# APRIL-ZJU/Ctrl-VIO

Measured on NVIDIA H100. Metric: residual+Jacobian block evaluations per second (sliding-window LM solve), higher is better.
Workload: dtype f64

## Files before the change

ctrl-vio_b200/csrc/engine.cu:

```cuda
#include <cuda_runtime.h>

#include <algorithm>
#include <atomic>
#include <chrono>
#include <cmath>
#include <cstdio>
#include <cstdlib>
#include <cstring>
#include <map>
#include <string>
#include <vector>

#include "../../include/ctvio.h"
#include "frontend.h"
#include "kernels.h"
#include "marginalize.h"
#include "poly_min.h"

using namespace ctvio;

namespace {

thread_local std::string g_err;
int fail(int code, const std::string& msg) {
// ... 205 lines not shown
    d.idx_ld = 6 * nK + 6 * nB;
    d.np = d.idx_ld + 1;
    return d;
  }
  NormalEqPtrs ne(int b) {
    double* s = ne_slab[b].p;
    return NormalEqPtrs{s, s + off_gc, s + off_hl, s + off_gl, s + off_wld, s + off_W, &d_scal.p->cost_eval};
  }
  LandmarkLayout lml() { return LandmarkLayout{d_lo.p, d_hi.p, d_woff.p}; }
};

namespace {

struct ArenaScope {
  PinnedArena* prev;
  explicit ArenaScope(ctvio_engine* e) : prev(g_arena) {
    if (e->stream && cudaStreamQuery(e->stream) == cudaSuccess) e->arena.rewind();
    else cudaGetLastError();
    g_arena = &e->arena;
  }
  ~ArenaScope() { g_arena = prev; }
};

int refresh_mirror(ctvio_engine* e, cudaStream_t on = nullptr) {
  const size_t need = 4 * size_t(e->nK) + kPStride * size_t(e->nK) + 6 * size_t(std::max(e->nB, 1)) + size_t(std::max(e->nL, 1)) + 8;
  if (need > e->h_mirror_cap) {
    if (e->h_mirror) cudaFreeHost(e->h_mirror);
    e->h_mirror = nullptr;
    e->h_mirror_cap = 0;
    if (cudaHostAlloc(reinterpret_cast<void**>(&e->h_mirror), (2 * need) * sizeof(double), cudaHostAllocDefault) != cudaSuccess) {
      cudaGetLastError();
      e->mirror_valid = false;
      return CTVIO_OK;
    }
    e->h_mirror_cap = 2 * need;
  }
  DevState& x = e->x[e->cur];
  double* m = e->h_mirror;
  cudaStream_t st = on ? on : e->stream;
  CUDA_OK(cudaMemcpyAsync(m, x.q.p, 4 * size_t(e->nK) * sizeof(double), cudaMemcpyDeviceToHost, st));
  m += 4 * size_t(e->nK);
  CUDA_OK(cudaMemcpyAsync(m, x.p.p, kPStride * size_t(e->nK) * sizeof(double), cudaMemcpyDeviceToHost, st));
  m += kPStride * size_t(e->nK);
  if (e->nB) CUDA_OK(cudaMemcpyAsync(m, x.bias.p, 6 * size_t(e->nB) * sizeof(double), cudaMemcpyDeviceToHost, st));
  m += 6 * size_t(std::max(e->nB, 1));
  if (e->nL) CUDA_OK(cudaMemcpyAsync(m, x.rho.p, size_t(e->nL) * sizeof(double), cudaMemcpyDeviceToHost, st));
  m += size_t(std::max(e->nL, 1));
  CUDA_OK(cudaMemcpyAsync(m, x.ld.p, sizeof(double), cudaMemcpyDeviceToHost, st));
  e->mirror_valid = true;
  return CTVIO_OK;
}

int knot_window_first(const ctvio_engine* e, int64_t t) {
  int64_t s = (t - e->cfg.t0_ns) / e->cfg.dt_ns;
  return int(s);
}

bool knot_window(const ctvio_engine* e, int64_t t, int& first, int& last) {
  const int64_t maxt = e->cfg.t0_ns + int64_t(e->nK - 3) * e->cfg.dt_ns;
  if (t < e->cfg.t0_ns || t >= maxt) return false;
  const int smax = e->nK - 4;
  const int s1 = knot_window_first(e, t);
  int64_t t2 = t + e->cfg.rs_padding_ns;
  int s2 = (t2 >= maxt) ? smax : int((t2 - e->cfg.t0_ns) / e->cfg.dt_ns);
  if (s2 > s1 + 1) return false;
  first = s1;
  last = std::min(s2 + 3, e->nK - 1);
  return true;
}

int prepare_prior(ctvio_engine* e);
int fetch_new_prior(ctvio_engine* e);

int prepare(ctvio_engine* e) {
  if (!e->have_knots) return fail(CTVIO_ERR_STATE, "knots have not been set");
  ArenaScope arena(e);
  static const bool prep_timing = std::getenv("CTVIO_PREP_TIMING") != nullptr;
  auto tp0 = std::chrono::steady_clock::now();
  auto lap = [&](const char* what) {
    if (!prep_timing) return;
    auto t = std::chrono::steady_clock::now();
    std::fprintf(stderr, "[prepare] %-22s %7.1f us\n", what, std::chrono::duration<double, std::micro>(t - tp0).count());
    tp0 = t;
  };
  if (e->nK < 4) return fail(CTVIO_ERR_STATE, "need at least 4 knots");
  if (!e->have_bias) { e->nB = 0; }
  cudaStream_t st = e->stream;
  const ProblemDims d = e->dims();
  if (e->structure_dirty) {
    e->shard_checked = false;
    const int n = int(e->img.size());
    std::vector<int32_t>&wi0 = e->img_wi0, &wj0 = e->img_wj0;
    wi0.resize(n); wj0.resize(n);
    e->img_li.resize(n); e->img_lj.resize(n);
    e->h_lo.assign(e->nL, INT32_MAX);
    e->h_hi.assign(e->nL, 0);
    struct WinCache { int64_t t = INT64_MIN; int f = 0, l = 0; bool ok = false; } wc[64];
    auto window_of = [&](int64_t t, int& f, int& l) {
      WinCache& c = wc[size_t(uint64_t(t) * 0x9E3779B97F4A7C15ull >> 58)];
      if (c.t != t) { c.t = t; c.ok = knot_window(e, t, c.f, c.l); }
      f = c.f; l = c.l;
      return c.ok;
    };
    for (int k = 0; k < n; ++k) {
      const HostImage& o = e->img[k];
      int f0, l0, f1, l1;
      if (!window_of(o.ti, f0, l0) || !window_of(o.tj, f1, l1))
        return fail(CTVIO_ERR_TIME_RANGE, "image factor time (+ rolling-shutter padding) outside the spline");
      if (o.lm < 0 || o.lm >= e->nL) return fail(CTVIO_ERR_INVALID, "landmark index out of range");
      wi0[k] = f0; wj0[k] = f1;
      e->img_li[k] = l0; e->img_lj[k] = l1;
      e->h_lo[o.lm] = std::min(e->h_lo[o.lm], 6 * std::min(f0, f1));
      e->h_hi[o.lm] = std::max(e->h_hi[o.lm], 6 * (std::max(l0, l1) + 1));
    }
    e->img_order.resize(n);
    {
      bool lm_sorted = true;
      for (int k = 1; k < n && lm_sorted; ++k) lm_sorted = e->img[k - 1].lm <= e->img[k].lm;
      const size_t nKk = size_t(e->nK) + 1;
      if (lm_sorted && nKk * nKk <= (size_t(1) << 22)) {
        std::vector<int32_t> start(nKk * nKk + 1, 0);
        for (int k = 0; k < n; ++k) ++start[size_t(wi0[k]) * nKk + size_t(wj0[k]) + 1];
        for (size_t g = 1; g < start.size(); ++g) start[g] += start[g - 1];
        for (int k = 0; k < n; ++k) e->img_order[start[size_t(wi0[k]) * nKk + size_t(wj0[k])]++] = k;
      } else {
        std::vector<uint64_t> key(n);
        const uint64_t nLl = uint64_t(std::max(e->nL, 1));
        if (uint64_t(nKk) * nKk * nLl < (uint64_t(1) << 40) && uint64_t(n) < (uint64_t(1) << 24)) {
          for (int k = 0; k < n; ++k)
            key[k] = (((uint64_t(wi0[k]) * nKk + uint64_t(wj0[k])) * nLl + uint64_t(e->img[k].lm)) << 24) | uint64_t(k);
          std::sort(key.begin(), key.end());
          for (int k = 0; k < n; ++k) e->img_order[k] = int32_t(key[k] & 0xffffffu);
        } else {
          for (int k = 0; k < n; ++k) e->img_order[k] = k;
          std::stable_sort(e->img_order.begin(), e->img_order.end(), [&](int a, int b) {
            if (wi0[a] != wi0[b]) return wi0[a] < wi0[b];
            if (wj0[a] != wj0[b]) return wj0[a] < wj0[b];
            return e->img[a].lm < e->img[b].lm;
          });
        }
      }
    }
    std::vector<longlong2> ht(n);
    std::vector<double2> hpi(n), hpj(n);
    std::vector<int4> hm(n);
    for (int k = 0; k < n; ++k) {
      const HostImage& o = e->img[e->img_order[k]];
      ht[k] = make_longlong2(o.ti, o.tj);
      hpi[k] = make_double2(o.pi[0], o.pi[1]);
      hpj[k] = make_double2(o.pj[0], o.pj[1]);
      hm[k] = make_int4(o.rowi, o.rowj, o.lm, o.marg);
    }
    lap("image windows + sort");
    int cap = kVisObsPerRound;
    if (const char* env = std::getenv("CTVIO_VIS_CAP")) cap = std::max(kVisObsPerRound, std::atoi(env) / kVisObsPerRound * kVisObsPerRound);
    std::vector<VisualItem>& items = e->h_items;
    items.clear();
    for (int k = 0; k < n;) {
      const int a = e->img_order[k];
      int end = k;
      while (end < n && wi0[e->img_order[end]] == wi0[a] && wj0[e->img_order[end]] == wj0[a]) ++end;
      const int cnt = end - k;
      const int nchunks = (cnt + cap - 1) / cap;
      const int per = (cnt + nchunks - 1) / nchunks;
      for (int s = k; s < end; s += per) items.push_back(VisualItem{s, std::min(per, end - s), wi0[a], wj0[a]});
      k = end;
    }
    e->n_items = int(items.size());
    if (!e->img_desc.empty()) {
      std::vector<ctvio::FactorDesc> sd(n);
      for (int k = 0; k < n; ++k) sd[k] = e->img_desc[e->img_order[k]];
      CUDA_OK(e->d_img_desc.upload(sd, st));
      CUDA_OK(e->d_img_t.reserve(n)); CUDA_OK(e->d_img_pi.reserve(n)); CUDA_OK(e->d_img_pj.reserve(n)); CUDA_OK(e->d_img_meta.reserve(n));
      ctvio::GatherFactorsArgs ga;
      ga.n = n; ga.desc = e->d_img_desc.p; ga.table = e->d_frames.p; ga.frame_t = e->d_frame_t.p;
      ga.frame_cap = ctvio_engine::kFrameCap;
      ga.t = e->d_img_t.p; ga.pi = e->d_img_pi.p; ga.pj = e->d_img_pj.p; ga.meta = e->d_img_meta.p;
      e->launches += ctvio::launch_gather_factors(ga, st);
    } else {
      CUDA_OK(e->d_img_t.upload(ht, st));
      CUDA_OK(e->d_img_pi.upload(hpi, st));
      CUDA_OK(e->d_img_pj.upload(hpj, st));
      CUDA_OK(e->d_img_meta.upload(hm, st));
    }
    CUDA_OK(e->d_img_orig.upload(e->img_order, st));
    CUDA_OK(e->d_items.upload(items, st));

    lap("image arrays + upload");
    e->h_woff.assign(e->nL + 1, 0);
    for (int l = 0; l < e->nL; ++l) {
      if (e->h_hi[l] == 0) e->h_lo[l] = 0;
      e->h_woff[l + 1] = e->h_woff[l] + (e->h_hi[l] - e->h_lo[l]);
    }
    CUDA_OK(e->d_lo.upload(e->h_lo, st));
    CUDA_OK(e->d_hi.upload(e->h_hi, st));
    CUDA_OK(e->d_woff.upload(e->h_woff, st));
    lap("landmark layout");
    const int ni = int(e->imu.size());
    std::vector<longlong2> it(ni);
    std::vector<double2> iga(3 * size_t(ni));
    const int64_t maxt = e->cfg.t0_ns + int64_t(e->nK - 3) * e->cfg.dt_ns;
    std::vector<int32_t>& imu_order = e->imu_order;
    imu_order.assign(ni, 0);
    std::vector<int32_t> imu_s(ni);
    for (int k = 0; k < ni; ++k) {
      const HostImu& o = e->imu[k];
      if (o.t < e->cfg.t0_ns || o.t >= maxt) return fail(CTVIO_ERR_TIME_RANGE, "imu time outside the spline");
      if (o.node < 0 || o.node >= e->nB) return fail(CTVIO_ERR_INVALID, "bias node out of range");
      imu_order[k] = k;
      imu_s[k] = knot_window_first(e, o.t);
    }
    std::stable_sort(imu_order.begin(), imu_order.end(), [&](int a, int b) {
      if (imu_s[a] != imu_s[b]) return imu_s[a] < imu_s[b];
      return e->imu[a].node < e->imu[b].node;
    });
    std::vector<ImuItem> imu_items;
    for (int k = 0; k < ni; ++k) {
      const HostImu& o = e->imu[imu_order[k]];
      it[k] = make_longlong2(o.t, o.node);
      iga[3 * k] = make_double2(o.gyro[0], o.gyro[1]);
      iga[3 * k + 1] = make_double2(o.gyro[2], o.accel[0]);
      iga[3 * k + 2] = make_double2(o.accel[1], o.accel[2]);
      const int s = imu_s[imu_order[k]];
      if (imu_items.empty() || imu_items.back().s != s || imu_items.back().node != o.node ||
          imu_items.back().count >= kImuMaxPerItem)
        imu_items.push_back(ImuItem{k, 0, s, o.node});
      imu_items.back().count++;
    }
    e->n_imu_items = int(imu_items.size());
    CUDA_OK(e->d_imu_items.upload(imu_items, st));
    CUDA_OK(e->d_imu_orig.upload(imu_order, st));
    if (!e->imu_src.empty()) {
      std::vector<int2> src(ni);
      for (int k = 0; k < ni; ++k) src[k] = make_int2(e->imu_src[imu_order[k]], e->imu[imu_order[k]].node);
      CUDA_OK(e->d_imu_src.upload(src, st));
      CUDA_OK(e->d_imu_t.reserve(ni)); CUDA_OK(e->d_imu_ga.reserve(3 * size_t(ni)));
      e->launches += ctvio::launch_gather_imu(e->d_imu_src.p, ni, e->d_imu_tab_t.p, e->d_imu_tab_ga.p, e->d_imu_t.p, e->d_imu_ga.p, st);
    } else {
      CUDA_OK(e->d_imu_t.upload(it, st));
      CUDA_OK(e->d_imu_ga.upload(iga, st));
    }
    const int nb = int(e->biasf.size());
    std::vector<int2> bij(nb);
    std::vector<double> bs(6 * size_t(nb));
    for (int k = 0; k < nb; ++k) {
      const HostBias& o = e->biasf[k];
      if (o.i < 0 || o.i >= e->nB || o.j < 0 || o.j >= e->nB) return fail(CTVIO_ERR_INVALID, "bias node out of range");
      bij[k] = make_int2(o.i, o.j);
      for (int c = 0; c < 6; ++c) bs[6 * k + c] = o.s[c];
    }
    CUDA_OK(e->d_bf_ij.upload(bij, st));
    CUDA_OK(e->d_bf_s.upload(bs, st));

    lap("imu / bias");
    const size_t np = size_t(d.np);
    e->off_gc = np * np;
    e->off_hl = e->off_gc + np;
    e->off_gl = e->off_hl + e->nL;
    e->off_wld = e->off_gl + e->nL;
    e->off_W = e->off_wld + e->nL;
    e->ne_slab_len = e->off_W + size_t(e->h_woff[e->nL]);
    for (int b = 0; b < 2; ++b) CUDA_OK(e->ne_slab[b].reserve(e->ne_slab_len));
    e->npad = ((d.np + kCholNB - 1) / kCholNB) * kCholNB;
    CUDA_OK(e->d_M.reserve(size_t(e->npad) * e->npad + 3 * size_t(e->npad)));
    if (chol_dag_lpub_len(e->npad) > e->d_Linv.cap || chol_dag_part_len(e->npad) > e->d_chol_part.cap || e->linv_npad != e->npad) {
      CUDA_OK(e->d_Linv.reserve(chol_dag_lpub_len(e->npad)));
      CUDA_OK(e->d_chol_part.reserve(chol_dag_part_len(e->npad)));
      e->launches += launch_chol_dag_init(e->d_Linv.p, e->d_chol_part.p, e->npad, e->stream);
      e->linv_npad = e->npad;
      e->chol_seq = 0;
    }
    lap("buffers");
    {
      const int T = e->npad / kCholNB;
      std::vector<std::vector<int32_t>> lists(size_t(T) * (T + 1) / 2);
      std::vector<int32_t> order;
      for (int l = 0; l < e->nL; ++l)
        if (e->h_hi[l] > 0) order.push_back(l);
      std::stable_sort(order.begin(), order.end(), [&](int a, int b) {
        if (e->h_lo[a] != e->h_lo[b]) return e->h_lo[a] < e->h_lo[b];
        return e->h_hi[a] < e->h_hi[b];
      });
      size_t total = 0;
      for (int l : order) {
        int blocks[64], nbk = 0;
        const int b0 = e->h_lo[l] / kCholNB, b1 = (e->h_hi[l] - 1) / kCholNB;
        for (int b = b0; b <= b1 && nbk < 63; ++b) blocks[nbk++] = b;
        for (int x = 0; x < nbk; ++x)
          for (int y = 0; y <= x; ++y) {
            lists[size_t(blocks[x]) * (blocks[x] + 1) / 2 + blocks[y]].push_back(l);
            ++total;
          }
      }
      const int n_sm = device_sm_count();
      const int part = std::max(32, int((total / size_t(2 * n_sm) + 31) / 32) * 32);
      std::vector<SchurTileItem> items;
      std::vector<SchurEntry> flat;
      flat.reserve(total);
      for (int ti = 0; ti < T; ++ti)
        for (int tj = 0; tj <= ti; ++tj) {
          const std::vector<int32_t>& v = lists[size_t(ti) * (ti + 1) / 2 + tj];
          for (size_t s0 = 0; s0 < v.size(); s0 += part)
            items.push_back(SchurTileItem{ti, tj, int32_t(flat.size() + s0), int32_t(std::min(v.size() - s0, size_t(part)))});
          for (int32_t l : v) flat.push_back(SchurEntry{l, e->h_lo[l], e->h_hi[l], 0, e->h_woff[l]});
        }
      e->n_schur_items = int(items.size());
      CUDA_OK(e->d_schur_list.upload(flat, st));
      CUDA_OK(e->d_schur_items.upload(items, st));
      CUDA_OK(e->d_lis.reserve(e->nL));
      CUDA_OK(e->d_lc.reserve(e->nL));
    }
    lap("schur lists");
    if (chol_dag_flags_len(e->npad) > e->d_chol_flags.cap) {
      CUDA_OK(e->d_chol_flags.reserve(chol_dag_flags_len(e->npad)));
      CUDA_OK(cudaMemsetAsync(e->d_chol_flags.p, 0, e->d_chol_flags.cap * sizeof(int32_t), e->stream));
    }
    CUDA_OK(e->d_y.reserve(e->npad));
    CUDA_OK(e->d_sc.reserve(np));
    CUDA_OK(e->d_sl.reserve(e->nL));
    CUDA_OK(e->d_hh.reserve(e->nL));
    CUDA_OK(e->d_dc.reserve(np));
    CUDA_OK(e->d_dl.reserve(e->nL));
    if (e->nL > 0) CUDA_OK(cudaMemsetAsync(e->d_hh.p, 0, sizeof(double) * e->nL, st));
    e->prior_dirty = true;
  }
  lap("reserves");
  if (e->structure_dirty || e->masks_dirty) {
    e->h_cmask.assign(d.np, 0);
    for (int k = 0; k < e->nK; ++k)
      if (e->opt.lock_traj || (e->opt.fixed_knot_index >= 0 && k <= e->opt.fixed_knot_index))
        for (int c = 0; c < 6; ++c) e->h_cmask[6 * k + c] = 1;
    for (int b = 0; b < e->nB; ++b)
      for (int c = 0; c < 3; ++c) {
        if (e->opt.lock_wb) e->h_cmask[d.idx_bias0 + 6 * b + c] = 1;
        if (e->opt.lock_ab) e->h_cmask[d.idx_bias0 + 6 * b + 3 + c] = 1;
      }
    if (e->opt.fix_ld) e->h_cmask[d.idx_ld] = 1;
    std::vector<uint8_t> touched(d.np + e->nL, 0);
    auto mark = [&](int f, int l) {
      for (int k = f; k <= l; ++k)
        for (int c = 0; c < 6; ++c) touched[6 * k + c] = 1;
    };
    {
      std::vector<uint8_t> seen(size_t(e->nK) * 8, 0);
      auto mark_once = [&](int f, int l) {
        uint8_t& sflag = seen[size_t(f) * 8 + size_t(l - f)];
        if (!sflag) { sflag = 1; mark(f, l); }
      };
      const size_t n = e->img.size();
      for (size_t k = 0; k < n; ++k) {
        mark_once(e->img_wi0[k], e->img_li[k]);
        mark_once(e->img_wj0[k], e->img_lj[k]);
        touched[d.np + e->img[k].lm] = 1;
      }
      if (n) touched[d.idx_ld] = 1;
    }
    for (const HostImu& o : e->imu) {
      const int s = knot_window_first(e, o.t);
      mark(s, s + 3);
      for (int c = 0; c < 6; ++c) touched[d.idx_bias0 + 6 * o.node + c] = 1;
    }
    for (const HostBias& o : e->biasf)
      for (int c = 0; c < 6; ++c) touched[d.idx_bias0 + 6 * o.i + c] = touched[d.idx_bias0 + 6 * o.j + c] = 1;
    if (e->prior.n > 0 && e->prior_enabled)
      for (size_t b = 0; b < e->prior.type.size(); ++b) {
        const int g = ctvio::prior_block_base(e->prior.type[b], e->prior.index[b], d.nK, d.nB);
        const int ls = (e->prior.type[b] == CTVIO_BLK_LD || e->prior.type[b] == CTVIO_BLK_RHO) ? 1 : 3;
        if (g >= 0) for (int c = 0; c < ls; ++c) touched[g + c] = 1;
      }
    e->h_active.assign(d.np + e->nL, 0);
    for (int i = 0; i < d.np; ++i) e->h_active[i] = touched[i] && !e->h_cmask[i];
    for (int l = 0; l < e->nL; ++l) e->h_active[d.np + l] = touched[d.np + l];
    CUDA_OK(e->d_cmask.upload(e->h_cmask, st));
    CUDA_OK(e->d_active.upload(e->h_active, st));
    e->masks_dirty = false;
  }
  lap("masks");
  e->structure_dirty = false;
  if (e->prior_dirty) {
    const int rc = prepare_prior(e);
    if (rc != CTVIO_OK) return rc;
  }
// ... 50 lines not shown
PriorPtrs prior_ptrs(ctvio_engine* e) {
  PriorPtrs p;
  std::memset(&p, 0, sizeof(p));
  p.n = e->prior_enabled ? e->prior.n : 0;
  if (p.n <= 0) return p;
  p.n_blocks = int(e->prior.type.size());
  p.J = e->d_prior_J.p; p.r = e->d_prior_r.p; p.JtJ = e->d_prior_JtJ.p;
  p.type = e->d_prior_type.p; p.index = e->d_prior_index.p; p.col = e->d_prior_col.p;
  p.x0 = e->d_prior_x0.p; p.col2g = e->d_prior_col2g.p;
  p.dx = e->d_prior_dx.p; p.res = e->d_prior_res.p;
  return p;
}

VisualLaunch visual_launch(ctvio_engine* e, int xb, int nb, double cauchy) {
  VisualLaunch v;
  v.obs = ImageObsPtrs{e->d_img_t.p, e->d_img_pi.p, e->d_img_pj.p, e->d_img_meta.p, int32_t(e->img.size())};
  v.items = e->d_items.p;
  v.n_items = e->n_items;
  v.st = e->state(xb).ptrs();
  v.ne = e->ne(nb);
  v.lm = e->lml();
  v.dims = e->dims();
  v.sp = e->sp;
  v.rig = e->rig;
  v.cauchy = cauchy;
  v.cmask = e->d_cmask.p;
  v.scal = e->d_scal.p;
  v.use_tma = e->use_tma;
  v.det_ticket = e->deterministic ? e->d_ticket.p : nullptr;
  return v;
}
ImuLaunch imu_launch(ctvio_engine* e, int xb, int nb) {
  ImuLaunch v;
  v.obs = ImuObsPtrs{e->d_imu_t.p, e->d_imu_ga.p, int32_t(e->imu.size())};
  v.items = e->d_imu_items.p;
  v.n_items = e->n_imu_items;
  v.st = e->state(xb).ptrs();
  v.ne = e->ne(nb);
  v.dims = e->dims();
  v.sp = e->sp;
  v.rig = e->rig;
  v.cmask = e->d_cmask.p;
  v.scal = e->d_scal.p;
  v.det_ticket = e->deterministic ? e->d_ticket.p : nullptr;
  return v;
}
SmallFactorsLaunch small_launch(ctvio_engine* e, int xb, int nb) {
  SmallFactorsLaunch v;
  v.bf = BiasFactorPtrs{e->d_bf_ij.p, e->d_bf_s.p, int32_t(e->biasf.size())};
  v.prior = prior_ptrs(e);
  v.st = e->state(xb).ptrs();
  v.ne = e->ne(nb);
  v.dims = e->dims();
  v.cmask = e->d_cmask.p;
  v.scal = e->d_scal.p;
  v.deterministic = e->deterministic ? 1 : 0;
  return v;
}
LinearLaunch linear_launch(ctvio_engine* e, int nb) {
  LinearLaunch a;
  a.dims = e->dims();
  a.ne = e->ne(nb);
  a.lm = e->lml();
  a.schur_list = e->d_schur_list.p;
  a.schur_items = e->d_schur_items.p;
  a.n_schur_items = e->n_schur_items;
  a.lis = e->d_lis.p; a.lc = e->d_lc.p;
  a.cmask = e->d_cmask.p;
  a.active = e->d_active.p;
  a.sc = e->d_sc.p; a.sl = e->d_sl.p;
  a.M = e->d_M.p; a.Linv = e->d_Linv.p; a.y = e->d_y.p;
  a.rhs = e->d_M.p + size_t(e->npad) * e->npad;
  a.diagA = a.rhs + e->npad;
  a.yf = a.diagA + e->npad;
  a.chol_part = e->d_chol_part.p; a.chol_flags = e->d_chol_flags.p; a.chol_seq = &e->chol_seq;
  a.sharded = e->world > 1 ? 1 : 0;
  a.hh = e->d_hh.p; a.dc = e->d_dc.p; a.dl = e->d_dl.p;
  a.npad = e->npad;
  a.scal = e->d_scal.p;
  a.go = nullptr;
  a.det_ticket = e->deterministic ? e->d_ticket.p : nullptr;
  return a;
}

int allreduce_scalars(ctvio_engine* e, bool publish = false) {
  if (e->world <= 1) return CTVIO_OK;
  CUDA_OK(e->d_shard_scal.reserve(8 + 8 * size_t(e->world)));
  e->launches += ctvio::launch_shard_scalars_pack(e->d_scal.p, e->d_shard_scal.p, e->stream);
  std::string err;
  if (!ctvio::comm_allgather(e->nccl_comm, e->d_shard_scal.p, e->d_shard_scal.p + 8, 8, e->stream, &err))
    return fail(CTVIO_ERR_NCCL, err);
  e->launches += ctvio::launch_shard_scalars_reduce(e->d_shard_scal.p + 8, e->world, e->d_scal.p, publish ? e->h_pub : nullptr,
                                                    publish ? ++e->pub_seq : 0, e->stream);
  return CTVIO_OK;
}

int shard_consensus(ctvio_engine* e, int local_rc) {
  if (e->world <= 1) return local_rc;
  const std::string local_msg = g_err;
  cudaStream_t st = e->stream;
  CUDA_OK(e->d_tmp.reserve(16));
  const double flag = local_rc ? 1.0 : 0.0;
  double total = 0.0;
  CUDA_OK(cudaMemcpyAsync(e->d_tmp.p, &flag, sizeof(double), cudaMemcpyHostToDevice, st));
  std::string err;
  if (!ctvio::comm_allreduce_sum(e->nccl_comm, e->d_tmp.p, 1, st, &err)) return fail(CTVIO_ERR_NCCL, err);
  CUDA_OK(cudaMemcpyAsync(&total, e->d_tmp.p, sizeof(double), cudaMemcpyDeviceToHost, st));
  CUDA_OK(cudaStreamSynchronize(st));
  if (local_rc) return fail(local_rc, local_msg);
  if (total != 0.0) return fail(CTVIO_ERR_STATE, "another rank of the sharded solve failed before the first collective");
  return CTVIO_OK;
}

int shard_check_ownership(ctvio_engine* e) {
  if (e->world <= 1 || e->shard_checked) return CTVIO_OK;
  cudaStream_t st = e->stream;
  std::vector<double> owned(size_t(std::max(e->nL, 1)), 0.0);
  for (const HostImage& o : e->img) owned[o.lm] = 1.0;
  CUDA_OK(e->d_rho_sync.reserve(2 * size_t(std::max(e->nL, 1))));
  CUDA_OK(cudaMemcpyAsync(e->d_rho_sync.p, owned.data(), owned.size() * sizeof(double), cudaMemcpyHostToDevice, st));
  std::string err;
  if (!ctvio::comm_allreduce_sum(e->nccl_comm, e->d_rho_sync.p, owned.size(), st, &err)) return fail(CTVIO_ERR_NCCL, err);
  CUDA_OK(cudaMemcpyAsync(owned.data(), e->d_rho_sync.p, owned.size() * sizeof(double), cudaMemcpyDeviceToHost, st));
  CUDA_OK(cudaStreamSynchronize(st));
  for (int l = 0; l < e->nL; ++l)
    if (owned[l] > 1.0)
      return fail(CTVIO_ERR_INVALID, "sharded solve: landmark " + std::to_string(l) + " has observations on " +
                                         std::to_string(int(owned[l])) + " ranks (shard image factors by landmark)");
  e->shard_checked = true;
  return CTVIO_OK;
}

int lm_step(ctvio_engine* e, int nb, double radius, const ApplyLaunch* fused_apply = nullptr, const double* radius_dev = nullptr,
            const int32_t* go = nullptr) {
  LinearLaunch lin = linear_launch(e, nb);
  lin.go = go;
  cudaStream_t st = e->stream;
  if (e->deterministic) cudaMemsetAsync(e->d_ticket.p, 0, 2 * sizeof(int32_t), st);
  e->launches += launch_reduced_system(lin, radius, st, radius_dev);
  if (e->world > 1) {
    std::string err;
    const size_t count = ctvio::shard_pack_len(e->npad);
    CUDA_OK(e->d_shard_pack.reserve(count));
    e->launches += ctvio::launch_shard_pack(lin, e->d_shard_pack.p, st);
    if (!ctvio::comm_allreduce_sum(e->nccl_comm, e->d_shard_pack.p, count, st, &err)) return fail(CTVIO_ERR_NCCL, err);
    e->launches += ctvio::launch_shard_unpack(lin, e->d_shard_pack.p, radius, st);
  }
  e->launches += launch_factor_solve(lin, st);
  if (fused_apply) e->launches += launch_step_and_apply(lin, *fused_apply, st);
  else e->launches += launch_step_vectors(lin, st);
  return CTVIO_OK;
}

void evaluate(ctvio_engine* e, int xb, int nb, bool full, bool reset_cost = true) {
  cudaStream_t st = e->stream;
  if (full) {
    if (e->slab_zeroed[nb]) {
      cudaStreamWaitEvent(st, e->ev_zero, 0);
      e->slab_zeroed[nb] = false;
    } else {
      cudaMemsetAsync(e->ne_slab[nb].p, 0, e->ne_slab_len * sizeof(double), st);
    }
  }
  if (reset_cost) cudaMemsetAsync(&e->d_scal.p->cost_eval, 0, sizeof(double), st);
  const bool fork = (e->rank == 0) && (!e->imu.empty() || !e->biasf.empty() || (e->prior.n > 0 && e->prior_enabled));
  if (e->deterministic) {
    cudaMemsetAsync(e->d_ticket.p, 0, 2 * sizeof(int32_t), st);
    e->launches += launch_visual(visual_launch(e, xb, nb, e->cfg.cauchy_solve), full, st);
    if (fork) {
      cudaMemsetAsync(e->d_ticket.p, 0, 2 * sizeof(int32_t), st);
      e->launches += launch_imu(imu_launch(e, xb, nb), full, st);
      e->launches += launch_small_factors(small_launch(e, xb, nb), full, st);
    }
    return;
  }
  const bool split = fork && !e->imu.empty() && (!e->biasf.empty() || (e->prior.n > 0 && e->prior_enabled));
  if (fork) {
    cudaEventRecord(e->ev_fork, st);
    cudaStreamWaitEvent(e->stream2, e->ev_fork, 0);
    e->launches += launch_imu(imu_launch(e, xb, nb), full, e->stream2);
    if (split) {
      cudaStreamWaitEvent(e->stream3, e->ev_fork, 0);
      e->launches += launch_small_factors(small_launch(e, xb, nb), full, e->stream3);
      cudaEventRecord(e->ev_join3, e->stream3);
    } else {
      e->launches += launch_small_factors(small_launch(e, xb, nb), full, e->stream2);
    }
    cudaEventRecord(e->ev_join, e->stream2);
  }
  e->launches += launch_visual(visual_launch(e, xb, nb, e->cfg.cauchy_solve), full, st);
  if (fork) cudaStreamWaitEvent(st, e->ev_join, 0);
  if (split) cudaStreamWaitEvent(st, e->ev_join3, 0);
}

void prezero_slab(ctvio_engine* e, int nb) {
  cudaMemsetAsync(e->ne_slab[nb].p, 0, e->ne_slab_len * sizeof(double), e->stream2);
  cudaEventRecord(e->ev_zero, e->stream2);
  e->slab_zeroed[nb] = true;
}

int read_scalars(ctvio_engine* e, bool published = false) {
  if (published) {
    volatile unsigned long long* seq = &e->h_pub->seq;
    unsigned spins = 0;
    while (*seq != e->pub_seq) {
      if ((++spins & 0xfffu) == 0 && cudaStreamQuery(e->stream) != cudaErrorNotReady) {
        if (*seq == e->pub_seq) break;
        CUDA_OK(cudaStreamSynchronize(e->stream));
        CUDA_OK(cudaStreamSynchronize(e->stream2));
        if (*seq != e->pub_seq) return fail(CTVIO_ERR_CUDA, "LM step finished without publishing its scalars");
      }
    }
    std::atomic_thread_fence(std::memory_order_acquire);
    *e->h_scal = const_cast<const LmPublished*>(e->h_pub)->s;
  } else {
    CUDA_OK(cudaMemcpyAsync(e->h_scal, e->d_scal.p, sizeof(LmScalars), cudaMemcpyDeviceToHost, e->stream));
    CUDA_OK(cudaStreamSynchronize(e->stream));
  }
  if ((e->h_scal->error_flags & 1) || (e->world > 1 && e->h_scal->err_sum > 0.0)) {
    cudaMemsetAsync(&e->d_scal.p->error_flags, 0, sizeof(int32_t), e->stream);
    return fail(CTVIO_ERR_TIME_RANGE, "a factor time left its knot window / the spline (line delay too large?)");
  }
  return CTVIO_OK;
}

int ensure_table(ctvio_engine* e) {
  if (!e->table_valid) {
    e->launches += launch_knot_table(e->x[e->cur].ptrs(), e->nK, e->stream);
    e->table_valid = true;
  }
  return CTVIO_OK;
}

int alloc_state(ctvio_engine* e, DevState& s) {
  CUDA_OK(s.q.reserve(4 * size_t(e->nK)));
  CUDA_OK(s.p.reserve(kPStride * size_t(e->nK)));
  CUDA_OK(s.tab.reserve(size_t(std::max(e->nK - 1, 1))));
  CUDA_OK(s.bias.reserve(6 * size_t(std::max(e->nB, 1))));
  CUDA_OK(s.rho.reserve(size_t(std::max(e->nL, 1))));
  CUDA_OK(s.ld.reserve(1));
  return CTVIO_OK;
}

}

extern "C" {

const char* ctvio_last_error(void) { return g_err.c_str(); }
int ctvio_abi_version(void) { return CTVIO_ABI_VERSION; }

int ctvio_create(const ctvio_config* cfg, ctvio_handle* out) {
  if (!cfg || !out) return fail(CTVIO_ERR_INVALID, "null argument");
  if (cfg->dt_ns <= 0) return fail(CTVIO_ERR_INVALID, "dt_ns must be positive");
  if (cfg->rs_padding_ns < 0 || cfg->rs_padding_ns > cfg->dt_ns)
    return fail(CTVIO_ERR_INVALID, "rs_padding_ns must lie in [0, dt_ns]: the staged knot window holds 5 knots "
                                   "(4 + one interval of rolling-shutter padding, se3_spline.h:463-503 with 39 ms / 50 ms)");
  int ndev = 0;
  if (cudaGetDeviceCount(&ndev) != cudaSuccess || ndev == 0)
    return fail(CTVIO_ERR_NO_DEVICE, "no CUDA device visible: the ctvio engine has no CPU fallback");
  if (cfg->device < 0 || cfg->device >= ndev) return fail(CTVIO_ERR_NO_DEVICE, "device ordinal out of range");
  CUDA_OK(cudaSetDevice(cfg->device));
  cudaDeviceProp prop;
  CUDA_OK(cudaGetDeviceProperties(&prop, cfg->device));
  if (prop.major != 9 || prop.minor != 0)
    return fail(CTVIO_ERR_NO_DEVICE, "libctvio_b200 is built for sm_90a (H100) only");
  ctvio_engine* e = new ctvio_engine();
  e->cfg = *cfg;
  std::memset(&e->opt, 0, sizeof(e->opt));
  e->opt.fixed_knot_index = -1;
  e->opt.fix_ld = 1;
  e->sp = SplineParams{cfg->t0_ns, cfg->dt_ns, 0, 1e9 / double(cfg->dt_ns)};
  e->rig.R_CI = so3_matrix(Q4{cfg->q_CtoI[0], cfg->q_CtoI[1], cfg->q_CtoI[2], cfg->q_CtoI[3]});
  e->rig.p_CI = V3{cfg->p_CinI[0], cfg->p_CinI[1], cfg->p_CinI[2]};
  e->rig.w_img = cfg->image_weight;
  e->rig.gravity = V3{cfg->gravity[0], cfg->gravity[1], cfg->gravity[2]};
  for (int k = 0; k < 6; ++k) e->rig.imu_info[k] = cfg->imu_info[k];
  if (const char* det = std::getenv("CTVIO_DETERMINISTIC")) e->deterministic = det[0] == '1';
  if (const char* ns = std::getenv("CTVIO_NO_SPECULATION")) e->speculate = ns[0] != '1';
  if (const char* dp = std::getenv("CTVIO_STAGED_PUBLISH")) e->staged_publish = dp[0] == '1';
  const char* no_tma = std::getenv("CTVIO_NO_TMA");
  e->use_tma = !(no_tma && no_tma[0] == '1');
  if (cudaStreamCreateWithFlags(&e->stream, cudaStreamNonBlocking) != cudaSuccess ||
      cudaStreamCreateWithFlags(&e->stream2, cudaStreamNonBlocking) != cudaSuccess ||
      cudaStreamCreateWithFlags(&e->stream3, cudaStreamNonBlocking) != cudaSuccess ||
      cudaEventCreateWithFlags(&e->ev_join3, cudaEventDisableTiming) != cudaSuccess ||
      cudaEventCreate(&e->ev0) != cudaSuccess || cudaEventCreate(&e->ev1) != cudaSuccess ||
      cudaEventCreateWithFlags(&e->ev_fork, cudaEventDisableTiming) != cudaSuccess ||
      cudaEventCreateWithFlags(&e->ev_join, cudaEventDisableTiming) != cudaSuccess ||
      cudaEventCreateWithFlags(&e->ev_zero, cudaEventDisableTiming) != cudaSuccess ||
      cudaEventCreate(&e->ev_iter) != cudaSuccess || e->d_dec.reserve(1) != cudaSuccess || e->d_pubstage.reserve(1) != cudaSuccess ||
      cudaHostAlloc(&e->h_pub, sizeof(LmPublished), cudaHostAllocMapped) != cudaSuccess ||
      cudaMallocHost(&e->h_scal, sizeof(LmScalars)) != cudaSuccess || e->d_scal.reserve(1) != cudaSuccess ||
      e->d_ticket.reserve(4) != cudaSuccess) {
    delete e;
    return fail(CTVIO_ERR_CUDA, "could not create stream / events / scalar block");
  }
  cudaMemsetAsync(e->d_scal.p, 0, sizeof(LmScalars), e->stream);
  std::memset(e->h_pub, 0, sizeof(LmPublished));
  *out = e;
  return CTVIO_OK;
}

int ctvio_destroy(ctvio_handle e) {
  if (!e) return CTVIO_OK;
  cudaSetDevice(e->cfg.device);
  cudaStreamSynchronize(e->stream);
  ctvio::comm_destroy(e->nccl_comm);
  if (e->h_scal) cudaFreeHost(e->h_scal);
  if (e->h_pub) cudaFreeHost(e->h_pub);
  if (e->h_mirror) cudaFreeHost(e->h_mirror);
  if (e->ev_zero) cudaEventDestroy(e->ev_zero);
  cudaEventDestroy(e->ev0);
  cudaEventDestroy(e->ev1);
  cudaEventDestroy(e->ev_fork);
  cudaEventDestroy(e->ev_join);
  cudaStreamDestroy(e->stream2);
  if (e->stream3) cudaStreamDestroy(e->stream3);
  if (e->ev_join3) cudaEventDestroy(e->ev_join3);
  cudaStreamDestroy(e->stream);
  delete e;
  return CTVIO_OK;
}

int ctvio_set_options(ctvio_handle e, const ctvio_options* o) {
  if (!e || !o) return fail(CTVIO_ERR_INVALID, "null argument");
  e->opt = *o;
  e->masks_dirty = true;
  e->prior_dirty = true;
  return CTVIO_OK;
}

int ctvio_set_knots(ctvio_handle e, int32_t n, const double* q, const double* p) {
  if (!e || !q || !p || n < 4) return fail(CTVIO_ERR_INVALID, "need >= 4 knots");
  cudaSetDevice(e->cfg.device);
  if (n != e->nK) e->structure_dirty = true;
  e->nK = n;
  e->sp.n_knots = n;
  for (int b = 0; b < 2; ++b) { const int rc = alloc_state(e, e->x[b]); if (rc) return rc; }
  ArenaScope arena(e);
  std::vector<double> p4(kPStride * size_t(n), 0.0);
  for (int k = 0; k < n; ++k) for (int c = 0; c < 3; ++c) p4[kPStride * k + c] = p[3 * k + c];
  CUDA_OK(staged_h2d(e->x[e->cur].q.p, q, 4 * size_t(n) * sizeof(double), e->stream));
  CUDA_OK(staged_h2d(e->x[e->cur].p.p, p4.data(), p4.size() * sizeof(double), e->stream));
  e->mirror_valid = false;
  e->h2d_bytes += size_t(n) * 56;
// ... 158 lines not shown
                    const int32_t* index, const int32_t* col, const double* x0) {
  if (!e) return fail(CTVIO_ERR_INVALID, "null handle");
  e->prior = ctvio::PriorHost();
  e->prior_dirty = true;
  e->prior_on_device = false;
  e->masks_dirty = true;
  if (n <= 0) return CTVIO_OK;
  if (!J || !r || nb <= 0 || !type || !index || !col || !x0) return fail(CTVIO_ERR_INVALID, "null argument");
  {
    std::vector<uint8_t> covered(size_t(n), 0);
    for (int b = 0; b < nb; ++b) {
      if (type[b] < CTVIO_BLK_ROT || type[b] > CTVIO_BLK_RHO) return fail(CTVIO_ERR_INVALID, "prior block type out of range");
      const int ls = (type[b] == CTVIO_BLK_LD || type[b] == CTVIO_BLK_RHO) ? 1 : 3;
      if (col[b] < 0 || col[b] + ls > n) return fail(CTVIO_ERR_INVALID, "prior block column outside [0, n)");
      for (int c = 0; c < ls; ++c) {
        if (covered[col[b] + c]) return fail(CTVIO_ERR_INVALID, "prior blocks overlap");
        covered[col[b] + c] = 1;
      }
    }
    for (int c = 0; c < n; ++c)
      if (!covered[c]) return fail(CTVIO_ERR_INVALID, "prior blocks do not cover all n columns");
  }
  e->prior.n = n;
  e->prior.J.assign(J, J + size_t(n) * n);
  e->prior.r.assign(r, r + n);
  e->prior.type.assign(type, type + nb);
  e->prior.index.assign(index, index + nb);
  e->prior.col.assign(col, col + nb);
  e->prior.x0.assign(x0, x0 + 4 * size_t(nb));
  return CTVIO_OK;
}

int ctvio_solve(ctvio_handle e, int32_t max_iterations, ctvio_summary* out) {
  if (!e) return fail(CTVIO_ERR_INVALID, "null handle");
  cudaSetDevice(e->cfg.device);
  int rc = prepare(e);
  rc = shard_consensus(e, rc);
  if (rc) return rc;
  rc = shard_check_ownership(e);
  if (rc) return rc;
  cudaStream_t st = e->stream;
  const ProblemDims d = e->dims();
  const double initial_radius = 1e4, max_radius = 1e16, min_radius = 1e-32, min_relative_decrease = 1e-3;
  const double function_tolerance = 1e-6, gradient_tolerance = 1e-10, parameter_tolerance = 1e-8;
  const int max_consecutive_invalid = 5;
  const double ls_sufficient_decrease = 1e-4, ls_max_contraction = 1e-3, ls_min_contraction = 0.6, ls_min_step = 1e-9;
  const int ls_max_iterations = 20;

  ctvio_summary sum;
  std::memset(&sum, 0, sizeof(sum));
  const int64_t launches0 = e->launches;
  cudaEventRecord(e->ev0, st);

  const bool is_constrained = !e->opt.fix_ld && (e->world > 1 || e->h_active[d.idx_ld]);
  if (is_constrained) {
    double ld;
    CUDA_OK(cudaMemcpyAsync(&ld, e->x[e->cur].ld.p, sizeof(double), cudaMemcpyDeviceToHost, st));
    CUDA_OK(cudaStreamSynchronize(st));
    const double c = std::min(std::max(ld, e->opt.ld_lower), e->opt.ld_upper);
    if (c != ld) CUDA_OK(cudaMemcpyAsync(e->x[e->cur].ld.p, &c, sizeof(double), cudaMemcpyHostToDevice, st));
  }
  ensure_table(e);
  const bool sharded = e->world > 1;
  int cur = e->cur;
  evaluate(e, cur, cur, true);
  sum.num_jacobian_evals++;
  LinearLaunch lin = linear_launch(e, cur);
  if (sharded) {
    e->launches += launch_extract_diag(lin, st);
    std::string err;
    if (!ctvio::comm_allreduce_sum(e->nccl_comm, lin.diagA, size_t(e->npad), st, &err)) return fail(CTVIO_ERR_NCCL, err);
    e->launches += launch_jacobi_scale_from_diag(lin, st);
  } else {
    e->launches += launch_jacobi_scale(lin, st);
  }
  if (sharded) {
    e->launches += launch_gradient_norm(lin, e->x[cur].ptrs(), e->opt.fix_ld, e->opt.ld_lower, e->opt.ld_upper, st);
    rc = allreduce_scalars(e);
    if (rc) return rc;
    rc = read_scalars(e);
  } else {
    e->launches += launch_gradient_norm(lin, e->x[cur].ptrs(), e->opt.fix_ld, e->opt.ld_lower, e->opt.ld_upper, st, true, e->h_pub,
                                        ++e->pub_seq);
    rc = read_scalars(e, true);
  }
  if (rc) return rc;
  double x_cost = e->h_scal->cost_eval;
  double gmax = e->h_scal->gmax;
  sum.initial_cost = x_cost;
  sum.num_successful_steps = 1;

  double radius = initial_radius, decrease_factor = 2.0;
  int num_invalid = 0;
  bool last_ok = true;
  int iter = 0;
  int term = CTVIO_TERM_NO_CONVERGENCE;

  auto make_apply = [&](int from, int to, double alpha) {
    ApplyLaunch ap;
    ap.dims = d;
    ap.x = e->state(from).ptrs();
    ap.xc = e->state(to).ptrs();
    ap.dc = e->d_dc.p; ap.dl = e->d_dl.p;
    ap.alpha = alpha;
    ap.active = e->d_active.p;
    ap.count_camera = e->rank == 0 ? 1 : 0;
    ap.clamp_ld = e->opt.fix_ld ? 0 : 1;
    ap.ld_lower = e->opt.ld_lower; ap.ld_upper = e->opt.ld_upper;
    ap.scal = e->d_scal.p;
    ap.det_ticket = e->deterministic ? e->d_ticket.p : nullptr;
    return ap;
  };
  auto apply = [&](int from, int to, double alpha, bool reset = true) {
    if (e->deterministic) cudaMemsetAsync(e->d_ticket.p, 0, 2 * sizeof(int32_t), st);
    e->launches += launch_apply_step(make_apply(from, to, alpha), st, reset);
  };

  bool spec_size_ok = e->img.size() <= 20000;
  if (const char* sp = std::getenv("CTVIO_SPECULATION")) {
    if (std::strcmp(sp, "always") == 0) spec_size_ok = true;
    if (std::strcmp(sp, "never") == 0) spec_size_ok = false;
  }
  const bool pipelined = e->speculate && spec_size_ok && !sharded && !is_constrained && !e->deterministic;
  int cur_ne = cur;
  if (pipelined) {
    rc = alloc_state(e, e->xs);
    if (rc) return rc;
    bool spec_ready = false;
    bool spec_in_flight = false;
    int spec_out = -1;
    unsigned spec_chol_seq0 = e->chol_seq;
    double host_spec_us = 0, host_wait_us = 0;
    static const bool lm_trace = std::getenv("CTVIO_LM_TRACE") != nullptr;
    cudaEventRecord(e->ev_iter, st);
    while (true) {
      if (iter >= max_iterations) { term = CTVIO_TERM_NO_CONVERGENCE; break; }
      if (last_ok && gmax <= gradient_tolerance) { term = CTVIO_TERM_GRADIENT; break; }
      if (radius < min_radius) { term = CTVIO_TERM_MIN_RADIUS; break; }
      ++iter;
      const int cand_ne = cur_ne ^ 1;
      int cand;
      if (spec_ready) {
        cand = spec_out;
        prezero_slab(e, cand_ne);
      } else {
        cand = 0;
        while (cand == cur) ++cand;
        if (!spec_in_flight) prezero_slab(e, cand_ne);
        const ApplyLaunch full_step = make_apply(cur, cand, 1.0);
        rc = lm_step(e, cur_ne, radius, &full_step);
        if (rc) return rc;
      }
      sum.num_linear_solves++;
      evaluate(e, cand, cand_ne, true, false);
      sum.num_jacobian_evals++;
      const LmDecideArgs da{e->d_dec.p, x_cost, radius, min_relative_decrease, max_radius,
                            parameter_tolerance, function_tolerance, gradient_tolerance, min_radius};
      e->launches += launch_gradient_norm(linear_launch(e, cand_ne), e->state(cand).ptrs(), e->opt.fix_ld, e->opt.ld_lower,
                                          e->opt.ld_upper, st, false, e->staged_publish ? e->d_pubstage.p : e->h_pub, ++e->pub_seq,
                                          &da);
      cudaEventRecord(e->ev_iter, st);
      if (e->staged_publish) {
        cudaStreamWaitEvent(e->stream2, e->ev_iter, 0);
        e->launches += launch_publish(e->d_pubstage.p, e->h_pub, e->stream2);
      }
      spec_ready = false;
      if (iter < max_iterations) {
        spec_out = 0;
        while (spec_out == cur || spec_out == cand) ++spec_out;
        const ApplyLaunch spec_step = make_apply(cand, spec_out, 1.0);
        spec_chol_seq0 = e->chol_seq;
        const auto th0 = std::chrono::steady_clock::now();
        rc = lm_step(e, cand_ne, 0.0, &spec_step, &e->d_dec.p->radius_next, &e->d_dec.p->go);
        if (rc) return rc;
        spec_ready = true;
        spec_in_flight = true;
        host_spec_us += std::chrono::duration<double, std::micro>(std::chrono::steady_clock::now() - th0).count();
      }
      const auto th1 = std::chrono::steady_clock::now();
      rc = read_scalars(e, true);
      host_wait_us += std::chrono::duration<double, std::micro>(std::chrono::steady_clock::now() - th1).count();
      if (rc) return rc;
      const LmScalars sc = *e->h_scal;
      const LmDecision dec = const_cast<const LmPublished*>(e->h_pub)->dec;
      if (spec_ready && !dec.go) {
        e->chol_seq = spec_chol_seq0;
        spec_ready = false;
      }
      if (!dec.valid) {
        spec_ready = false;
        ++sum.num_unsuccessful_steps;
        last_ok = false;
        if (++num_invalid >= max_consecutive_invalid) { term = CTVIO_TERM_FAILURE; break; }
        radius /= decrease_factor;
        decrease_factor *= 2.0;
        continue;
      }
      num_invalid = 0;
      const double step_norm = std::sqrt(sc.step_norm2), x_norm = std::sqrt(sc.x_norm2);
      if (step_norm <= parameter_tolerance * (x_norm + parameter_tolerance)) { term = CTVIO_TERM_PARAMETER; break; }
      const double cost_change = x_cost - sc.cost_eval;
      if (std::fabs(cost_change) <= function_tolerance * x_cost) { term = CTVIO_TERM_FUNCTION; break; }
      if (dec.accept) {
        cur = cand;
        cur_ne = cand_ne;
        x_cost = sc.cost_eval;
        gmax = sc.gmax;
        radius = dec.radius_next;
        decrease_factor = 2.0;
        last_ok = true;
        ++sum.num_successful_steps;
        if (!spec_ready) spec_in_flight = false;
      } else {
        spec_ready = false;
        radius /= decrease_factor;
        decrease_factor *= 2.0;
        last_ok = false;
        ++sum.num_unsuccessful_steps;
      }
    }
    if (cur == 2) {
      const int f = 0;
      DevState &a = e->xs, &b = e->x[f];
      std::swap(a.q.p, b.q.p); std::swap(a.q.cap, b.q.cap);
      std::swap(a.p.p, b.p.p); std::swap(a.p.cap, b.p.cap);
      std::swap(a.bias.p, b.bias.p); std::swap(a.bias.cap, b.bias.cap);
      std::swap(a.rho.p, b.rho.p); std::swap(a.rho.cap, b.rho.cap);
      std::swap(a.ld.p, b.ld.p); std::swap(a.ld.cap, b.ld.cap);
      std::swap(a.tab.p, b.tab.p); std::swap(a.tab.cap, b.tab.cap);
      cur = f;
    }
    e->cur = cur;
    e->table_valid = true;
    e->slab_zeroed[0] = e->slab_zeroed[1] = false;
    CUDA_OK(cudaStreamWaitEvent(e->stream2, e->ev_iter, 0));
    {
      const int rcm = refresh_mirror(e, e->stream2);
      if (rcm) return rcm;
    }
    CUDA_OK(cudaStreamSynchronize(e->stream2));
    float ms = 0;
    cudaEventElapsedTime(&ms, e->ev0, e->ev_iter);
    if (lm_trace) std::fprintf(stderr, "[lm] iters %d device %.3f ms host: spec enqueue %.1f us/iter, wait %.1f us/iter\n", iter, ms, host_spec_us / std::max(iter, 1), host_wait_us / std::max(iter, 1));
    sum.iterations = iter;
    sum.termination = term;
    sum.final_cost = x_cost;
    sum.final_radius = radius;
    sum.device_ms = ms;
    sum.kernel_launches = e->launches - launches0;
    if (out) *out = sum;
    return CTVIO_OK;
  }

  while (true) {
    if (iter >= max_iterations) { term = CTVIO_TERM_NO_CONVERGENCE; break; }
    if (last_ok && gmax <= gradient_tolerance) { term = CTVIO_TERM_GRADIENT; break; }
    if (radius < min_radius) { term = CTVIO_TERM_MIN_RADIUS; break; }
    ++iter;
    const int cand = cur ^ 1;
    prezero_slab(e, cand);
    const ApplyLaunch full_step = make_apply(cur, cand, 1.0);
    rc = lm_step(e, cur, radius, &full_step);
    if (rc) return rc;
    sum.num_linear_solves++;
    evaluate(e, cand, cand, true, false);
    sum.num_jacobian_evals++;
    LinearLaunch linc = linear_launch(e, cand);
    if (!sharded) {
      e->launches += launch_gradient_norm(linc, e->x[cand].ptrs(), e->opt.fix_ld, e->opt.ld_lower, e->opt.ld_upper, st, false,
                                          e->h_pub, ++e->pub_seq);
    } else {
      e->launches += launch_gradient_norm(linc, e->x[cand].ptrs(), e->opt.fix_ld, e->opt.ld_lower, e->opt.ld_upper, st, false,
                                          nullptr, 0);
      rc = allreduce_scalars(e, true);
      if (rc) return rc;
    }
    rc = read_scalars(e, true);
    if (rc) return rc;
    LmScalars sc = *e->h_scal;
    const double model_cost_change = -sc.gd - 0.5 * sc.dHd;
    const bool valid = !sc.chol_fail && std::isfinite(model_cost_change) && model_cost_change > 0.0;
    if (!valid) {
      ++sum.num_unsuccessful_steps;
      last_ok = false;
      if (++num_invalid >= max_consecutive_invalid) { term = CTVIO_TERM_FAILURE; break; }
      radius /= decrease_factor;
      decrease_factor *= 2.0;
      continue;
    }
    num_invalid = 0;
    double cand_cost = sc.cost_eval, cand_gmax = sc.gmax, step_norm2 = sc.step_norm2, x_norm2 = sc.x_norm2;
    if (is_constrained) {
      const double g0 = sc.gd;
      struct Sample { double x, value, gradient; bool value_ok, grad_ok; };
      Sample initial{0.0, x_cost, g0, true, true}, previous{0, 0, 0, false, false};
      Sample current{1.0, cand_cost, 0.0, std::isfinite(cand_cost), false};
      bool have_grad = false;
      int ls_iters = 0;
      bool success = true;
      while (!current.value_ok || current.value > x_cost + ls_sufficient_decrease * g0 * current.x) {
        ++ls_iters;
        if (ls_iters >= ls_max_iterations) { success = false; break; }
        if (current.value_ok && !have_grad) {
          e->launches += ctvio::launch_dot_gradient(linear_launch(e, cand), st);
          rc = allreduce_scalars(e);
          if (rc) return rc;
          rc = read_scalars(e);
          if (rc) return rc;
          current.gradient = e->h_scal->gd;
          current.grad_ok = std::isfinite(current.gradient);
        }
        const double smin = ls_max_contraction * current.x, smax = ls_min_contraction * current.x;
        double step;
// ... 190 lines not shown
  if (!e || !counts || !sums) return fail(CTVIO_ERR_INVALID, "null argument");
  cudaSetDevice(e->cfg.device);
  int rc = prepare(e);
  if (rc) return rc;
  ensure_table(e);
  cudaStream_t st = e->stream;
  const size_t ni = e->img.size(), nm = e->imu.size(), nb = e->biasf.size();
  const int np_ = e->prior_enabled ? e->prior.n : 0;
  DevBuf<double> dr, dout;
  DevBuf<int32_t> ds;
  CUDA_OK(dr.reserve(2 * ni + 6 * nm + 8));
  CUDA_OK(ds.reserve(2 * ni + nm + 8));
  CUDA_OK(dout.reserve(18));
  CUDA_OK(cudaMemsetAsync(dout.p, 0, 18 * sizeof(double), st));
  if (ni) e->launches += launch_probe_image(visual_launch(e, e->cur, e->cur, 0.0), e->d_img_orig.p, false, dr.p, ds.p, nullptr, st);
  if (nm) e->launches += launch_probe_imu(imu_launch(e, e->cur, e->cur), e->d_imu_orig.p, false, dr.p + 2 * ni, ds.p + 2 * ni, nullptr, st);
  e->launches += ctvio::launch_abs_column_sums(dr.p, int(ni), 2, dout.p, st);
  e->launches += ctvio::launch_abs_column_sums(dr.p + 2 * ni, int(nm), 6, dout.p + 2, st);
  e->launches += ctvio::launch_bias_abs_sums(e->d_bf_ij.p, e->d_bf_s.p, int(nb), e->x[e->cur].bias.p, dout.p + 8, st);
  if (np_ > 0) {
    e->launches += launch_small_factors(small_launch(e, e->cur, e->cur), false, st);
  }
  rc = read_scalars(e);
  if (rc) return rc;
  CUDA_OK(cudaMemcpy(sums, dout.p, 18 * sizeof(double), cudaMemcpyDeviceToHost));
  counts[0] = int32_t(ni); counts[1] = int32_t(nm); counts[2] = int32_t(nb); counts[3] = np_ > 0 ? 1 : 0;
  if (prior_sum && np_ > 0) {
    CUDA_OK(cudaMemcpy(prior_sum, e->d_prior_res.p, size_t(np_) * sizeof(double), cudaMemcpyDeviceToHost));
    for (int i = 0; i < np_; ++i) prior_sum[i] = std::fabs(prior_sum[i]);
  }
  return CTVIO_OK;
}

int ctvio_eval_cost(ctvio_handle e, double* cost) {
  if (!e || !cost) return fail(CTVIO_ERR_INVALID, "null argument");
  cudaSetDevice(e->cfg.device);
  int rc = prepare(e);
  if (rc) return rc;
  ensure_table(e);
  evaluate(e, e->cur, e->cur, false);
  rc = read_scalars(e);
  if (rc) return rc;
  *cost = e->h_scal->cost_eval;
  return CTVIO_OK;
}

int ctvio_normal_equations(ctvio_handle e, double* Hcc, double* gc, double* hl, double* gl, double* cost) {
  if (!e) return fail(CTVIO_ERR_INVALID, "null handle");
  cudaSetDevice(e->cfg.device);
  int rc = prepare(e);
  if (rc) return rc;
  ensure_table(e);
  evaluate(e, e->cur, e->cur, true);
  rc = read_scalars(e);
  if (rc) return rc;
  const ProblemDims d = e->dims();
  const size_t np = d.np;
  NormalEqPtrs ne = e->ne(e->cur);
  if (Hcc) {
    std::vector<double> up(np * np);
    CUDA_OK(cudaMemcpy(up.data(), ne.A, np * np * sizeof(double), cudaMemcpyDeviceToHost));
    for (size_t i = 0; i < np; ++i)
      for (size_t j = i; j < np; ++j) Hcc[i * np + j] = Hcc[j * np + i] = up[i * np + j];
  }
  if (gc) CUDA_OK(cudaMemcpy(gc, ne.gc, np * sizeof(double), cudaMemcpyDeviceToHost));
  if (hl && e->nL) CUDA_OK(cudaMemcpy(hl, ne.hl, e->nL * sizeof(double), cudaMemcpyDeviceToHost));
  if (gl && e->nL) CUDA_OK(cudaMemcpy(gl, ne.gl, e->nL * sizeof(double), cudaMemcpyDeviceToHost));
  if (cost) *cost = e->h_scal->cost_eval;
  return CTVIO_OK;
}

int ctvio_query_trajectory(ctvio_handle e, int32_t n, const int64_t* t, double* q, double* p, double* omega,
                           double* vel, double* acc) {
  if (!e || n < 0 || (n > 0 && !t)) return fail(CTVIO_ERR_INVALID, "bad argument");
  if (!e->have_knots) return fail(CTVIO_ERR_STATE, "knots have not been set");
  cudaSetDevice(e->cfg.device);
  ensure_table(e);
  if (n == 0) return CTVIO_OK;
  DevBuf<int64_t> dt;
  DevBuf<double> out;
  CUDA_OK(dt.reserve(n));
  CUDA_OK(out.reserve(16 * size_t(n)));
  cudaStream_t st = e->stream;
  CUDA_OK(cudaMemcpyAsync(dt.p, t, size_t(n) * sizeof(int64_t), cudaMemcpyHostToDevice, st));
  QueryLaunch a;
  a.st = e->x[e->cur].ptrs();
  a.sp = e->sp;
  a.n = n;
  a.t = dt.p;
  a.q = out.p; a.p = out.p + 4 * size_t(n); a.omega = out.p + 7 * size_t(n); a.vel = out.p + 10 * size_t(n);
  a.acc = out.p + 13 * size_t(n);
  a.scal = e->d_scal.p;
  e->launches += launch_query(a, st);
  int rc = read_scalars(e);
  if (rc) return rc;
  if (q) CUDA_OK(cudaMemcpy(q, a.q, 4 * size_t(n) * sizeof(double), cudaMemcpyDeviceToHost));
  if (p) CUDA_OK(cudaMemcpy(p, a.p, 3 * size_t(n) * sizeof(double), cudaMemcpyDeviceToHost));
  if (omega) CUDA_OK(cudaMemcpy(omega, a.omega, 3 * size_t(n) * sizeof(double), cudaMemcpyDeviceToHost));
  if (vel) CUDA_OK(cudaMemcpy(vel, a.vel, 3 * size_t(n) * sizeof(double), cudaMemcpyDeviceToHost));
  if (acc) CUDA_OK(cudaMemcpy(acc, a.acc, 3 * size_t(n) * sizeof(double), cudaMemcpyDeviceToHost));
  return CTVIO_OK;
}

int ctvio_triangulate(ctvio_handle e, int32_t n_frames, const double* Rs, const double* Ps, const double* ric,
                      const double* tic, int32_t nl, const int32_t* start_frame, const int32_t* obs_offset,
                      const double* obs_point, int32_t window_size, double init_depth, double* depth) {
  if (!e || n_frames <= 0 || !Rs || !Ps || !ric || !tic || nl < 0 || (nl > 0 && (!start_frame || !obs_offset || !obs_point || !depth)))
    return fail(CTVIO_ERR_INVALID, "bad argument");
  if (nl == 0) return CTVIO_OK;
  cudaSetDevice(e->cfg.device);
  const int total = obs_offset[nl];
  if (total < 0) return fail(CTVIO_ERR_INVALID, "obs_offset must be non-decreasing");
  for (int l = 0; l < nl; ++l)
    if (obs_offset[l + 1] < obs_offset[l]) return fail(CTVIO_ERR_INVALID, "obs_offset must be non-decreasing");
  cudaStream_t st = e->stream;
  const size_t nd = 12 * size_t(n_frames) + 3 * size_t(total) + size_t(nl);
  CUDA_OK(e->d_tmp.reserve(nd));
  CUDA_OK(e->d_tri_idx.reserve(2 * size_t(nl) + 1));
  double* dRs = e->d_tmp.p;
  double* dPs = dRs + 9 * size_t(n_frames);
  double* dobs = dPs + 3 * size_t(n_frames);
  double* ddepth = dobs + 3 * size_t(total);
  CUDA_OK(cudaMemcpyAsync(dRs, Rs, 9 * size_t(n_frames) * sizeof(double), cudaMemcpyHostToDevice, st));
  CUDA_OK(cudaMemcpyAsync(dPs, Ps, 3 * size_t(n_frames) * sizeof(double), cudaMemcpyHostToDevice, st));
  if (total) CUDA_OK(cudaMemcpyAsync(dobs, obs_point, 3 * size_t(total) * sizeof(double), cudaMemcpyHostToDevice, st));
  CUDA_OK(cudaMemcpyAsync(ddepth, depth, size_t(nl) * sizeof(double), cudaMemcpyHostToDevice, st));
  CUDA_OK(cudaMemcpyAsync(e->d_tri_idx.p, start_frame, size_t(nl) * sizeof(int32_t), cudaMemcpyHostToDevice, st));
  CUDA_OK(cudaMemcpyAsync(e->d_tri_idx.p + nl, obs_offset, (size_t(nl) + 1) * sizeof(int32_t), cudaMemcpyHostToDevice, st));
  ctvio::TriangulateArgs a;
  a.n_frames = n_frames; a.Rs = dRs; a.Ps = dPs;
  for (int k = 0; k < 9; ++k) a.ric.m[k] = ric[k];
  a.tic = V3{tic[0], tic[1], tic[2]};
  a.n_landmarks = nl; a.start_frame = e->d_tri_idx.p; a.obs_offset = e->d_tri_idx.p + nl; a.obs_point = dobs;
  a.window_size = window_size; a.init_depth = init_depth; a.depth = ddepth;
  e->launches += ctvio::launch_triangulate(a, st);
  CUDA_OK(cudaMemcpyAsync(depth, ddepth, size_t(nl) * sizeof(double), cudaMemcpyDeviceToHost, st));
  CUDA_OK(cudaStreamSynchronize(st));
  return CTVIO_OK;
}

int ctvio_profile_kernels(ctvio_handle e, int32_t reps, int32_t flush_l2, double* out) {
  if (!e || !out || reps == 0) return fail(CTVIO_ERR_INVALID, "bad argument");
  const bool visual_only = reps < 0;
  if (visual_only) reps = -reps;
  cudaSetDevice(e->cfg.device);
  int rc = prepare(e);
  if (rc) return rc;
  ensure_table(e);
  cudaStream_t st = e->stream;
  const int cur = e->cur, cand = cur ^ 1;
  DevBuf<unsigned char> flush;
  const size_t flush_bytes = size_t(256) << 20;
  if (flush_l2) CUDA_OK(flush.reserve(flush_bytes));
  if (visual_only) {
    for (int k = 0; k < 8; ++k) out[k] = 0.0;
    double total = 0;
    for (int it = -3; it < reps; ++it) {
      if (flush_l2) cudaMemsetAsync(flush.p, it & 0xff, flush_bytes, st);
      cudaMemsetAsync(e->ne_slab[cur].p, 0, e->ne_slab_len * sizeof(double), st);
      cudaEventRecord(e->ev0, st);
      launch_visual(visual_launch(e, cur, cur, e->cfg.cauchy_solve), true, st);
      cudaEventRecord(e->ev1, st);
      if (cudaEventSynchronize(e->ev1) != cudaSuccess) return fail(CTVIO_ERR_CUDA, "kernel failed while profiling");
      float ms = 0;
      cudaEventElapsedTime(&ms, e->ev0, e->ev1);
      if (it >= 0) total += ms;
    }
    out[0] = total / reps;
    cudaMemsetAsync(&e->d_scal.p->error_flags, 0, sizeof(int32_t), st);
    CUDA_OK(cudaStreamSynchronize(st));
    return CTVIO_OK;
  }
  evaluate(e, cur, cur, true);
  LinearLaunch lin = linear_launch(e, cur);
  launch_jacobi_scale(lin, st);
  launch_lm_step(lin, 1e4, st);
  rc = read_scalars(e);
  if (rc) return rc;
  ApplyLaunch ap;
  ap.dims = e->dims();
  ap.x = e->x[cur].ptrs(); ap.xc = e->x[cand].ptrs();
  ap.dc = e->d_dc.p; ap.dl = e->d_dl.p; ap.alpha = 1.0; ap.active = e->d_active.p;
  ap.count_camera = 1;
  ap.clamp_ld = e->opt.fix_ld ? 0 : 1; ap.ld_lower = e->opt.ld_lower; ap.ld_upper = e->opt.ld_upper;
  ap.scal = e->d_scal.p;
  auto time_stage = [&](int stage, double* ms_out) -> int {
    double total = 0;
    for (int it = -3; it < reps; ++it) {
      if (flush_l2) cudaMemsetAsync(flush.p, it & 0xff, flush_bytes, st);
      if (stage == 0 || stage == 1 || stage == 2)
        cudaMemsetAsync(e->ne_slab[cur].p, 0, e->ne_slab_len * sizeof(double), st);
      cudaEventRecord(e->ev0, st);
      switch (stage) {
        case 0: launch_visual(visual_launch(e, cur, cur, e->cfg.cauchy_solve), true, st); break;
        case 1: launch_imu(imu_launch(e, cur, cur), true, st); break;
        case 2: launch_small_factors(small_launch(e, cur, cur), true, st); break;
        case 3: launch_reduced_system(lin, 1e4, st); break;
        case 4: launch_factor_solve(lin, st); break;
        case 5: launch_step_vectors(lin, st); break;
        case 6: launch_apply_step(ap, st); break;
        default: launch_visual(visual_launch(e, cur, cur, e->cfg.cauchy_solve), false, st); break;
      }
      cudaEventRecord(e->ev1, st);
      if (cudaEventSynchronize(e->ev1) != cudaSuccess) return fail(CTVIO_ERR_CUDA, "kernel failed while profiling");
      float ms = 0;
      cudaEventElapsedTime(&ms, e->ev0, e->ev1);
      if (it >= 0) total += ms;
    }
    *ms_out = total / reps;
    return CTVIO_OK;
  };
  for (int stage : {0, 1, 2, 7}) { rc = time_stage(stage, &out[stage]); if (rc) return rc; }
  evaluate(e, cur, cur, true);
  {
    double total3 = 0, total4 = 0, total5 = 0;
    for (int it = -3; it < reps; ++it) {
      float ms;
      if (flush_l2) cudaMemsetAsync(flush.p, it & 0xff, flush_bytes, st);
      cudaEventRecord(e->ev0, st); launch_reduced_system(lin, 1e4, st); cudaEventRecord(e->ev1, st);
      cudaEventSynchronize(e->ev1); cudaEventElapsedTime(&ms, e->ev0, e->ev1); if (it >= 0) total3 += ms;
      if (flush_l2) cudaMemsetAsync(flush.p, it & 0xff, flush_bytes, st);
      cudaEventRecord(e->ev0, st); launch_factor_solve(lin, st); cudaEventRecord(e->ev1, st);
      cudaEventSynchronize(e->ev1); cudaEventElapsedTime(&ms, e->ev0, e->ev1); if (it >= 0) total4 += ms;
      if (flush_l2) cudaMemsetAsync(flush.p, it & 0xff, flush_bytes, st);
      cudaEventRecord(e->ev0, st); launch_step_vectors(lin, st); cudaEventRecord(e->ev1, st);
      cudaEventSynchronize(e->ev1); cudaEventElapsedTime(&ms, e->ev0, e->ev1); if (it >= 0) total5 += ms;
    }
    out[3] = total3 / reps; out[4] = total4 / reps; out[5] = total5 / reps;
  }
  rc = time_stage(6, &out[6]);
  if (rc) return rc;
  cudaMemsetAsync(&e->d_scal.p->error_flags, 0, sizeof(int32_t), st);
  CUDA_OK(cudaStreamSynchronize(st));
  return CTVIO_OK;
}

int ctvio_selfcheck_solver(ctvio_handle e, int32_t reps, int32_t* mismatches, double* rel_residual) {
  if (!e || !mismatches || !rel_residual || reps <= 0) return fail(CTVIO_ERR_INVALID, "bad argument");
  cudaSetDevice(e->cfg.device);
  int rc = prepare(e);
  if (rc) return rc;
  ensure_table(e);
  cudaStream_t st = e->stream;
  const int cur = e->cur;
  evaluate(e, cur, cur, true);
  LinearLaunch lin = linear_launch(e, cur);
  launch_jacobi_scale(lin, st);
  launch_reduced_system(lin, 1e4, st);
  const size_t n = size_t(e->npad), len = n * n + n;
  DevBuf<double> backup;
  CUDA_OK(backup.reserve(len));
  CUDA_OK(cudaMemcpyAsync(backup.p, lin.M, len * sizeof(double), cudaMemcpyDeviceToDevice, st));
  std::vector<double> hM(len), x0(n), x(n);
  CUDA_OK(cudaMemcpyAsync(hM.data(), lin.M, len * sizeof(double), cudaMemcpyDeviceToHost, st));
  *mismatches = 0;
  for (int r = 0; r < reps; ++r) {
    if (r > 0) CUDA_OK(cudaMemcpyAsync(lin.M, backup.p, len * sizeof(double), cudaMemcpyDeviceToDevice, st));
    launch_factor_solve(lin, st);
    CUDA_OK(cudaMemcpyAsync((r == 0 ? x0 : x).data(), lin.y, n * sizeof(double), cudaMemcpyDeviceToHost, st));
    CUDA_OK(cudaStreamSynchronize(st));
    if (r > 0 && std::memcmp(x.data(), x0.data(), n * sizeof(double)) != 0) ++*mismatches;
  }
  for (size_t i = 0; i < n; ++i)
    for (size_t j = i + 1; j < n; ++j) hM[i * n + j] = hM[j * n + i];
  const double* rhs = hM.data() + n * n;
  double rmax = 0, bmax = 0;
  for (size_t i = 0; i < n; ++i) {
    double s = -rhs[i];
    for (size_t j = 0; j < n; ++j) s += hM[i * n + j] * x0[j];
    rmax = std::max(rmax, std::fabs(s));
    bmax = std::max(bmax, std::fabs(rhs[i]));
  }
  *rel_residual = bmax > 0 ? rmax / bmax : rmax;
  cudaMemsetAsync(&e->d_scal.p->error_flags, 0, sizeof(int32_t), st);
  CUDA_OK(cudaStreamSynchronize(st));
  return CTVIO_OK;
}

int ctvio_measure_fp64_tflops(ctvio_handle e, double* tflops) {
  if (!e || !tflops) return fail(CTVIO_ERR_INVALID, "null argument");
  cudaSetDevice(e->cfg.device);
  const double v = ctvio::measure_fp64_tflops(e->stream);
  if (v < 0) return fail(CTVIO_ERR_CUDA, "fp64 micro-benchmark failed");
  *tflops = v;
  return CTVIO_OK;
}

int ctvio_measure_fp64_tensor_tflops(ctvio_handle e, double* tflops) {
  if (!e || !tflops) return fail(CTVIO_ERR_INVALID, "null argument");
  cudaSetDevice(e->cfg.device);
  const double v = ctvio::measure_fp64_tensor_tflops(e->stream);
  if (v < 0) return fail(CTVIO_ERR_CUDA, "fp64 tensor-core micro-benchmark failed");
  *tflops = v;
  return CTVIO_OK;
}

int ctvio_marginalize(ctvio_handle e, int32_t* n_out, int32_t* nb_out) {
  if (!e || !n_out || !nb_out) return fail(CTVIO_ERR_INVALID, "null argument");
  *n_out = 0;
  *nb_out = 0;
  cudaSetDevice(e->cfg.device);
  e->new_prior = ctvio::PriorHost();
  if (!e->opt.is_marg_state) return CTVIO_OK;
  ArenaScope arena(e);
  int rc = prepare(e);
  if (rc) return rc;
  ensure_table(e);
  cudaStream_t st = e->stream;
  const ProblemDims d = e->dims();
  const int later = e->opt.ctrl_to_be_opt_later, nowk = e->opt.ctrl_to_be_opt_now;
  const bool drop_knots = later > nowk;

  struct Key {
    int type, index;
    bool operator<(const Key& o) const {
      auto rank = [](const Key& k) {
        switch (k.type) {
          case CTVIO_BLK_ROT: return std::make_pair(0, 2 * k.index);
          case CTVIO_BLK_POS: return std::make_pair(0, 2 * k.index + 1);
          case CTVIO_BLK_BG: return std::make_pair(1, 2 * k.index);
          case CTVIO_BLK_BA: return std::make_pair(1, 2 * k.index + 1);
          case CTVIO_BLK_LD: return std::make_pair(2, 0);
          default: return std::make_pair(3, k.index);
        }
      };
      return rank(*this) < rank(o);
    }
  };
  struct Info { bool dropped = false; int pos = -1; };
  std::map<Key, Info> blocks;
  auto touch = [&](int type, int index, bool drop) { Info& b = blocks[Key{type, index}]; b.dropped = b.dropped || drop; };
  bool use_prior = false;
  if (e->prior.n > 0) {
    auto is_drop = [&](size_t b) {
      const int t = e->prior.type[b], i = e->prior.index[b];
      const bool isknot = t == CTVIO_BLK_ROT || t == CTVIO_BLK_POS;
      return (isknot && i >= nowk && i < later) || ((t == CTVIO_BLK_BG || t == CTVIO_BLK_BA) && i == 0);
    };
    for (size_t b = 0; b < e->prior.type.size(); ++b) use_prior = use_prior || is_drop(b);
    if (use_prior)
      for (size_t b = 0; b < e->prior.type.size(); ++b) touch(e->prior.type[b], e->prior.index[b], is_drop(b));
  }
  std::vector<int32_t> marg_img, marg_imu;
  for (size_t k = 0; k < e->img_order.size(); ++k) {
    const HostImage& o = e->img[e->img_order[k]];
    if (!o.marg) continue;
    marg_img.push_back(int32_t(k));
    int f0, l0, f1, l1;
    knot_window(e, o.ti, f0, l0);
    knot_window(e, o.tj, f1, l1);
    for (int side = 0; side < 2; ++side)
      for (int kk = (side ? f1 : f0); kk <= (side ? l1 : l0); ++kk) {
        touch(CTVIO_BLK_ROT, kk, drop_knots && kk < later);
        touch(CTVIO_BLK_POS, kk, drop_knots && kk < later);
// ... 498 lines not shown
```

ctrl-vio_b200/csrc/kernels.h:

```cpp
#pragma once
#include <cuda_runtime.h>

#include <atomic>

#include <cstdint>

#include "spline_eval.cuh"

namespace ctvio {

constexpr int kPStride = 4;
constexpr int kVisThreads = 256;
constexpr int kVisObsPerRound = 128;
constexpr int kLocalDim = 64;
constexpr int kRowStride = 66;
constexpr int kObsStride = 2 * kRowStride + 2;
constexpr int kWinKnots = 5;
constexpr int kColLd = 60, kColR = 61, kColRho = 62;
constexpr int kCholNB = 64;

struct StatePtrs {
  double* q;
  double* p;
  double* bias;
// ... 21 lines not shown
};

struct VisualItem {
  int32_t start, count;
  int32_t wi0, wj0;
};

struct ImuObsPtrs {
  const longlong2* t_node;
  const double2* ga;
  int32_t n;
};

struct ImuItem {
  int32_t start, count;
  int32_t s, node;
};
constexpr int kImuMaxPerItem = 32;

struct BiasFactorPtrs {
  const int2* ij;
  const double* sqrt_info;
  int32_t n;
};

struct PriorPtrs {
  int32_t n, n_blocks;
  const double* J;
  const double* r;
  const double* JtJ;
  const int32_t* type;
  const int32_t* index;
  const int32_t* col;
  const double* x0;
  const int32_t* col2g;
  double* dx;
  double* res;
};

struct ProblemDims {
  int32_t nK, nB, nL, np, idx_bias0, idx_ld;
};

struct LandmarkLayout {
  const int32_t* lo;
  const int32_t* hi;
  const int64_t* woff;
};

struct SchurEntry {
  int32_t l, lo, hi, pad;
  int64_t woff;
};
struct SchurTileItem {
  int32_t ti, tj;
  int32_t first, count;
};

struct LmScalars {
  double cost_eval;
  double gd;
  double dHd;
  double step_norm2;
  double x_norm2;
  double err_sum;
  double gmax;
  double dir_max;
  double ld_value;
  int32_t chol_fail;
  int32_t error_flags;
  int32_t pad[2];
};
struct LmDecision {
  double radius_next;
  double model_cost_change;
  double rho;
  int32_t valid;
  int32_t accept;
  int32_t go;
  int32_t pad;
};
struct LmDecideArgs {
  LmDecision* dec;
  double x_cost, radius;
  double min_relative_decrease, max_radius;
  double parameter_tolerance, function_tolerance, gradient_tolerance, min_radius;
};
struct LmPublished {
  LmScalars s;
  LmDecision dec;
  unsigned long long seq;
  unsigned long long pad;
};
constexpr int kLmSumScalars = 6;

struct PerDeviceOnce {
  std::atomic<unsigned long long> mask{0};
  bool first() {
    int d = 0;
    cudaGetDevice(&d);
    const unsigned long long bit = 1ull << (d & 63);
    return !(mask.fetch_or(bit) & bit);
  }
};
inline int device_sm_count() {
  static std::atomic<int> cache[64];
  int d = 0;
  cudaGetDevice(&d);
  int v = cache[d & 63].load(std::memory_order_relaxed);
  if (v == 0) {
    cudaDeviceGetAttribute(&v, cudaDevAttrMultiProcessorCount, d);
    cache[d & 63].store(v, std::memory_order_relaxed);
  }
  return v;
}

#if defined(__CUDACC__)
__device__ __forceinline__ void det_ticket_wait(const int* ticket, int my) {
  if (!ticket) return;
  if (threadIdx.x == 0) {
    int v;
    do { asm volatile("ld.acquire.gpu.global.s32 %0, [%1];" : "=r"(v) : "l"(ticket) : "memory"); } while (v != my);
  }
  __syncthreads();
}
__device__ __forceinline__ void det_ticket_done(int* ticket, int my) {
  if (!ticket) return;
  __threadfence();
  __syncthreads();
  if (threadIdx.x == 0) asm volatile("st.release.gpu.global.s32 [%0], %1;" ::"l"(ticket), "r"(my + 1) : "memory");
}
#endif

int launch_knot_table(const StatePtrs& st, int nK, cudaStream_t s);

struct VisualLaunch {
  ImageObsPtrs obs;
  const VisualItem* items;
  int32_t n_items;
  StatePtrs st;
  NormalEqPtrs ne;
  LandmarkLayout lm;
  ProblemDims dims;
  SplineParams sp;
  RigParams rig;
  double cauchy;
  const uint8_t* cmask;
  LmScalars* scal;
  bool use_tma;
  int* det_ticket = nullptr;
};
int launch_visual(const VisualLaunch& a, bool full, cudaStream_t s);
size_t visual_smem_bytes();

struct ImuLaunch {
  ImuObsPtrs obs;
  const ImuItem* items;
  int32_t n_items;
  StatePtrs st;
  NormalEqPtrs ne;
  ProblemDims dims;
  SplineParams sp;
  RigParams rig;
  const uint8_t* cmask;
  LmScalars* scal;
  int* det_ticket = nullptr;
};
int launch_imu(const ImuLaunch& a, bool full, cudaStream_t s);

struct SmallFactorsLaunch {
  BiasFactorPtrs bf;
  PriorPtrs prior;
  StatePtrs st;
  NormalEqPtrs ne;
  ProblemDims dims;
  const uint8_t* cmask;
  LmScalars* scal;
  int deterministic = 0;
};
int launch_small_factors(const SmallFactorsLaunch& a, bool full, cudaStream_t s);

int launch_probe_image(const VisualLaunch& a, const int32_t* orig_index, bool want_jac, double* r, int32_t* s,
                       double* J, cudaStream_t st);
int launch_probe_imu(const ImuLaunch& a, const int32_t* orig_index, bool want_jac, double* r, int32_t* s, double* J,
                     cudaStream_t st);

struct LinearLaunch {
  ProblemDims dims;
  NormalEqPtrs ne;
  LandmarkLayout lm;
  const SchurEntry* schur_list;
  const SchurTileItem* schur_items;
  int32_t n_schur_items;
  double* lis;
  double* lc;
  const uint8_t* cmask;
  const uint8_t* active;
  double* sc;
  double* sl;
  double* M;
  double* Linv;
  double* rhs;
  double* y;
  double* yf;
  double* chol_part;
  int32_t* chol_flags;
  unsigned* chol_seq;
  double* hh;
  double* diagA;
  int32_t sharded;
  double* dc;
  double* dl;
  int32_t npad;
  LmScalars* scal;
  int* det_ticket;
  const int32_t* go;
};
int launch_jacobi_scale(const LinearLaunch& a, cudaStream_t s);
int launch_lm_step(const LinearLaunch& a, double radius, cudaStream_t s);
int launch_reduced_system(const LinearLaunch& a, double radius, cudaStream_t s, const double* radius_dev = nullptr);
int launch_publish(const LmPublished* stage, LmPublished* pub, cudaStream_t s);
int launch_factor_solve(const LinearLaunch& a, cudaStream_t s);
bool chol_dag_supported(int npad, int n_sm);
size_t chol_dag_part_len(int npad);
size_t chol_dag_flags_len(int npad);
size_t chol_dag_lpub_len(int npad);
int launch_chol_dag_init(double* linv_buf, double* part_buf, int npad, cudaStream_t s);
int launch_chol_dag(const LinearLaunch& a, cudaStream_t s);
int launch_chol_coop(const LinearLaunch& a, cudaStream_t s);
int launch_step_vectors(const LinearLaunch& a, cudaStream_t s);
int launch_add_damping(const LinearLaunch& a, double radius, cudaStream_t s);
int launch_extract_diag(const LinearLaunch& a, cudaStream_t s);
int launch_jacobi_scale_from_diag(const LinearLaunch& a, cudaStream_t s);
int launch_gradient_norm(const LinearLaunch& a, const StatePtrs& st, int fix_ld, double ld_lower, double ld_upper,
                         cudaStream_t s, bool reset = true, LmPublished* pub = nullptr, unsigned long long seq = 0,
                         const LmDecideArgs* decide = nullptr);

struct ApplyLaunch {
  int32_t count_camera;
  ProblemDims dims;
  StatePtrs x, xc;
  const double* dc;
  const double* dl;
  double alpha;
  const uint8_t* active;
  int32_t clamp_ld;
  double ld_lower, ld_upper;
  LmScalars* scal;
  int* det_ticket = nullptr;
};
int launch_apply_step(const ApplyLaunch& a, cudaStream_t s, bool reset = true);
int launch_step_and_apply(const LinearLaunch& a, const ApplyLaunch& ap, cudaStream_t s);
int launch_gauge_realign(const StatePtrs& st, int nK, int min_idx, const double* R0_t0_dev, cudaStream_t s);

struct QueryLaunch {
  StatePtrs st;
  SplineParams sp;
  int32_t n;
  const int64_t* t;
  double *q, *p, *omega, *vel, *acc;
  LmScalars* scal;
};
int launch_query(const QueryLaunch& a, cudaStream_t s);

}
```

ctrl-vio_b200/csrc/kernels_linear.cu:

```cuda
#include <algorithm>

#include "dmma_tiles.cuh"
#include <cstddef>

#include "kernels.h"

namespace ctvio {

__device__ __forceinline__ double warp_sum_d(double v) {
#pragma unroll
  for (int o = 16; o > 0; o >>= 1) v += __shfl_xor_sync(0xffffffffu, v, o);
  return v;
}
__device__ __forceinline__ double warp_max_d(double v) {
#pragma unroll
  for (int o = 16; o > 0; o >>= 1) v = fmax(v, __shfl_xor_sync(0xffffffffu, v, o));
  return v;
}
__device__ __forceinline__ void atomic_max_pos(double* addr, double v) {
  atomicMax(reinterpret_cast<unsigned long long*>(addr), static_cast<unsigned long long>(__double_as_longlong(v)));
}

constexpr double kMinLmDiag = 1e-6, kMaxLmDiag = 1e32;

__global__ void jacobi_scale_kernel(LinearLaunch a) {
  const int i = blockIdx.x * blockDim.x + threadIdx.x;
  const int np = a.dims.np;
  if (i < np) a.sc[i] = 1.0 / (1.0 + sqrt(a.ne.A[size_t(i) * np + i]));
  if (i < a.dims.nL) a.sl[i] = 1.0 / (1.0 + sqrt(a.ne.hl[i]));
}
int launch_jacobi_scale(const LinearLaunch& a, cudaStream_t s) {
  const int n = max(a.dims.np, a.dims.nL);
  jacobi_scale_kernel<<<(n + 255) / 256, 256, 0, s>>>(a);
  return 1;
}

__global__ void scale_copy_kernel(LinearLaunch a, double radius, const double* __restrict__ radius_dev) {
  if (radius_dev) radius = *radius_dev;
  const int npad = a.npad, np = a.dims.np;
  const size_t idx = size_t(blockIdx.x) * blockDim.x + threadIdx.x;
  if (idx < size_t(a.dims.nL)) {
    const int l = int(idx);
    const double sl = a.sl[l], hl = a.ne.hl[l];
    const double hs = sl * sl * hl;
    const double hh = hl > 0.0 ? hs + fmin(fmax(hs, kMinLmDiag), kMaxLmDiag) / radius : 0.0;
    const double is = hh > 0.0 ? rsqrt(hh) * sl : 0.0;
    a.hh[l] = hh;
    a.lis[l] = is;
    a.lc[l] = is * a.ne.gl[l];
  }
  if (idx >= size_t(npad) * npad) return;
  const int i = int(idx / npad), j = int(idx % npad);
  double m;
  const double ident = a.sharded ? 0.0 : 1.0;
  if (i < np && j < np) {
    if (a.cmask[i] || a.cmask[j]) {
      m = (i == j) ? ident : 0.0;
    } else {
      const double v = (i <= j) ? a.ne.A[size_t(i) * np + j] : a.ne.A[size_t(j) * np + i];
      m = a.sc[i] * v * a.sc[j];
      if (i == j) {
        if (a.sharded) a.diagA[i] = v;
        else m += fmin(fmax(m, kMinLmDiag), kMaxLmDiag) / radius;
      }
    }
  } else {
    m = (i == j) ? ident : 0.0;
    if (a.sharded && i == j) a.diagA[i] = 0.0;
  }
  if (a.sharded && i == j && i < np && a.cmask[i]) a.diagA[i] = 0.0;
  a.M[idx] = m;
  if (j == 0) {
    a.rhs[i] = (i < np && !a.cmask[i]) ? a.sc[i] * a.ne.gc[i] : 0.0;
    if (i == 0) {
      a.scal->gd = 0.0;
      a.scal->dHd = 0.0;
      a.scal->dir_max = 0.0;
      a.scal->chol_fail = 0;
      a.scal->step_norm2 = 0.0;
      a.scal->x_norm2 = 0.0;
      a.scal->cost_eval = 0.0;
      a.scal->gmax = 0.0;
    }
  }
}

constexpr int kSchurKC = 32;
__device__ __forceinline__ void schur_fetch(const LinearLaunch& a, const SchurTileItem& it, int c0, int k, int dseg,
                                            const double* scA, const double* scB, double sc_ld, bool diag, double va[8],
                                            double vb[8], double cl[3]) {
#pragma unroll
  for (int e = 0; e < 8; ++e) va[e] = vb[e] = 0.0;
  cl[0] = cl[1] = cl[2] = 0.0;
  if (c0 + k >= it.count) return;
  const SchurEntry en = a.schur_list[it.first + c0 + k];
  const double is = a.lis[en.l];
  const double* Wl = a.ne.W + en.woff - en.lo;
  const int ga0 = kCholNB * it.ti + dseg, gb0 = kCholNB * it.tj + dseg;
  cl[0] = a.lc[en.l];
  cl[1] = is * a.ne.wld[en.l] * sc_ld;
  cl[2] = en.lo / kCholNB == it.ti ? 1.0 : 0.0;
  if (ga0 + 8 > en.lo && ga0 < en.hi) {
#pragma unroll
    for (int e = 0; e < 8; ++e)
      if (ga0 + e >= en.lo && ga0 + e < en.hi) va[e] = is * Wl[ga0 + e] * scA[dseg + e];
  }
  if (!diag && gb0 + 8 > en.lo && gb0 < en.hi) {
#pragma unroll
    for (int e = 0; e < 8; ++e)
      if (gb0 + e >= en.lo && gb0 + e < en.hi) vb[e] = is * Wl[gb0 + e] * scB[dseg + e];
  }
}

__global__ void __launch_bounds__(256, 2) schur_tile_kernel(LinearLaunch a) {
  __shared__ __align__(16) double At[kSchurKC * kTS];
  __shared__ __align__(16) double Bt[kSchurKC * kTS];
  __shared__ double scA[kCholNB], scB[kCholNB], cvec[3][kSchurKC];
  const SchurTileItem it = a.schur_items[blockIdx.x];
  const int tid = threadIdx.x;
  const Lane L = lane_of(tid);
  const int np = a.dims.np, npad = a.npad, ild = a.dims.idx_ld;
  const bool diag = it.ti == it.tj;
  if (tid < kCholNB) {
    const int ga = kCholNB * it.ti + tid, gb = kCholNB * it.tj + tid;
    scA[tid] = (ga < np && !a.cmask[ga]) ? a.sc[ga] : 0.0;
    scB[tid] = (gb < np && !a.cmask[gb]) ? a.sc[gb] : 0.0;
  }
  const double sc_ld = a.cmask[ild] ? 0.0 : a.sc[ild];
  const int go = a.go ? *a.go : 1;
  __syncthreads();
  if (!go) return;
  Frag acc;
  frag_zero(acc);
  double racc = 0.0, lacc = 0.0, ll = 0.0, lr = 0.0;
  const int k = tid >> 3, dseg = (tid & 7) * 8;
  double va[8], vb[8], cl[3];
  schur_fetch(a, it, 0, k, dseg, scA, scB, sc_ld, diag, va, vb, cl);
  for (int c0 = 0; c0 < it.count; c0 += kSchurKC) {
#pragma unroll
    for (int e = 0; e < 8; e += 2) {
      *reinterpret_cast<double2*>(At + k * kTS + dseg + e) = make_double2(va[e], va[e + 1]);
      if (!diag) *reinterpret_cast<double2*>(Bt + k * kTS + dseg + e) = make_double2(vb[e], vb[e + 1]);
    }
    if ((tid & 7) == 0) { cvec[0][k] = cl[0]; cvec[1][k] = cl[1]; cvec[2][k] = cl[2]; }
    __syncthreads();
    if (c0 + kSchurKC < it.count) schur_fetch(a, it, c0 + kSchurKC, k, dseg, scA, scB, sc_ld, diag, va, vb, cl);
    tile_gemm_dmma<false, kSchurKC>(At, diag ? At : Bt, acc, L);
    if (diag) {
      if (tid < kCholNB) {
#pragma unroll 8
        for (int kk = 0; kk < kSchurKC; ++kk) {
          const double v = At[kk * kTS + tid];
          racc = fma(v, cvec[0][kk], racc);
          lacc = fma(v, cvec[1][kk], lacc);
        }
      } else if (tid < kCholNB + kSchurKC) {
        const int kk = tid - kCholNB;
        const double vld = cvec[1][kk] * cvec[2][kk];
// ... 32 lines not shown


__device__ __forceinline__ void camera_step_block(const LinearLaunch& a, int block, double* dsh) {
  __shared__ double red[3][8];
  const int np = a.dims.np;
  const int i = block * 8 + (threadIdx.x >> 5);
  const int lane = threadIdx.x & 31;
  double gd = 0, dHd = 0, dmax = 0;
  const int j0 = block * 8;
  for (int j = j0 + threadIdx.x; j < np; j += blockDim.x) dsh[j - j0] = a.cmask[j] ? 0.0 : -a.sc[j] * a.y[j];
  __syncthreads();
  if (i < np) {
    const double di = dsh[i - j0];
    if (lane == 0) {
      a.dc[i] = di;
      gd = a.ne.gc[i] * di;
      dmax = fabs(di);
      if (!isfinite(di)) a.scal->chol_fail = 1;
    }
    if (di != 0.0) {
      double s = 0;
      for (int j = i + lane; j < np; j += 32) s = fma(a.ne.A[size_t(i) * np + j] * (j == i ? 0.5 : 1.0), dsh[j - j0], s);
      dHd = 2.0 * di * s;
    }
  }
  dHd = warp_sum_d(dHd);
  if (lane == 0) { red[0][threadIdx.x >> 5] = gd; red[1][threadIdx.x >> 5] = dHd; red[2][threadIdx.x >> 5] = dmax; }
  __syncthreads();
  det_ticket_wait(a.det_ticket ? a.det_ticket + 1 : nullptr, blockIdx.x);
  if (threadIdx.x == 0) {
    double g = 0, h = 0, m = 0;
    for (int w = 0; w < 8; ++w) { g += red[0][w]; h += red[1][w]; m = fmax(m, red[2][w]); }
    atomicAdd(&a.scal->gd, g);
    atomicAdd(&a.scal->dHd, h);
    atomic_max_pos(&a.scal->dir_max, m);
  }
  det_ticket_done(a.det_ticket ? a.det_ticket + 1 : nullptr, blockIdx.x);
}

__device__ __forceinline__ void landmark_step_block(const LinearLaunch& a, int block, const ApplyLaunch* ap = nullptr) {
  __shared__ double red[3][8];
  __shared__ double red2[2][8];
  double xn = 0, sn = 0;
  const int lane = threadIdx.x & 31, warp = threadIdx.x >> 5;
  const int l = block * 8 + warp;
  double gd = 0, dHd = 0, dmax = 0;
  if (l < a.dims.nL) {
    const double sl = a.sl[l];
    const int lo = a.lm.lo[l], hi = a.lm.hi[l], ild = a.dims.idx_ld;
    const double* Wl = a.ne.W + a.lm.woff[l] - lo;
    double wy = 0;
    for (int g = lo + lane; g < hi; g += 32) wy = fma(Wl[g], a.cmask[g] ? 0.0 : a.sc[g] * a.y[g], wy);
    wy = warp_sum_d(wy);
    if (lane == 0) {
      wy = fma(a.ne.wld[l], a.cmask[ild] ? 0.0 : a.sc[ild] * a.y[ild], wy);
      const double hh = a.hh[l];
      const double yl = hh > 0.0 ? (sl * a.ne.gl[l] - sl * wy) / hh : 0.0;
      const double d = -sl * yl;
      a.dl[l] = d;
      gd = a.ne.gl[l] * d;
      dHd = 2.0 * d * (-wy) + a.ne.hl[l] * d * d;
      dmax = fabs(d);
      if (!isfinite(d)) a.scal->chol_fail = 1;
      if (ap) {
        const double v = ap->x.rho[l], vn = v + d;
        ap->xc.rho[l] = vn;
        if (ap->active[a.dims.np + l]) { xn = v * v; sn = (v - vn) * (v - vn); }
      }
    }
  }
  if (lane == 0) { red[0][warp] = gd; red[1][warp] = dHd; red[2][warp] = dmax; red2[0][warp] = xn; red2[1][warp] = sn; }
  __syncthreads();
  det_ticket_wait(a.det_ticket ? a.det_ticket + 1 : nullptr, blockIdx.x);
  if (threadIdx.x == 0) {
    double g = 0, h = 0, m = 0, x = 0, s = 0;
    for (int w = 0; w < 8; ++w) { g += red[0][w]; h += red[1][w]; m = fmax(m, red[2][w]); x += red2[0][w]; s += red2[1][w]; }
    if (g != 0.0) atomicAdd(&a.scal->gd, g);
    if (h != 0.0) atomicAdd(&a.scal->dHd, h);
    if (m > 0.0) atomic_max_pos(&a.scal->dir_max, m);
    if (x != 0.0) atomicAdd(&a.scal->x_norm2, x);
    if (s != 0.0) atomicAdd(&a.scal->step_norm2, s);
  }
  det_ticket_done(a.det_ticket ? a.det_ticket + 1 : nullptr, blockIdx.x);
}

__global__ void __launch_bounds__(256) step_vectors_kernel(LinearLaunch a, int ncb) {
  extern __shared__ double step_dsh[];
  if (int(blockIdx.x) < ncb) camera_step_block(a, blockIdx.x, step_dsh);
  else landmark_step_block(a, blockIdx.x - ncb, nullptr);
}

__global__ void add_damping_kernel(LinearLaunch a, double radius) {
  const int i = blockIdx.x * blockDim.x + threadIdx.x;
  if (i >= a.npad) return;
  double* d = a.M + size_t(i) * a.npad + i;
  if (i < a.dims.np && !a.cmask[i]) {
    const double sd = a.sc[i] * a.sc[i] * a.diagA[i];
    *d += fmin(fmax(sd, kMinLmDiag), kMaxLmDiag) / radius;
  } else {
    *d = 1.0;
    a.rhs[i] = 0.0;
  }
}
int launch_add_damping(const LinearLaunch& a, double radius, cudaStream_t s) {
  add_damping_kernel<<<(a.npad + 255) / 256, 256, 0, s>>>(a, radius);
  return 1;
}
__global__ void extract_diag_kernel(LinearLaunch a) {
  const int i = blockIdx.x * blockDim.x + threadIdx.x;
  if (i >= a.npad) return;
  a.diagA[i] = i < a.dims.np ? a.ne.A[size_t(i) * a.dims.np + i] : 0.0;
}
int launch_extract_diag(const LinearLaunch& a, cudaStream_t s) {
  extract_diag_kernel<<<(a.npad + 255) / 256, 256, 0, s>>>(a);
  return 1;
}
__global__ void jacobi_scale_from_diag_kernel(LinearLaunch a) {
  const int i = blockIdx.x * blockDim.x + threadIdx.x;
  if (i < a.dims.np) a.sc[i] = 1.0 / (1.0 + sqrt(a.diagA[i]));
  if (i < a.dims.nL) a.sl[i] = 1.0 / (1.0 + sqrt(a.ne.hl[i]));
}
int launch_jacobi_scale_from_diag(const LinearLaunch& a, cudaStream_t s) {
  const int n = max(a.dims.np, a.dims.nL);
  jacobi_scale_from_diag_kernel<<<(n + 255) / 256, 256, 0, s>>>(a);
  return 1;
}

int launch_reduced_system(const LinearLaunch& a, double radius, cudaStream_t s, const double* radius_dev) {
  int launches = 0;
  const size_t total = std::max(size_t(a.npad) * a.npad, size_t(a.dims.nL));
  scale_copy_kernel<<<unsigned((total + 255) / 256), 256, 0, s>>>(a, radius, radius_dev);
  ++launches;
  if (a.n_schur_items > 0) {
    schur_tile_kernel<<<a.n_schur_items, 256, 0, s>>>(a);
    ++launches;
  }
  return launches;
}

int launch_step_vectors(const LinearLaunch& a, cudaStream_t s) {
  const int ncb = (a.dims.np + 7) / 8, nlb = (a.dims.nL + 7) / 8;
  step_vectors_kernel<<<ncb + nlb, 256, size_t(a.dims.np) * sizeof(double), s>>>(a, ncb);
  return 1;
}

int launch_lm_step(const LinearLaunch& a, double radius, cudaStream_t s) {
  return launch_reduced_system(a, radius, s) + launch_factor_solve(a, s) + launch_step_vectors(a, s);
}

__global__ void __launch_bounds__(1024) gradient_norm_kernel(LinearLaunch a, StatePtrs st, int fix_ld, double ld_lower,
                                                             double ld_upper, LmPublished* pub, unsigned long long seq,
                                                             LmDecideArgs da) {
  __shared__ double red[32];
  const int np = a.dims.np, nL = a.dims.nL;
  double v = 0.0;
  for (int i = blockIdx.x * blockDim.x + threadIdx.x; i < np + nL; i += gridDim.x * blockDim.x) {
    if (!a.active[i]) continue;
    double x;
    if (i < np) {
      x = fabs(a.ne.gc[i]);
      if (i == a.dims.idx_ld && !fix_ld) {
        const double ld = *st.ld;
        x = fabs(ld - fmin(fmax(ld - a.ne.gc[i], ld_lower), ld_upper));
      }
    } else {
      x = fabs(a.ne.gl[i - np]);
    }
    v = fmax(v, x);
  }
  v = warp_max_d(v);
  if ((threadIdx.x & 31) == 0) red[threadIdx.x >> 5] = v;
  __syncthreads();
  if (threadIdx.x < 32) {
    v = warp_max_d(red[threadIdx.x]);
    if (threadIdx.x == 0) {
      bool last = true;
      if (gridDim.x > 1) {
        atomicMax(reinterpret_cast<unsigned long long*>(&a.scal->gmax), static_cast<unsigned long long>(__double_as_longlong(v)));
        __threadfence();
        last = atomicAdd(&a.scal->pad[0], 1) == int(gridDim.x) - 1;
        if (last) a.scal->pad[0] = 0;
      } else {
        a.scal->gmax = fmax(a.scal->gmax, v);
      }
      if (last && pub) {
        static_assert(sizeof(LmScalars) == 88, "scalar block is copied as five 16-byte words + one 8-byte word");
        __threadfence();
        const uint4* src = reinterpret_cast<const uint4*>(a.scal);
        uint4 w[5];
#pragma unroll
        for (int k = 0; k < 5; ++k) w[k] = __ldcg(src + k);
        const uint2 w5 = __ldcg(reinterpret_cast<const uint2*>(src + 5));
        uint4* dst = reinterpret_cast<uint4*>(&pub->s);
#pragma unroll
        for (int k = 0; k < 5; ++k) dst[k] = w[k];
        *reinterpret_cast<uint2*>(dst + 5) = w5;
        if (da.dec) {
          LmScalars sc;
          uint4* loc = reinterpret_cast<uint4*>(&sc);
#pragma unroll
          for (int k = 0; k < 5; ++k) loc[k] = w[k];
          *reinterpret_cast<uint2*>(loc + 5) = w5;
          LmDecision d;
          d.model_cost_change = __dsub_rn(-sc.gd, __dmul_rn(0.5, sc.dHd));
          d.valid = (!sc.chol_fail && isfinite(d.model_cost_change) && d.model_cost_change > 0.0) ? 1 : 0;
          d.rho = __ddiv_rn(__dsub_rn(da.x_cost, sc.cost_eval), d.model_cost_change);
          d.accept = (d.valid && d.rho > da.min_relative_decrease) ? 1 : 0;
          const double t = __dsub_rn(__dmul_rn(2.0, d.rho), 1.0);
          const double t3 = __dmul_rn(__dmul_rn(t, t), t);
          d.radius_next = fmin(da.max_radius, __ddiv_rn(da.radius, fmax(1.0 / 3.0, __dsub_rn(1.0, t3))));
          const double step_norm = sqrt(sc.step_norm2), x_norm = sqrt(sc.x_norm2);
          const bool stop = step_norm <= __dmul_rn(da.parameter_tolerance, __dadd_rn(x_norm, da.parameter_tolerance)) ||
                            fabs(__dsub_rn(da.x_cost, sc.cost_eval)) <= __dmul_rn(da.function_tolerance, da.x_cost) ||
                            fmax(sc.gmax, v) <= da.gradient_tolerance || d.radius_next < da.min_radius;
          d.go = (d.accept && !stop) ? 1 : 0;
          d.pad = 0;
          *da.dec = d;
          pub->dec = d;
        }
        __threadfence_system();
        *reinterpret_cast<volatile unsigned long long*>(&pub->seq) = seq;
      }
    }
  }
}
int launch_gradient_norm(const LinearLaunch& a, const StatePtrs& st, int fix_ld, double ld_lower, double ld_upper,
                         cudaStream_t s, bool reset, LmPublished* pub, unsigned long long seq, const LmDecideArgs* decide) {
  if (reset) cudaMemsetAsync(&a.scal->gmax, 0, sizeof(double), s);
  LmDecideArgs da{};
  if (decide) da = *decide;
  const int n = a.dims.np + a.dims.nL;
  const int grid = std::min(16, std::max(1, (n + 1023) / 1024));
  gradient_norm_kernel<<<grid, 1024, 0, s>>>(a, st, fix_ld, ld_lower, ld_upper, pub, seq, da);
  return 1;
}

__global__ void publish_kernel(const LmPublished* __restrict__ stage, LmPublished* pub) {
  if (threadIdx.x == 0) {
    static_assert(sizeof(LmPublished) % 16 == 0, "copied as 16-byte words");
    constexpr int kWords = int(offsetof(LmPublished, seq) / 16);
    static_assert(offsetof(LmPublished, seq) % 16 == 0, "payload is a whole number of 16-byte words");
    const uint4* src = reinterpret_cast<const uint4*>(stage);
    uint4* dst = reinterpret_cast<uint4*>(pub);
    uint4 w[kWords];
#pragma unroll
    for (int k = 0; k < kWords; ++k) w[k] = __ldcg(src + k);
    const unsigned long long seq = __ldcg(&stage->seq);
#pragma unroll
    for (int k = 0; k < kWords; ++k) dst[k] = w[k];
    __threadfence_system();
    *reinterpret_cast<volatile unsigned long long*>(&pub->seq) = seq;
  }
}
int launch_publish(const LmPublished* stage, LmPublished* pub, cudaStream_t s) {
  publish_kernel<<<1, 32, 0, s>>>(stage, pub);
  return 1;
}

struct StepSource {
  const double* dc;
  const double* y;
  const double* sc;
  const uint8_t* cmask;
  __device__ __forceinline__ double operator()(int g) const {
    if (dc) return dc[g];
    return cmask[g] ? 0.0 : -sc[g] * y[g];
  }
};

__device__ __forceinline__ Q4 stepped_knot(const ApplyLaunch& a, const StepSource& src, int i) {
  const double d0 = src(6 * i), d1 = src(6 * i + 1), d2 = src(6 * i + 2);
  const Q4 q = load_q(a.x.q, i);
  if (d0 != 0.0 || d1 != 0.0 || d2 != 0.0) return so3_mul(q, so3_exp(V3{a.alpha * d0, a.alpha * d1, a.alpha * d2}));
  return q;
}

__device__ __forceinline__ void apply_step_block(const ApplyLaunch& a, const StepSource& src, int block, bool with_landmarks) {
  __shared__ double red[2][8];
  const int i = block * blockDim.x + threadIdx.x;
  const int nK = a.dims.nK, nB = a.dims.nB, nL = with_landmarks ? a.dims.nL : 0;
  double xn = 0, sn = 0;
  if (i < nK) {
    const Q4 q = load_q(a.x.q, i);
    const Q4 qn = stepped_knot(a, src, i);
    a.xc.q[4 * i] = qn.x; a.xc.q[4 * i + 1] = qn.y; a.xc.q[4 * i + 2] = qn.z; a.xc.q[4 * i + 3] = qn.w;
    if (i + 1 < nK) {
      const Q4 qm = stepped_knot(a, src, i + 1);
      const double q2[8] = {qn.x, qn.y, qn.z, qn.w, qm.x, qm.y, qm.z, qm.w};
      KnotPair kp;
      make_knot_pair(q2, 0, kp);
      a.xc.tab[i] = kp;
    }
    if (a.count_camera && a.active[6 * i]) {
      xn += q.x * q.x + q.y * q.y + q.z * q.z + q.w * q.w;
      sn += (q.x - qn.x) * (q.x - qn.x) + (q.y - qn.y) * (q.y - qn.y) + (q.z - qn.z) * (q.z - qn.z) + (q.w - qn.w) * (q.w - qn.w);
    }
#pragma unroll
    for (int c = 0; c < 3; ++c) {
      const double p = a.x.p[kPStride * i + c];
      const double pn = p + a.alpha * src(6 * i + 3 + c);
      a.xc.p[kPStride * i + c] = pn;
      if (a.count_camera && a.active[6 * i + 3 + c]) { xn += p * p; sn += (p - pn) * (p - pn); }
    }
    a.xc.p[kPStride * i + 3] = 0.0;
  } else if (i < nK + 6 * nB) {
    const int b = i - nK;
    const double v = a.x.bias[b];
    const double vn = v + a.alpha * src(a.dims.idx_bias0 + b);
    a.xc.bias[b] = vn;
    if (a.count_camera && a.active[a.dims.idx_bias0 + b]) { xn += v * v; sn += (v - vn) * (v - vn); }
  } else if (i == nK + 6 * nB) {
    const double v = *a.x.ld;
    double vn = v + a.alpha * src(a.dims.idx_ld);
    if (a.clamp_ld) vn = fmin(fmax(vn, a.ld_lower), a.ld_upper);
    *a.xc.ld = vn;
    a.scal->ld_value = vn;
    if (a.count_camera && a.active[a.dims.idx_ld]) { xn += v * v; sn += (v - vn) * (v - vn); }
  } else if (i < nK + 6 * nB + 1 + nL) {
    const int l = i - (nK + 6 * nB + 1);
    const double v = a.x.rho[l];
    const double vn = v + a.alpha * a.dl[l];
    a.xc.rho[l] = vn;
    if (a.active[a.dims.np + l]) { xn += v * v; sn += (v - vn) * (v - vn); }
  }
  xn = warp_sum_d(xn); sn = warp_sum_d(sn);
  if ((threadIdx.x & 31) == 0) { red[0][threadIdx.x >> 5] = xn; red[1][threadIdx.x >> 5] = sn; }
  __syncthreads();
  det_ticket_wait(a.det_ticket ? a.det_ticket + 1 : nullptr, blockIdx.x);
  if (threadIdx.x == 0) {
    double x = 0, s = 0;
    for (int w = 0; w < 8; ++w) { x += red[0][w]; s += red[1][w]; }
    if (x != 0.0) atomicAdd(&a.scal->x_norm2, x);
    if (s != 0.0) atomicAdd(&a.scal->step_norm2, s);
  }
  det_ticket_done(a.det_ticket ? a.det_ticket + 1 : nullptr, blockIdx.x);
}

__global__ void __launch_bounds__(256) apply_step_kernel(ApplyLaunch a) {
  apply_step_block(a, StepSource{a.dc, nullptr, nullptr, nullptr}, blockIdx.x, true);
}

int launch_apply_step(const ApplyLaunch& a, cudaStream_t s, bool reset) {
  const int n = a.dims.nK + 6 * a.dims.nB + 1 + a.dims.nL;
  if (reset) cudaMemsetAsync(&a.scal->step_norm2, 0, 2 * sizeof(double), s);
  apply_step_kernel<<<(n + 255) / 256, 256, 0, s>>>(a);
  return 1;
}

__global__ void __launch_bounds__(256) step_apply_kernel(LinearLaunch a, ApplyLaunch ap, int ncb, int nlb) {
  extern __shared__ double step_dsh[];
  const int b = blockIdx.x;
  if (b < ncb) camera_step_block(a, b, step_dsh);
  else if (b < ncb + nlb) landmark_step_block(a, b - ncb, &ap);
  else apply_step_block(ap, StepSource{nullptr, a.y, a.sc, a.cmask}, b - ncb - nlb, false);
}

int launch_step_and_apply(const LinearLaunch& a, const ApplyLaunch& ap, cudaStream_t s) {
  const int ncb = (a.dims.np + 7) / 8, nlb = (a.dims.nL + 7) / 8;
  const int nab = (a.dims.nK + 6 * a.dims.nB + 1 + 255) / 256;
  step_apply_kernel<<<ncb + nlb + nab, 256, size_t(a.dims.np) * sizeof(double), s>>>(a, ap, ncb, nlb);
  return 1;
}

__device__ void r2ypr_deg(const M3& R, double ypr[3]) {
  const double nx = R.m[0], ny = R.m[3], nz = R.m[6];
  const double ox = R.m[1], oy = R.m[4];
  const double ax = R.m[2], ay = R.m[5];
  const double y = atan2(ny, nx);
  const double p = atan2(-nz, nx * cos(y) + ny * sin(y));
  const double r = atan2(ax * sin(y) - ay * cos(y), -ox * sin(y) + oy * cos(y));
  const double k = 180.0 / 3.14159265358979323846;
  ypr[0] = y * k; ypr[1] = p * k; ypr[2] = r * k;
}

__global__ void gauge_realign_kernel(StatePtrs st, int nK, int min_idx, const double* R0t0) {
  __shared__ double T[16];
  if (threadIdx.x == 0) {
// ... 34 lines not shown
```

ctrl-vio_b200/csrc/kernels_residual.cu:

```cuda
#include <cstdio>

#include "kernels.h"

namespace ctvio {


__device__ __forceinline__ uint32_t smem_u32(const void* p) { return static_cast<uint32_t>(__cvta_generic_to_shared(p)); }

__device__ __forceinline__ void mbar_init(uint64_t* bar, uint32_t count) {
  asm volatile("mbarrier.init.shared::cta.b64 [%0], %1;" ::"r"(smem_u32(bar)), "r"(count) : "memory");
}
__device__ __forceinline__ void fence_mbar_init() { asm volatile("fence.mbarrier_init.release.cluster;" ::: "memory"); }
__device__ __forceinline__ void fence_proxy_async() { asm volatile("fence.proxy.async.shared::cta;" ::: "memory"); }
__device__ __forceinline__ void mbar_expect_tx(uint64_t* bar, uint32_t bytes) {
  asm volatile("mbarrier.arrive.expect_tx.shared::cta.b64 _, [%0], %1;" ::"r"(smem_u32(bar)), "r"(bytes) : "memory");
}
__device__ __forceinline__ void tma_bulk_g2s(void* dst, const void* src, uint32_t bytes, uint64_t* bar) {
  asm volatile("cp.async.bulk.shared::cluster.global.mbarrier::complete_tx::bytes [%0], [%1], %2, [%3];" ::"r"(
                   smem_u32(dst)),
               "l"(src), "r"(bytes), "r"(smem_u32(bar))
               : "memory");
}
__device__ __forceinline__ bool mbar_try_wait(uint64_t* bar, uint32_t phase) {
  uint32_t ok;
  asm volatile(
      "{\n"
      ".reg .pred p;\n"
      "mbarrier.try_wait.parity.shared::cta.b64 p, [%1], %2;\n"
      "selp.u32 %0, 1, 0, p;\n"
      "}\n"
      : "=r"(ok)
      : "r"(smem_u32(bar)), "r"(phase)
      : "memory");
  return ok != 0;
}

__device__ __forceinline__ double warp_sum(double v) {
#pragma unroll
  for (int o = 16; o > 0; o >>= 1) v += __shfl_xor_sync(0xffffffffu, v, o);
  return v;
}


__global__ void knot_table_kernel(StatePtrs st, int nK) {
  const int k = blockIdx.x * blockDim.x + threadIdx.x;
  if (k >= nK - 1) return;
  KnotPair kp;
  make_knot_pair(st.q, k, kp);
  st.tab[k] = kp;
}

int launch_knot_table(const StatePtrs& st, int nK, cudaStream_t s) {
  if (nK < 2) return 0;
  knot_table_kernel<<<(nK - 1 + 127) / 128, 128, 0, s>>>(st, nK);
  return 1;
}


struct VisArgs {
  ImageObsPtrs obs;
  const VisualItem* items;
  StatePtrs st;
  NormalEqPtrs ne;
  LandmarkLayout lm;
  ProblemDims dims;
  SplineParams sp;
  RigParams rig;
  double cauchy;
  const uint8_t* cmask;
  LmScalars* scal;
  int use_tma;
  int* det_ticket;
};

struct __align__(128) VisStatic {
  KnotPair tab[2][4];
  double q[2][kWinKnots][4];
  double p[2][kWinKnots][4];
  double cost_part[8];
  unsigned long long bar;
  int err;
};

__constant__ uint8_t c_tile_i[36] = {0, 0, 0, 0, 0, 0, 0, 0, 1, 1, 1, 1, 1, 1, 1, 2, 2, 2,
                                     2, 2, 2, 3, 3, 3, 3, 3, 4, 4, 4, 4, 5, 5, 5, 6, 6, 7};
__constant__ uint8_t c_tile_j[36] = {0, 1, 2, 3, 4, 5, 6, 7, 1, 2, 3, 4, 5, 6, 7, 2, 3, 4,
                                     5, 6, 7, 3, 4, 5, 6, 7, 4, 5, 6, 7, 5, 6, 7, 6, 7, 7};

#ifdef CTVIO_CHOL_TIMING
__device__ long long g_vis_clk[8];
#define VCLK(i) do { if (blockIdx.x == 0 && threadIdx.x == 0) g_vis_clk[(i)] = clock64(); } while (0)
extern "C" int ctvio_debug_vis_clk(long long* out) {
  return cudaMemcpyFromSymbol(out, g_vis_clk, sizeof(g_vis_clk)) == cudaSuccess ? 0 : -1;
}
#else
#define VCLK(i)
#endif

size_t visual_smem_bytes() {
  return size_t(kVisObsPerRound) * kObsStride * sizeof(double) + size_t(36) * 64 * sizeof(double);
}

__device__ __noinline__ void syrk_round(const double* Jt, double* accs, int nround, int tid) {
  const int warp = tid >> 5, lane = tid & 31, g = lane >> 2, q = lane & 3;
  const int nblk = warp < 6 ? 1 : 2;
  int bi[2], bj[2];
  if (warp < 6) {
    bi[0] = warp < 3 ? 0 : (warp < 5 ? 1 : 2);
    bj[0] = warp < 3 ? warp + 1 : (warp < 5 ? warp - 1 : 3);
    bi[1] = bj[1] = 0;
  } else {
    bi[0] = bj[0] = 2 * (warp - 6);
    bi[1] = bj[1] = 2 * (warp - 6) + 1;
  }
  const bool dg = warp >= 6;
  double acc[2][2][2][2];
#pragma unroll
  for (int b = 0; b < 2; ++b)
#pragma unroll
    for (int mi = 0; mi < 2; ++mi)
#pragma unroll
      for (int nj = 0; nj < 2; ++nj) {
        const int ti = 2 * bi[b] + mi, tj = 2 * bj[b] + nj;
        double2 v = make_double2(0.0, 0.0);
        if (b < nblk && ti <= tj) v = *reinterpret_cast<const double2*>(accs + (ti * 8 - ti * (ti - 1) / 2 + (tj - ti)) * 64 + g * 8 + 2 * q);
        acc[b][mi][nj][0] = v.x; acc[b][mi][nj][1] = v.y;
      }
  const int nsteps = (2 * nround + 3) >> 2;
#pragma unroll 2
  for (int st = 0; st < nsteps; ++st) {
    const int row = 4 * st + q;
    const double* rp = Jt + size_t(row >> 1) * kObsStride + (row & 1) * kRowStride + g;
#pragma unroll
    for (int b = 0; b < 2; ++b) {
      if (b < nblk) {
        double av[2], bv[2];
#pragma unroll
        for (int m = 0; m < 2; ++m) {
          av[m] = rp[16 * bi[b] + 8 * m];
          bv[m] = dg ? av[m] : rp[16 * bj[b] + 8 * m];
        }
#pragma unroll
        for (int mi = 0; mi < 2; ++mi)
#pragma unroll
          for (int nj = 0; nj < 2; ++nj) {
            if (dg && mi == 1 && nj == 0) continue;
            asm volatile("mma.sync.aligned.m8n8k4.row.col.f64.f64.f64.f64 {%0,%1}, {%2}, {%3}, {%0,%1};"
                         : "+d"(acc[b][mi][nj][0]), "+d"(acc[b][mi][nj][1])
                         : "d"(av[mi]), "d"(bv[nj]));
          }
      }
    }
  }
#pragma unroll
  for (int b = 0; b < 2; ++b)
#pragma unroll
    for (int mi = 0; mi < 2; ++mi)
#pragma unroll
      for (int nj = 0; nj < 2; ++nj) {
        const int ti = 2 * bi[b] + mi, tj = 2 * bj[b] + nj;
        if (b < nblk && ti <= tj)
          *reinterpret_cast<double2*>(accs + (ti * 8 - ti * (ti - 1) / 2 + (tj - ti)) * 64 + g * 8 + 2 * q) =
              make_double2(acc[b][mi][nj][0], acc[b][mi][nj][1]);
      }
  __syncthreads();
}

template <bool FULL>
__global__ void __launch_bounds__(kVisThreads, 1) visual_kernel(const __grid_constant__ VisArgs a) {
  extern __shared__ __align__(128) unsigned char dyn_smem[];
  double* Jt = reinterpret_cast<double*>(dyn_smem);
  double* accs = Jt + size_t(kVisObsPerRound) * kObsStride;
  __shared__ VisStatic sm;

  const int tid = threadIdx.x;
  const int lane = tid & 31, warp = tid >> 5;
  const VisualItem item = a.items[blockIdx.x];
  const int nK = a.dims.nK;
  VCLK(0);

  const int w0[2] = {item.wi0, item.wj0};
  if (a.use_tma) {
    if (tid == 0) {
      sm.err = 0;
      mbar_init(reinterpret_cast<uint64_t*>(&sm.bar), 1);
      fence_mbar_init();
    }
    __syncthreads();
    if (tid == 0) {
      uint32_t bytes = 0;
#pragma unroll
      for (int sd = 0; sd < 2; ++sd) {
        const int nk = min(kWinKnots, nK - w0[sd]);
        const int npair = min(4, nK - 1 - w0[sd]);
        bytes += uint32_t(nk) * 64u + uint32_t(npair) * uint32_t(sizeof(KnotPair));
      }
      mbar_expect_tx(reinterpret_cast<uint64_t*>(&sm.bar), bytes);
#pragma unroll
      for (int sd = 0; sd < 2; ++sd) {
        const int nk = min(kWinKnots, nK - w0[sd]);
        const int npair = min(4, nK - 1 - w0[sd]);
        tma_bulk_g2s(&sm.q[sd][0][0], a.st.q + 4 * w0[sd], uint32_t(nk) * 32u, reinterpret_cast<uint64_t*>(&sm.bar));
        tma_bulk_g2s(&sm.p[sd][0][0], a.st.p + 4 * w0[sd], uint32_t(nk) * 32u, reinterpret_cast<uint64_t*>(&sm.bar));
        tma_bulk_g2s(&sm.tab[sd][0], a.st.tab + w0[sd], uint32_t(npair) * uint32_t(sizeof(KnotPair)),
                     reinterpret_cast<uint64_t*>(&sm.bar));
      }
    }
  } else {
    if (tid == 0) sm.err = 0;
    for (int i = tid; i < 2 * kWinKnots * 4; i += kVisThreads) {
      const int sd = i / (kWinKnots * 4), r = i % (kWinKnots * 4);
      const int k = w0[sd] + r / 4;
      (&sm.q[sd][0][0])[r] = k < nK ? a.st.q[4 * k + (r & 3)] : 0.0;
      (&sm.p[sd][0][0])[r] = k < nK ? a.st.p[4 * k + (r & 3)] : 0.0;
    }
    for (int i = tid; i < 2 * 4 * 16; i += kVisThreads) {
      const int sd = i / 64, r = i % 64;
      const int k = w0[sd] + r / 16;
      reinterpret_cast<double*>(&sm.tab[sd][0])[r] = k < nK - 1 ? reinterpret_cast<const double*>(a.st.tab + k)[r & 15] : 0.0;
    }
  }
  if (FULL)
    for (int i = tid; i < 36 * 64; i += kVisThreads) accs[i] = 0.0;
  if (a.use_tma) {
    while (!mbar_try_wait(reinterpret_cast<uint64_t*>(&sm.bar), 0)) {
    }
  }
  __syncthreads();

  const double ld = *a.st.ld;
  const int64_t ld_ns = int64_t(ld * 1e9);
  const int side = tid & 1;
  double cost_local = 0.0;
  VCLK(1);

  for (int base = 0; base < item.count; base += kVisObsPerRound) {
    const int nround = min(kVisObsPerRound, item.count - base);
    const int ol = tid >> 1;
    const bool active = ol < nround;
    double* row0 = Jt + size_t(ol) * kObsStride;
    double* row1 = row0 + kRowStride;
    bool valid = false;
    const unsigned m_act = __ballot_sync(0xffffffffu, active);
    if (active) {
      const int oi = item.start + base + ol;
      const longlong2 tt = a.obs.t[oi];
      const double2 pi = a.obs.pi[oi];
      const double2 pj = a.obs.pj[oi];
      const int4 meta = a.obs.meta[oi];
      const double rho = a.st.rho[meta.z];
      const int64_t w_base = FULL ? a.lm.woff[meta.z] - a.lm.lo[meta.z] : 0;
      const int64_t t_eval = side == 0 ? tt.x + int64_t(meta.x) * ld_ns : tt.y + int64_t(meta.y) * ld_ns;
      int32_t s;
      double u;
      bool ok = spline_index(a.sp, t_eval, s, u);
      const int slot = s - w0[side];
      ok = ok && (slot == 0 || slot == 1);
      const bool ok_both = __shfl_xor_sync(m_act, ok ? 1 : 0, 1) && ok;
      const unsigned m_ok = __ballot_sync(m_act, ok_both);
      valid = ok_both;
      if (!ok_both) {
        atomicOr(&sm.err, 1);
      } else {
        PoseStage ev;
        pose_stage<FULL, kPStride>(a.sp, &sm.q[side][0][0], &sm.p[side][0][0], sm.tab[side], slot, u, ev);
        M3 Ro;
        V3 po, omo, vo;
#pragma unroll
        for (int e = 0; e < 9; ++e) Ro.m[e] = __shfl_xor_sync(m_ok, ev.R.m[e], 1);
        po = V3{__shfl_xor_sync(m_ok, ev.p.x, 1), __shfl_xor_sync(m_ok, ev.p.y, 1), __shfl_xor_sync(m_ok, ev.p.z, 1)};
        if (FULL) {
          omo = V3{__shfl_xor_sync(m_ok, ev.omega.x, 1), __shfl_xor_sync(m_ok, ev.omega.y, 1),
                   __shfl_xor_sync(m_ok, ev.omega.z, 1)};
          vo = V3{__shfl_xor_sync(m_ok, ev.vel.x, 1), __shfl_xor_sync(m_ok, ev.vel.y, 1),
                  __shfl_xor_sync(m_ok, ev.vel.z, 1)};
        }
        const M3& R_i = side == 0 ? ev.R : Ro;
        const M3& R_j = side == 0 ? Ro : ev.R;
        const V3 p_i = side == 0 ? ev.p : po;
        const V3 p_j = side == 0 ? po : ev.p;
        ImageCommon cm;
        const double pixy[2] = {pi.x, pi.y}, pjxy[2] = {pj.x, pj.y};
        image_common(a.rig, pixy, pjxy, rho, R_i, p_i, R_j, p_j, a.cauchy, cm);
        if (side == 0) cost_local += cm.cost;
        if (FULL) {
          double jrho[2], lhs[6];
          image_jrho(a.rig, cm, R_i, rho, jrho);
          image_side_lhs(side, cm, ev.R, lhs);
          const int cb = side * 30;
          const int gk0 = w0[side];
          const int l = meta.z;
          double* Wl = a.ne.W + w_base;
          {
            const int unused = cb + (slot == 0 ? 4 : 0) * 6;
#pragma unroll
            for (int c = 0; c < 6; ++c) { row0[unused + c] = 0.0; row1[unused + c] = 0.0; }
          }
          const double sgn = side == 0 ? 1.0 : -1.0;
          jacobian_stage(sm.tab[side], ev, [&](int k, const M3& Jk) {
            double rk[6];
            mul23_33(lhs, Jk, rk);
            const int gd = 6 * (gk0 + slot + k);
            const int col = cb + (slot + k) * 6;
            const double ck = sgn * ev.c[k];
#pragma unroll
            for (int c = 0; c < 3; ++c) {
              const bool mr = a.cmask[gd + c] != 0, mp = a.cmask[gd + 3 + c] != 0;
              const double r0v = mr ? 0.0 : rk[c], r1v = mr ? 0.0 : rk[3 + c];
              const double p0v = mp ? 0.0 : ck * cm.JvR[c], p1v = mp ? 0.0 : ck * cm.JvR[3 + c];
              row0[col + c] = r0v; row1[col + c] = r1v;
              row0[col + 3 + c] = p0v; row1[col + 3 + c] = p1v;
#ifndef CTVIO_EXPERIMENT_NO_W_ATOMICS
              if (!a.det_ticket) {
                if (!mr) atomicAdd(Wl + gd + c, r0v * jrho[0] + r1v * jrho[1]);
                if (!mp) atomicAdd(Wl + gd + 3 + c, p0v * jrho[0] + p1v * jrho[1]);
              }
#endif
            }
          });
          if (side == 0) {
            row0[kColR] = cm.r[0]; row1[kColR] = cm.r[1];
            row0[kColRho] = jrho[0]; row1[kColRho] = jrho[1];
          } else {
            double jld[2];
            image_jld(a.rig, cm, meta.x, meta.y, R_i, omo, vo, R_j, ev.omega, ev.vel, jld);
            const bool ld_const = a.cmask[a.dims.idx_ld] != 0;
            row0[kColLd] = ld_const ? 0.0 : jld[0];
            row1[kColLd] = ld_const ? 0.0 : jld[1];
            row0[63] = 0.0; row1[63] = 0.0;
          }
          if (!a.det_ticket) {
            if (side == 0) {
              atomicAdd(a.ne.hl + l, jrho[0] * jrho[0] + jrho[1] * jrho[1]);
              atomicAdd(a.ne.gl + l, jrho[0] * cm.r[0] + jrho[1] * cm.r[1]);
            } else {
              atomicAdd(a.ne.wld + l, row0[kColLd] * jrho[0] + row1[kColLd] * jrho[1]);
            }
          }
        }
      }
    }
    if (FULL) {
      if (!valid && ol < kVisObsPerRound) {
        const int cb = side * 30;
        for (int c = 0; c < 30; ++c) { row0[cb + c] = 0.0; row1[cb + c] = 0.0; }
        if (side == 0) { row0[kColR] = row1[kColR] = 0.0; row0[kColRho] = row1[kColRho] = 0.0; }
        else { row0[kColLd] = row1[kColLd] = 0.0; row0[63] = row1[63] = 0.0; }
      }
      VCLK(2);
      __syncthreads();
      VCLK(3);
      if (a.det_ticket) {
        det_ticket_wait(a.det_ticket, blockIdx.x * 1024 + base / kVisObsPerRound);
        if (active && valid) {
          const int oi = item.start + base + ol;
          const int l = a.obs.meta[oi].z;
          const double j0 = row0[kColRho], j1 = row1[kColRho];
          if (side == 0) {
            atomicAdd(a.ne.hl + l, j0 * j0 + j1 * j1);
            atomicAdd(a.ne.gl + l, j0 * row0[kColR] + j1 * row1[kColR]);
          } else {
            atomicAdd(a.ne.wld + l, row0[kColLd] * j0 + row1[kColLd] * j1);
          }
        }
        for (int ph = 0; ph < 2; ++ph) {
          if (active && valid && side == ph) {
            const int oi = item.start + base + ol;
            const int l = a.obs.meta[oi].z;
            const double j0 = row0[kColRho], j1 = row1[kColRho];
            double* Wl = a.ne.W + (a.lm.woff[l] - a.lm.lo[l]);
            const int cb = side * 30, gk0 = w0[side];
            for (int c = 0; c < 30; ++c) {
              const double v = row0[cb + c] * j0 + row1[cb + c] * j1;
              if (v != 0.0) atomicAdd(Wl + 6 * gk0 + c, v);
            }
          }
          __threadfence();
          __syncthreads();
        }
        det_ticket_done(a.det_ticket, blockIdx.x * 1024 + base / kVisObsPerRound);
      }
      syrk_round(Jt, accs, nround, tid);
      VCLK(4);
    }
  }

  const int n_rounds = (item.count + kVisObsPerRound - 1) / kVisObsPerRound;
  det_ticket_wait(a.det_ticket, blockIdx.x * 1024 + (FULL ? n_rounds : 0));
  cost_local = warp_sum(cost_local);
  if (lane == 0) sm.cost_part[warp] = cost_local;
  __syncthreads();
  if (tid == 0) {
    double c = 0;
#pragma unroll
    for (int w = 0; w < kVisThreads / 32; ++w) c += sm.cost_part[w];
    atomicAdd(a.ne.cost, c);
    if (sm.err) atomicOr(&a.scal->error_flags, 1);
  }
  if (FULL) {
    const int np = a.dims.np;
    const int n_class = a.det_ticket ? 11 : 1;
    for (int cls = 0; cls < n_class; ++cls) {
      for (int idx = tid; idx < 36 * 64; idx += kVisThreads) {
        const double val = accs[idx];
        if (val == 0.0) continue;
        const int tile = idx >> 6, e = idx & 63;
        const int la = c_tile_i[tile] * 8 + (e >> 3), lb = c_tile_j[tile] * 8 + (e & 7);
        if (la > lb || lb > kColR || la >= kColR) continue;
        const int sa = la < 30 ? 0 : (la < 60 ? 1 : 2);
        const int ga = sa == 0 ? 6 * item.wi0 + la : (sa == 1 ? 6 * item.wj0 + (la - 30) : a.dims.idx_ld);
        if (lb == kColR) {
          if (n_class > 1 && cls != 8 + sa) continue;
          atomicAdd(a.ne.gc + ga, val);
          continue;
        }
        const int sb = lb < 30 ? 0 : (lb < 60 ? 1 : 2);
        const int gb = sb == 0 ? 6 * item.wi0 + lb : (sb == 1 ? 6 * item.wj0 + (lb - 30) : a.dims.idx_ld);
        if (n_class > 1) {
          int c;
          if (sb == 2) c = 5 + sa;
          else if (sa == sb) c = sa == 0 ? 0 : 4;
          else c = ga < gb ? 1 : (ga > gb ? 2 : 3);
          if (c != cls) continue;
        }
        const double v = (la != lb && ga == gb) ? 2.0 * val : val;
        const int g0 = min(ga, gb), g1 = max(ga, gb);
        atomicAdd(a.ne.A + size_t(g0) * np + g1, v);
      }
      if (n_class > 1) {
        __threadfence();
        __syncthreads();
      }
    }
  }
  if (a.det_ticket) {
    __threadfence();
    __syncthreads();
    if (tid == 0) asm volatile("st.release.gpu.global.s32 [%0], %1;" ::"l"(a.det_ticket), "r"((int(blockIdx.x) + 1) * 1024) : "memory");
  }
  VCLK(5);
}

int launch_visual(const VisualLaunch& l, bool full, cudaStream_t s) {
  if (l.n_items <= 0) return 0;
  VisArgs a{l.obs, l.items, l.st, l.ne, l.lm, l.dims, l.sp, l.rig, l.cauchy, l.cmask, l.scal, l.use_tma ? 1 : 0, l.det_ticket};
  static PerDeviceOnce once;
  if (once.first()) {
    cudaFuncSetAttribute(visual_kernel<true>, cudaFuncAttributeMaxDynamicSharedMemorySize, int(visual_smem_bytes()));
    cudaFuncSetAttribute(visual_kernel<false>, cudaFuncAttributeMaxDynamicSharedMemorySize, int(visual_smem_bytes()));
  }
  if (full) visual_kernel<true><<<l.n_items, kVisThreads, visual_smem_bytes(), s>>>(a);
  else visual_kernel<false><<<l.n_items, kVisThreads, 0, s>>>(a);
  return 1;
}


struct ImuArgs {
  ImuObsPtrs obs;
  const ImuItem* items;
  StatePtrs st;
  NormalEqPtrs ne;
  ProblemDims dims;
  SplineParams sp;
  RigParams rig;
  const uint8_t* cmask;
  LmScalars* scal;
  int* det_ticket;
};

constexpr int kImuThreads = 64;
constexpr int kImuCols = 32;
constexpr int kImuRowStride = 34;
__constant__ uint8_t c_imu_tile_i[10] = {0, 0, 0, 0, 1, 1, 1, 2, 2, 3};
__constant__ uint8_t c_imu_tile_j[10] = {0, 1, 2, 3, 1, 2, 3, 2, 3, 3};

template <bool FULL>
__global__ void __launch_bounds__(kImuThreads) imu_kernel(const __grid_constant__ ImuArgs a) {
  extern __shared__ __align__(16) unsigned char dyn_smem[];
  double* Js = reinterpret_cast<double*>(dyn_smem);
  double* accs = Js + kImuMaxPerItem * 6 * kImuRowStride;
  const int tid = threadIdx.x;
  const ImuItem item = a.items[blockIdx.x];
  double cost = 0.0;
  if (FULL)
    for (int i = tid; i < 10 * 64; i += kImuThreads) accs[i] = 0.0;
  if (tid < item.count) {
    const int n = item.start + tid;
    const longlong2 tn = a.obs.t_node[n];
    const double2 g0 = a.obs.ga[3 * n], g1 = a.obs.ga[3 * n + 1], g2 = a.obs.ga[3 * n + 2];
    const double gyro[3] = {g0.x, g0.y, g1.x}, accel[3] = {g1.y, g2.x, g2.y};
    const int node = item.node;
    double bias[6];
#pragma unroll
    for (int c = 0; c < 6; ++c) bias[c] = a.st.bias[6 * node + c];
    int32_t s;
    double u;
    const bool ok = spline_index(a.sp, tn.x, s, u) && s == item.s;
    double* J = Js + size_t(tid) * 6 * kImuRowStride;
    if (!ok) {
      atomicOr(&a.scal->error_flags, 1);
      if (FULL)
        for (int e = 0; e < 6 * kImuRowStride; ++e) J[e] = 0.0;
    } else {
      ImuEvalOut o;
      eval_imu<FULL, kPStride>(a.sp, a.rig, a.st.q, a.st.p, a.st.tab, s, u, gyro, accel, bias, o);
      cost = o.cost;
      if (FULL) {
        const int gb0 = a.dims.idx_bias0 + 6 * node;
#pragma unroll
        for (int r = 0; r < 6; ++r) {
          double* Jr = J + r * kImuRowStride;
#pragma unroll
          for (int k = 0; k < 4; ++k)
#pragma unroll
            for (int c = 0; c < 3; ++c) {
              Jr[k * 6 + c] = a.cmask[6 * (s + k) + c] ? 0.0 : o.Jrot[k][3 * r + c];
              Jr[k * 6 + 3 + c] = a.cmask[6 * (s + k) + 3 + c] ? 0.0 : o.Jpos[k][3 * r + c];
            }
#pragma unroll
          for (int c = 0; c < 6; ++c) Jr[24 + c] = (c == r && !a.cmask[gb0 + c]) ? a.rig.imu_info[r] : 0.0;
          Jr[30] = o.r[r];
          Jr[31] = 0.0;
        }
      }
    }
  }
  if (FULL) {
    __syncthreads();
    const int grp = tid / 10, tile = tid % 10;
    double acc[64];
    if (tid < 60) {
      const int ti = c_imu_tile_i[tile], tj = c_imu_tile_j[tile];
#pragma unroll
      for (int e = 0; e < 64; ++e) acc[e] = 0.0;
      const int nrows = 6 * item.count;
      for (int row = grp; row < nrows; row += 6) {
        const double2* ra = reinterpret_cast<const double2*>(Js + size_t(row) * kImuRowStride + ti * 8);
        const double2* rb = reinterpret_cast<const double2*>(Js + size_t(row) * kImuRowStride + tj * 8);
        double av[8], bv[8];
#pragma unroll
        for (int e = 0; e < 4; ++e) {
          const double2 x = ra[e], y = rb[e];
          av[2 * e] = x.x; av[2 * e + 1] = x.y;
          bv[2 * e] = y.x; bv[2 * e + 1] = y.y;
        }
#pragma unroll
        for (int i = 0; i < 8; ++i)
#pragma unroll
          for (int j = 0; j < 8; ++j) acc[i * 8 + j] = fma(av[i], bv[j], acc[i * 8 + j]);
      }
    }
    for (int g = 0; g < 6; ++g) {
      if (tid < 60 && grp == g) {
#pragma unroll
        for (int e = 0; e < 64; ++e) accs[tile * 64 + e] += acc[e];
      }
      __syncthreads();
    }
    const int np = a.dims.np;
    det_ticket_wait(a.det_ticket, blockIdx.x);
    for (int idx = tid; idx < 10 * 64; idx += kImuThreads) {
      const double val = accs[idx];
      if (val == 0.0) continue;
      const int tile2 = idx >> 6, e = idx & 63;
      const int la = c_imu_tile_i[tile2] * 8 + (e >> 3), lb = c_imu_tile_j[tile2] * 8 + (e & 7);
      if (la > lb || lb > 30 || la >= 30) continue;
      const int ga = la < 24 ? 6 * item.s + la : a.dims.idx_bias0 + 6 * item.node + (la - 24);
      if (lb == 30) {
        atomicAdd(a.ne.gc + ga, val);
        continue;
      }
      const int gb = lb < 24 ? 6 * item.s + lb : a.dims.idx_bias0 + 6 * item.node + (lb - 24);
      atomicAdd(a.ne.A + size_t(ga) * np + gb, val);
    }
  }
  if (!FULL) det_ticket_wait(a.det_ticket, blockIdx.x);
  cost = warp_sum(cost);
  if (tid == 0 && cost != 0.0) atomicAdd(a.ne.cost, cost);
  det_ticket_done(a.det_ticket, blockIdx.x);
}

int launch_imu(const ImuLaunch& l, bool full, cudaStream_t s) {
  if (l.n_items <= 0) return 0;
  ImuArgs a{l.obs, l.items, l.st, l.ne, l.dims, l.sp, l.rig, l.cmask, l.scal, l.det_ticket};
  const size_t smem = (size_t(kImuMaxPerItem) * 6 * kImuRowStride + 10 * 64) * sizeof(double);
  static PerDeviceOnce once;
  if (once.first()) cudaFuncSetAttribute(imu_kernel<true>, cudaFuncAttributeMaxDynamicSharedMemorySize, int(smem));
  if (full) imu_kernel<true><<<l.n_items, kImuThreads, smem, s>>>(a);
  else imu_kernel<false><<<l.n_items, kImuThreads, 0, s>>>(a);
  return 1;
}


struct SmallArgs {
  BiasFactorPtrs bf;
  PriorPtrs prior;
  StatePtrs st;
  NormalEqPtrs ne;
  ProblemDims dims;
  const uint8_t* cmask;
  LmScalars* scal;
  int deterministic;
};

__device__ __forceinline__ const double* block_data(const StatePtrs& st, int type, int index) {
  switch (type) {
    case 0: return st.q + 4 * index;
    case 1: return st.p + kPStride * index;
    case 2: return st.bias + 6 * index;
    case 3: return st.bias + 6 * index + 3;
    case 4: return st.ld;
    default: return st.rho + index;
  }
}

template <bool FULL>
__global__ void __launch_bounds__(256) small_factors_kernel(const __grid_constant__ SmallArgs a) {
  __shared__ double red[8];
  const int tid = threadIdx.x;
  double cost = 0.0;
  const int np = a.dims.np;
  for (int n = a.deterministic ? (tid == 0 ? 0 : a.bf.n) : tid; n < a.bf.n; n += a.deterministic ? 1 : blockDim.x) {
    const int2 ij = a.bf.ij[n];
#pragma unroll
    for (int k = 0; k < 6; ++k) {
      const double s = a.bf.sqrt_info[6 * n + k];
      const double r = s * (a.st.bias[6 * ij.y + k] - a.st.bias[6 * ij.x + k]);
      cost += 0.5 * r * r;
      if (FULL) {
        const int gi = a.dims.idx_bias0 + 6 * ij.x + k, gj = a.dims.idx_bias0 + 6 * ij.y + k;
        const double ji = a.cmask[gi] ? 0.0 : -s, jj = a.cmask[gj] ? 0.0 : s;
        atomicAdd(a.ne.gc + gi, ji * r);
        atomicAdd(a.ne.gc + gj, jj * r);
        atomicAdd(a.ne.A + size_t(gi) * np + gi, ji * ji);
        atomicAdd(a.ne.A + size_t(gj) * np + gj, jj * jj);
        atomicAdd(a.ne.A + size_t(min(gi, gj)) * np + max(gi, gj), ji * jj);
      }
    }
  }
  const int n = a.prior.n;
  if (n > 0) {
    for (int b = tid; b < a.prior.n_blocks; b += blockDim.x) {
      const int type = a.prior.type[b];
      const double* x = block_data(a.st, type, a.prior.index[b]);
      const double* x0 = a.prior.x0 + 4 * b;
      double* dx = a.prior.dx + a.prior.col[b];
      if (type == 0) {
        const double n2 = x0[0] * x0[0] + x0[1] * x0[1] + x0[2] * x0[2] + x0[3] * x0[3];
        const double ax = -x0[0] / n2, ay = -x0[1] / n2, az = -x0[2] / n2, aw = x0[3] / n2;
        const double bx = x[0], by = x[1], bz = x[2], bw = x[3];
        const double qx = aw * bx + ax * bw + ay * bz - az * by;
        const double qy = aw * by + ay * bw + az * bx - ax * bz;
        const double qz = aw * bz + az * bw + ax * by - ay * bx;
        const double qw = aw * bw - ax * bx - ay * by - az * bz;
        const double sg = (qw >= 0) ? 2.0 : -2.0;
        dx[0] = sg * qx; dx[1] = sg * qy; dx[2] = sg * qz;
      } else {
        const int sz = (type == 4 || type == 5) ? 1 : 3;
        for (int d = 0; d < sz; ++d) dx[d] = x[d] - x0[d];
      }
    }
    __syncthreads();
    for (int i = tid; i < n; i += blockDim.x) {
      double s = a.prior.r[i];
      const double* Ji = a.prior.J + size_t(i) * n;
      for (int j = 0; j < n; ++j) s = fma(Ji[j], a.prior.dx[j], s);
      a.prior.res[i] = s;
      cost += 0.5 * s * s;
    }
    if (FULL) {
      __syncthreads();
      for (int j = tid; j < n; j += blockDim.x) {
        const int g = a.prior.col2g[j];
        if (g < 0) continue;
        double s = 0;
        for (int i = 0; i < n; ++i) s = fma(a.prior.J[size_t(i) * n + j], a.prior.res[i], s);
        atomicAdd(a.ne.gc + g, s);
      }
    }
  }
  cost = warp_sum(cost);
  if ((tid & 31) == 0) red[tid >> 5] = cost;
  __syncthreads();
  if (tid == 0) {
    double c = 0;
    for (int w = 0; w < 8; ++w) c += red[w];
    if (c != 0.0) atomicAdd(a.ne.cost, c);
  }
}

__global__ void prior_add_jtj_kernel(PriorPtrs pr, double* A, int np) {
  const int idx = blockIdx.x * blockDim.x + threadIdx.x;
  const int n = pr.n;
  if (idx >= n * n) return;
  const int i = idx / n, j = idx % n;
  if (j < i) return;
  const int gi = pr.col2g[i], gj = pr.col2g[j];
  if (gi < 0 || gj < 0) return;
  const double v = pr.JtJ[idx];
  if (v == 0.0) return;
  atomicAdd(A + size_t(min(gi, gj)) * np + max(gi, gj), v);
}

int launch_small_factors(const SmallFactorsLaunch& l, bool full, cudaStream_t s) {
  if (l.bf.n <= 0 && l.prior.n <= 0) return 0;
  SmallArgs a{l.bf, l.prior, l.st, l.ne, l.dims, l.cmask, l.scal, l.deterministic};
  int launches = 1;
  if (full) small_factors_kernel<true><<<1, 256, 0, s>>>(a);
  else small_factors_kernel<false><<<1, 256, 0, s>>>(a);
  if (full && l.prior.n > 0) {
    const int n2 = l.prior.n * l.prior.n;
    prior_add_jtj_kernel<<<(n2 + 255) / 256, 256, 0, s>>>(l.prior, l.ne.A, l.dims.np);
    ++launches;
  }
  return launches;
}


__global__ void probe_image_kernel(VisArgs a, const int32_t* orig_index, int want_jac, double* r, int32_t* sidx,
                                   double* J) {
  const int n = blockIdx.x * blockDim.x + threadIdx.x;
  if (n >= a.obs.n) return;
  const longlong2 tt = a.obs.t[n];
  const double2 pi = a.obs.pi[n], pj = a.obs.pj[n];
  const int4 meta = a.obs.meta[n];
  const double rho = a.st.rho[meta.z];
  const int64_t ld_ns = int64_t(*a.st.ld * 1e9);
  int32_t si, sj;
  double ui, uj;
  const int out = orig_index[n];
  if (!spline_index(a.sp, tt.x + int64_t(meta.x) * ld_ns, si, ui) ||
      !spline_index(a.sp, tt.y + int64_t(meta.y) * ld_ns, sj, uj)) {
    atomicOr(&a.scal->error_flags, 1);
    return;
  }
  SideEval ea, eb;
  if (want_jac) {
    eval_side<true, kPStride>(a.sp, a.st.q, a.st.p, a.st.tab, si, ui, ea);
    eval_side<true, kPStride>(a.sp, a.st.q, a.st.p, a.st.tab, sj, uj, eb);
  } else {
    eval_side<false, kPStride>(a.sp, a.st.q, a.st.p, a.st.tab, si, ui, ea);
    eval_side<false, kPStride>(a.sp, a.st.q, a.st.p, a.st.tab, sj, uj, eb);
  }
  ImageCommon cm;
  const double pixy[2] = {pi.x, pi.y}, pjxy[2] = {pj.x, pj.y};
  image_common(a.rig, pixy, pjxy, rho, ea.R, ea.p, eb.R, eb.p, a.cauchy, cm);
  atomicAdd(a.ne.cost, cm.cost);
  if (r) { r[2 * out] = cm.r[0]; r[2 * out + 1] = cm.r[1]; }
  if (sidx) { sidx[2 * out] = si; sidx[2 * out + 1] = sj; }
  if (!want_jac || !J) return;
  double* Jo = J + size_t(out) * 100;
  double rot[4][6], pos[4][6];
  image_side_blocks(0, cm, ea, rot, pos);
  for (int k = 0; k < 4; ++k)
    for (int e = 0; e < 6; ++e) { Jo[k * 12 + e] = rot[k][e]; Jo[k * 12 + 6 + e] = pos[k][e]; }
  image_side_blocks(1, cm, eb, rot, pos);
  for (int k = 0; k < 4; ++k)
    for (int e = 0; e < 6; ++e) { Jo[48 + k * 12 + e] = rot[k][e]; Jo[48 + k * 12 + 6 + e] = pos[k][e]; }
  image_jrho(a.rig, cm, ea.R, rho, Jo + 96);
  image_jld(a.rig, cm, meta.x, meta.y, ea.R, ea.omega, ea.vel, eb.R, eb.omega, eb.vel, Jo + 98);
}

int launch_probe_image(const VisualLaunch& l, const int32_t* orig_index, bool want_jac, double* r, int32_t* s,
                       double* J, cudaStream_t st) {
  if (l.obs.n <= 0) return 0;
  VisArgs a{l.obs, l.items, l.st, l.ne, l.lm, l.dims, l.sp, l.rig, l.cauchy, l.cmask, l.scal, 0, nullptr};
  probe_image_kernel<<<(l.obs.n + 63) / 64, 64, 0, st>>>(a, orig_index, want_jac ? 1 : 0, r, s, J);
  return 1;
}

__global__ void probe_imu_kernel(ImuArgs a, const int32_t* orig_index, int want_jac, double* r, int32_t* sidx, double* J) {
  const int n = blockIdx.x * blockDim.x + threadIdx.x;
  if (n >= a.obs.n) return;
  const int out = orig_index[n];
  const longlong2 tn = a.obs.t_node[n];
  const double2 g0 = a.obs.ga[3 * n], g1 = a.obs.ga[3 * n + 1], g2 = a.obs.ga[3 * n + 2];
  const double gyro[3] = {g0.x, g0.y, g1.x}, accel[3] = {g1.y, g2.x, g2.y};
  const int node = int(tn.y);
  double bias[6];
  for (int c = 0; c < 6; ++c) bias[c] = a.st.bias[6 * node + c];
  int32_t s;
  double u;
  if (!spline_index(a.sp, tn.x, s, u)) {
    atomicOr(&a.scal->error_flags, 1);
    return;
  }
  ImuEvalOut o;
  if (want_jac) eval_imu<true, kPStride>(a.sp, a.rig, a.st.q, a.st.p, a.st.tab, s, u, gyro, accel, bias, o);
  else eval_imu<false, kPStride>(a.sp, a.rig, a.st.q, a.st.p, a.st.tab, s, u, gyro, accel, bias, o);
  atomicAdd(a.ne.cost, o.cost);
  if (r) for (int k = 0; k < 6; ++k) r[6 * out + k] = o.r[k];
  if (sidx) sidx[out] = s;
  if (!want_jac || !J) return;
  double* Jo = J + size_t(out) * 156;
  for (int k = 0; k < 4; ++k)
    for (int e = 0; e < 18; ++e) { Jo[k * 36 + e] = o.Jrot[k][e]; Jo[k * 36 + 18 + e] = o.Jpos[k][e]; }
  for (int k = 0; k < 3; ++k) {
    Jo[144 + k] = a.rig.imu_info[k]; Jo[147 + k] = 0; Jo[150 + k] = 0; Jo[153 + k] = a.rig.imu_info[3 + k];
  }
}

int launch_probe_imu(const ImuLaunch& l, const int32_t* orig_index, bool want_jac, double* r, int32_t* s, double* J,
                     cudaStream_t st) {
  if (l.obs.n <= 0) return 0;
  ImuArgs a{l.obs, l.items, l.st, l.ne, l.dims, l.sp, l.rig, l.cmask, l.scal, nullptr};
  probe_imu_kernel<<<(l.obs.n + 63) / 64, 64, 0, st>>>(a, orig_index, want_jac ? 1 : 0, r, s, J);
  return 1;
}


__global__ void query_kernel(QueryLaunch a) {
  const int n = blockIdx.x * blockDim.x + threadIdx.x;
  if (n >= a.n) return;
  int32_t s;
  double u;
  if (!spline_index(a.sp, a.t[n], s, u)) {
    atomicOr(&a.scal->error_flags, 1);
    return;
  }
  SideEval ev;
  eval_side<true, kPStride>(a.sp, a.st.q, a.st.p, a.st.tab, s, u, ev);
  if (a.q) {
    const Q4 q = quat_from_matrix(ev.R);
    a.q[4 * n] = q.x; a.q[4 * n + 1] = q.y; a.q[4 * n + 2] = q.z; a.q[4 * n + 3] = q.w;
  }
  if (a.p) { a.p[3 * n] = ev.p.x; a.p[3 * n + 1] = ev.p.y; a.p[3 * n + 2] = ev.p.z; }
  if (a.omega) { a.omega[3 * n] = ev.omega.x; a.omega[3 * n + 1] = ev.omega.y; a.omega[3 * n + 2] = ev.omega.z; }
  if (a.vel) { a.vel[3 * n] = ev.vel.x; a.vel[3 * n + 1] = ev.vel.y; a.vel[3 * n + 2] = ev.vel.z; }
  if (a.acc) {
    double c2[4];
    plain_coeffs<2>(u, a.sp.inv_dt, c2);
    V3 acc = c2[0] * load_p<kPStride>(a.st.p, s);
    for (int k = 1; k < 4; ++k) acc = acc + c2[k] * load_p<kPStride>(a.st.p, s + k);
    a.acc[3 * n] = acc.x; a.acc[3 * n + 1] = acc.y; a.acc[3 * n + 2] = acc.z;
  }
}

int launch_query(const QueryLaunch& a, cudaStream_t s) {
  if (a.n <= 0) return 0;
  query_kernel<<<(a.n + 127) / 128, 128, 0, s>>>(a);
  return 1;
}

}
```

ctrl-vio_b200/csrc/spline_eval.cuh:

```cuda
#pragma once
#include "device_math.cuh"

namespace ctvio {

struct KnotPair {
  double d[3];
  double theta;
  double jrinv[9];
  double pad[3];
};

struct SplineParams {
  int64_t t0_ns, dt_ns;
  int32_t n_knots;
  double inv_dt;
};

CTVIO_HD bool spline_index(const SplineParams& sp, int64_t t, int32_t& s, double& u) {
  const int64_t st = t - sp.t0_ns;
  if (st < 0 || t >= sp.t0_ns + int64_t(sp.n_knots - 3) * sp.dt_ns) return false;
  const int64_t si = st / sp.dt_ns;
  s = int32_t(si);
  u = double(st - si * sp.dt_ns) / double(sp.dt_ns);
  return true;
// ... 285 lines not shown
#pragma unroll
  for (int e = 0; e < 6; ++e) jv.m[e] = cm.JvR[e];
  jv.m[6] = jv.m[7] = jv.m[8] = 0.0;
  if (side == 0) {
    const M3 t = m3_mul_hat(m3_mul(jv, R_me), cm.p_Ii);
#pragma unroll
    for (int e = 0; e < 6; ++e) lhs[e] = -t.m[e];
  } else {
    const M3 t = m3_mul(m3_mul_hat(jv, cm.dp), R_me);
#pragma unroll
    for (int e = 0; e < 6; ++e) lhs[e] = t.m[e];
  }
}
CTVIO_HD void image_side_blocks(int side, const ImageCommon& cm, const SideEval& me, double rot[4][6], double pos[4][6]) {
  double lhs[6];
  image_side_lhs(side, cm, me.R, lhs);
  const double sgn = side == 0 ? 1.0 : -1.0;
#pragma unroll
  for (int k = 0; k < 4; ++k) {
    mul23_33(lhs, me.J[k], rot[k]);
#pragma unroll
    for (int e = 0; e < 6; ++e) pos[k][e] = sgn * me.c[k] * cm.JvR[e];
  }
}

CTVIO_HD void image_jrho(const RigParams& rig, const ImageCommon& cm, const M3& R_i, double rho, double out[2]) {
  const V3 t = m3_vec(R_i, m3_vec(rig.R_CI, cm.xci));
  const V3 v = V3{-t.x / rho, -t.y / rho, -t.z / rho};
  out[0] = cm.JvR[0] * v.x + cm.JvR[1] * v.y + cm.JvR[2] * v.z;
  out[1] = cm.JvR[3] * v.x + cm.JvR[4] * v.y + cm.JvR[5] * v.z;
}

CTVIO_HD void image_jld(const RigParams& rig, const ImageCommon& cm, int rowi, int rowj, const M3& R_i, V3 om_i, V3 v_i,
                        const M3& R_j, V3 om_j, V3 v_j, double out[2]) {
  const double ri = double(rowi), rj = double(rowj);
  V3 Jx = m3_tvec(R_j, ri * v_i - rj * v_j);
  const V3 a = m3_tvec(R_j, cm.dp);
  Jx = Jx - rj * cross(om_j, a);
  Jx = Jx + ri * m3_tvec(R_j, m3_vec(R_i, cross(om_i, cm.p_Ii)));
  const V3 y = m3_tvec(rig.R_CI, Jx);
  out[0] = cm.Jv[0] * y.x + cm.Jv[1] * y.y + cm.Jv[2] * y.z;
  out[1] = cm.Jv[3] * y.x + cm.Jv[4] * y.y + cm.Jv[5] * y.z;
}

struct ImuEvalOut {
  int32_t s;
  double r[6];
  double Jrot[4][18];
  double Jpos[4][18];
  double cost;
};

template <bool WANT_JAC, int PS>
CTVIO_HD void eval_imu(const SplineParams& sp, const RigParams& rig, const double* q, const double* p,
                       const KnotPair* tab, int32_t s, double u, const double gyro[3], const double accel[3],
                       const double bias[6], ImuEvalOut& o) {
  o.s = s;
  double lam[4], dl[4], ca[4];
  cum_coeffs(u, lam);
  cum_dcoeffs(u, sp.inv_dt, dl);
  plain_coeffs<2>(u, sp.inv_dt, ca);
  V3 acc = ca[0] * load_p<PS>(p, s);
#pragma unroll
  for (int k = 1; k < 4; ++k) acc = acc + ca[k] * load_p<PS>(p, s + k);
  Q4 E[3];
  V3 phi[3], d[3];
#pragma unroll
  for (int j = 0; j < 3; ++j) {
    const KnotPair& kp = tab[s + j];
    d[j] = V3{kp.d[0], kp.d[1], kp.d[2]};
    phi[j] = lam[j + 1] * d[j];
    const double th = fabs(lam[j + 1]) * kp.theta;
    E[j] = so3_exp_theta(neg(phi[j]), th * th, th);
  }
  const Q4 B3 = E[2];
  const Q4 B32 = so3_mul(B3, E[1]);
  const Q4 B321 = so3_mul(B32, E[0]);
  V3 om[4];
  om[0] = V3{0, 0, 0};
#pragma unroll
  for (int i = 0; i < 3; ++i) om[i + 1] = so3_rotate(E[i], om[i]) + dl[i + 1] * d[i];
  const Q4 Rinv_q = so3_mul(B321, q_conj(load_q(q, s)));
  const M3 Rinv = so3_matrix(Rinv_q);
  const V3 ag = acc + rig.gravity;
  const V3 a_body = so3_rotate(Rinv_q, ag);
  const V3 g = om[3];
  o.r[0] = rig.imu_info[0] * (g.x - (gyro[0] - bias[0]));
  o.r[1] = rig.imu_info[1] * (g.y - (gyro[1] - bias[1]));
  o.r[2] = rig.imu_info[2] * (g.z - (gyro[2] - bias[2]));
  o.r[3] = rig.imu_info[3] * (a_body.x - (accel[0] - bias[3]));
  o.r[4] = rig.imu_info[4] * (a_body.y - (accel[1] - bias[4]));
  o.r[5] = rig.imu_info[5] * (a_body.z - (accel[2] - bias[5]));
  double cs = 0;
#pragma unroll
  for (int k = 0; k < 6; ++k) cs += o.r[k] * o.r[k];
  o.cost = 0.5 * cs;
  if (!WANT_JAC) return;

  const M3 P[4] = {so3_matrix(B321), so3_matrix(B32), so3_matrix(B3), m3_identity()};
  M3 JrN[3], JI[3];
#pragma unroll
  for (int j = 0; j < 3; ++j) {
    JrN[j] = right_jacobian_from_half(neg(phi[j]), E[j]);
#pragma unroll
    for (int e = 0; e < 9; ++e) JI[j].m[e] = tab[s + j].jrinv[e];
  }
  M3 dw[3];
  dw[0] = m3_scale(dl[1], P[1]);
#pragma unroll
  for (int i = 1; i < 3; ++i) {
    const M3 t = m3_mul(m3_mul_hat(P[i], om[i]), JrN[i]);
#pragma unroll
    for (int e = 0; e < 9; ++e) dw[i].m[e] = lam[i + 1] * t.m[e] + dl[i + 1] * P[i + 1].m[e];
  }
  M3 Jw[4], Ja[4];
#pragma unroll
  for (int k = 0; k < 4; ++k)
#pragma unroll
    for (int e = 0; e < 9; ++e) Jw[k].m[e] = Ja[k].m[e] = 0.0;
#pragma unroll
  for (int i = 0; i < 3; ++i) {
    const M3 a = m3_mul_bt(dw[i], JI[i]), b = m3_mul(dw[i], JI[i]);
#pragma unroll
    for (int e = 0; e < 9; ++e) { Jw[i].m[e] -= a.m[e]; Jw[i + 1].m[e] += b.m[e]; }
  }
  const M3 R = m3_transpose(Rinv);
  const M3 lhs = m3_mul_hat(Rinv, ag);
  const M3 lR = m3_mul(lhs, R);
  {
    const M3 t = m3_mul(lR, P[0]);
#pragma unroll
    for (int e = 0; e < 9; ++e) Ja[0].m[e] += t.m[e];
  }
#pragma unroll
  for (int i = 0; i < 3; ++i) {
    const M3 da = m3_scale(lam[i + 1], m3_mul(m3_mul(lR, P[i]), JrN[i]));
    const M3 a = m3_mul_bt(da, JI[i]), b = m3_mul(da, JI[i]);
#pragma unroll
    for (int e = 0; e < 9; ++e) { Ja[i].m[e] -= a.m[e]; Ja[i + 1].m[e] += b.m[e]; }
  }
#pragma unroll
  for (int k = 0; k < 4; ++k)
#pragma unroll
    for (int r = 0; r < 3; ++r)
#pragma unroll
      for (int c = 0; c < 3; ++c) {
        o.Jrot[k][3 * r + c] = rig.imu_info[r] * Jw[k].m[3 * r + c];
        o.Jrot[k][9 + 3 * r + c] = rig.imu_info[3 + r] * Ja[k].m[3 * r + c];
        o.Jpos[k][3 * r + c] = 0.0;
        o.Jpos[k][9 + 3 * r + c] = rig.imu_info[3 + r] * (ca[k] * Rinv.m[3 * r + c]);
      }
}

}
```

Before: 31.45 million.

## Fuse visual, IMU, small-factor and gradient-norm evaluation into one role-dispatched kernel

Replaces the three-stream fork/join of visual, IMU and small-factor kernels with a single evaluation kernel whose CTAs take roles by block index. The gradient-norm/LM-decision tail is folded into the same launch. The IMU kernel is restructured so each knot block's Jacobian is computed separately from shared per-sample state. The visual chunk cap is now picked so that visual chunks plus fixed-role CTAs fit within the SM count. The aim is to remove launch and cross-stream synchronisation overhead and to balance work across SMs, at the cost of a uniform block size and shared-memory footprint for all roles and extra code complexity.

```diff
diff --git a/ctrl-vio_b200/csrc/engine.cu b/ctrl-vio_b200/csrc/engine.cu
--- a/ctrl-vio_b200/csrc/engine.cu
+++ b/ctrl-vio_b200/csrc/engine.cu
@@ -381,21 +381,6 @@
       hm[k] = make_int4(o.rowi, o.rowj, o.lm, o.marg);
     }
     lap("image windows + sort");
-    int cap = kVisObsPerRound;
-    if (const char* env = std::getenv("CTVIO_VIS_CAP")) cap = std::max(kVisObsPerRound, std::atoi(env) / kVisObsPerRound * kVisObsPerRound);
-    std::vector<VisualItem>& items = e->h_items;
-    items.clear();
-    for (int k = 0; k < n;) {
-      const int a = e->img_order[k];
-      int end = k;
-      while (end < n && wi0[e->img_order[end]] == wi0[a] && wj0[e->img_order[end]] == wj0[a]) ++end;
-      const int cnt = end - k;
-      const int nchunks = (cnt + cap - 1) / cap;
-      const int per = (cnt + nchunks - 1) / nchunks;
-      for (int s = k; s < end; s += per) items.push_back(VisualItem{s, std::min(per, end - s), wi0[a], wj0[a]});
-      k = end;
-    }
-    e->n_items = int(items.size());
     if (!e->img_desc.empty()) {
       std::vector<ctvio::FactorDesc> sd(n);
       for (int k = 0; k < n; ++k) sd[k] = e->img_desc[e->img_order[k]];
@@ -413,7 +398,6 @@
       CUDA_OK(e->d_img_meta.upload(hm, st));
     }
     CUDA_OK(e->d_img_orig.upload(e->img_order, st));
-    CUDA_OK(e->d_items.upload(items, st));
 
     lap("image arrays + upload");
     e->h_woff.assign(e->nL + 1, 0);
@@ -457,6 +441,36 @@
       imu_items.back().count++;
     }
     e->n_imu_items = int(imu_items.size());
+    {
+      std::vector<VisualItem>& items = e->h_items;
+      const int n_fixed = e->n_imu_items + 1 + kEvalPriorCtas;
+      const int n_sm = ctvio::device_sm_count();
+      std::vector<int> group_start;
+      for (int k = 0; k < n; ++k) {
+        const int a = e->img_order[k], b = k > 0 ? e->img_order[k - 1] : -1;
+        if (k == 0 || wi0[a] != wi0[b] || wj0[a] != wj0[b]) group_start.push_back(k);
+      }
+      group_start.push_back(n);
+      const int n_groups = int(group_start.size()) - 1;
+      int cap = kVisObsPerRound;
+      for (int c = kVisObsPerRound / 4; c < kVisObsPerRound; c *= 2) {
+        int chunks = 0;
+        for (int g = 0; g < n_groups; ++g) chunks += (group_start[g + 1] - group_start[g] + c - 1) / c;
+        if (chunks + n_fixed <= n_sm) {
+          cap = c;
+          break;
+        }
+      }
+      items.clear();
+      for (int g = 0; g < n_groups; ++g) {
+        const int k = group_start[g], end = group_start[g + 1], a = e->img_order[k];
+        const int nchunks = (end - k + cap - 1) / cap;
+        const int per = (end - k + nchunks - 1) / nchunks;
+        for (int s = k; s < end; s += per) items.push_back(VisualItem{s, std::min(per, end - s), wi0[a], wj0[a]});
+      }
+      e->n_items = int(items.size());
+      CUDA_OK(e->d_items.upload(items, st));
+    }
     CUDA_OK(e->d_imu_items.upload(imu_items, st));
     CUDA_OK(e->d_imu_orig.upload(imu_order, st));
     if (!e->imu_src.empty()) {
@@ -813,7 +827,7 @@
   return CTVIO_OK;
 }
 
-void evaluate(ctvio_engine* e, int xb, int nb, bool full, bool reset_cost = true) {
+void evaluate(ctvio_engine* e, int xb, int nb, bool full, bool reset_cost = true, const EvalTail* tail = nullptr) {
   cudaStream_t st = e->stream;
   if (full) {
     if (e->slab_zeroed[nb]) {
@@ -824,34 +838,21 @@
     }
   }
   if (reset_cost) cudaMemsetAsync(&e->d_scal.p->cost_eval, 0, sizeof(double), st);
-  const bool fork = (e->rank == 0) && (!e->imu.empty() || !e->biasf.empty() || (e->prior.n > 0 && e->prior_enabled));
+  const bool others = (e->rank == 0) && (!e->imu.empty() || !e->biasf.empty() || (e->prior.n > 0 && e->prior_enabled));
   if (e->deterministic) {
     cudaMemsetAsync(e->d_ticket.p, 0, 2 * sizeof(int32_t), st);
     e->launches += launch_visual(visual_launch(e, xb, nb, e->cfg.cauchy_solve), full, st);
-    if (fork) {
+    if (others) {
       cudaMemsetAsync(e->d_ticket.p, 0, 2 * sizeof(int32_t), st);
       e->launches += launch_imu(imu_launch(e, xb, nb), full, st);
       e->launches += launch_small_factors(small_launch(e, xb, nb), full, st);
     }
     return;
   }
-  const bool split = fork && !e->imu.empty() && (!e->biasf.empty() || (e->prior.n > 0 && e->prior_enabled));
-  if (fork) {
-    cudaEventRecord(e->ev_fork, st);
-    cudaStreamWaitEvent(e->stream2, e->ev_fork, 0);
-    e->launches += launch_imu(imu_launch(e, xb, nb), full, e->stream2);
-    if (split) {
-      cudaStreamWaitEvent(e->stream3, e->ev_fork, 0);
-      e->launches += launch_small_factors(small_launch(e, xb, nb), full, e->stream3);
-      cudaEventRecord(e->ev_join3, e->stream3);
-    } else {
-      e->launches += launch_small_factors(small_launch(e, xb, nb), full, e->stream2);
-    }
-    cudaEventRecord(e->ev_join, e->stream2);
-  }
-  e->launches += launch_visual(visual_launch(e, xb, nb, e->cfg.cauchy_solve), full, st);
-  if (fork) cudaStreamWaitEvent(st, e->ev_join, 0);
-  if (split) cudaStreamWaitEvent(st, e->ev_join3, 0);
+  const ImuLaunch im = imu_launch(e, xb, nb);
+  const SmallFactorsLaunch sm = small_launch(e, xb, nb);
+  e->launches += launch_evaluation(visual_launch(e, xb, nb, e->cfg.cauchy_solve), others ? &im : nullptr,
+                                   others ? &sm : nullptr, full, tail, st);
 }
 
 void prezero_slab(ctvio_engine* e, int nb) {
@@ -1316,13 +1317,12 @@
         if (rc) return rc;
       }
       sum.num_linear_solves++;
-      evaluate(e, cand, cand_ne, true, false);
-      sum.num_jacobian_evals++;
       const LmDecideArgs da{e->d_dec.p, x_cost, radius, min_relative_decrease, max_radius,
                             parameter_tolerance, function_tolerance, gradient_tolerance, min_radius};
-      e->launches += launch_gradient_norm(linear_launch(e, cand_ne), e->state(cand).ptrs(), e->opt.fix_ld, e->opt.ld_lower,
-                                          e->opt.ld_upper, st, false, e->staged_publish ? e->d_pubstage.p : e->h_pub, ++e->pub_seq,
-                                          &da);
+      const EvalTail tail{linear_launch(e, cand_ne), e->state(cand).ptrs(), e->opt.fix_ld, e->opt.ld_lower, e->opt.ld_upper,
+                          e->staged_publish ? e->d_pubstage.p : e->h_pub, ++e->pub_seq, da};
+      evaluate(e, cand, cand_ne, true, false, &tail);
+      sum.num_jacobian_evals++;
       cudaEventRecord(e->ev_iter, st);
       if (e->staged_publish) {
         cudaStreamWaitEvent(e->stream2, e->ev_iter, 0);
@@ -1819,6 +1819,13 @@
   DevBuf<unsigned char> flush;
   const size_t flush_bytes = size_t(256) << 20;
   if (flush_l2) CUDA_OK(flush.reserve(flush_bytes));
+  auto launch_role = [&](int role, bool full) {
+    VisualLaunch v = visual_launch(e, cur, cur, e->cfg.cauchy_solve);
+    if (role != 0) v.n_items = 0;
+    const ImuLaunch im = imu_launch(e, cur, cur);
+    const SmallFactorsLaunch sm = small_launch(e, cur, cur);
+    launch_evaluation(v, role == 1 ? &im : nullptr, role == 2 ? &sm : nullptr, full, nullptr, st);
+  };
   if (visual_only) {
     for (int k = 0; k < 8; ++k) out[k] = 0.0;
     double total = 0;
@@ -1826,7 +1833,7 @@
       if (flush_l2) cudaMemsetAsync(flush.p, it & 0xff, flush_bytes, st);
       cudaMemsetAsync(e->ne_slab[cur].p, 0, e->ne_slab_len * sizeof(double), st);
       cudaEventRecord(e->ev0, st);
-      launch_visual(visual_launch(e, cur, cur, e->cfg.cauchy_solve), true, st);
+      launch_role(0, true);
       cudaEventRecord(e->ev1, st);
       if (cudaEventSynchronize(e->ev1) != cudaSuccess) return fail(CTVIO_ERR_CUDA, "kernel failed while profiling");
       float ms = 0;
@@ -1859,14 +1866,14 @@
         cudaMemsetAsync(e->ne_slab[cur].p, 0, e->ne_slab_len * sizeof(double), st);
       cudaEventRecord(e->ev0, st);
       switch (stage) {
-        case 0: launch_visual(visual_launch(e, cur, cur, e->cfg.cauchy_solve), true, st); break;
-        case 1: launch_imu(imu_launch(e, cur, cur), true, st); break;
-        case 2: launch_small_factors(small_launch(e, cur, cur), true, st); break;
+        case 0: launch_role(0, true); break;
+        case 1: launch_role(1, true); break;
+        case 2: launch_role(2, true); break;
         case 3: launch_reduced_system(lin, 1e4, st); break;
         case 4: launch_factor_solve(lin, st); break;
         case 5: launch_step_vectors(lin, st); break;
         case 6: launch_apply_step(ap, st); break;
-        default: launch_visual(visual_launch(e, cur, cur, e->cfg.cauchy_solve), false, st); break;
+        default: launch_role(0, false); break;
       }
       cudaEventRecord(e->ev1, st);
       if (cudaEventSynchronize(e->ev1) != cudaSuccess) return fail(CTVIO_ERR_CUDA, "kernel failed while profiling");
diff --git a/ctrl-vio_b200/csrc/kernels.h b/ctrl-vio_b200/csrc/kernels.h
--- a/ctrl-vio_b200/csrc/kernels.h
+++ b/ctrl-vio_b200/csrc/kernels.h
@@ -197,6 +197,7 @@
 };
 int launch_visual(const VisualLaunch& a, bool full, cudaStream_t s);
 size_t visual_smem_bytes();
+size_t imu_smem_bytes();
 
 struct ImuLaunch {
   ImuObsPtrs obs;
@@ -281,6 +282,19 @@
                          cudaStream_t s, bool reset = true, LmPublished* pub = nullptr, unsigned long long seq = 0,
                          const LmDecideArgs* decide = nullptr);
 
+constexpr int kEvalPriorCtas = 4;
+struct EvalTail {
+  LinearLaunch lin;
+  StatePtrs st;
+  int fix_ld;
+  double ld_lower, ld_upper;
+  LmPublished* pub;
+  unsigned long long seq;
+  LmDecideArgs da;
+};
+int launch_evaluation(const VisualLaunch& v, const ImuLaunch* imu, const SmallFactorsLaunch* small, bool full,
+                      const EvalTail* tail, cudaStream_t s);
+
 struct ApplyLaunch {
   int32_t count_camera;
   ProblemDims dims;
diff --git a/ctrl-vio_b200/csrc/kernels_linear.cu b/ctrl-vio_b200/csrc/kernels_linear.cu
--- a/ctrl-vio_b200/csrc/kernels_linear.cu
+++ b/ctrl-vio_b200/csrc/kernels_linear.cu
@@ -4,6 +4,7 @@
 #include <cstddef>
 
 #include "kernels.h"
+#include "step_publish.cuh"
 
 namespace ctvio {
 
@@ -342,77 +343,7 @@
                                                              double ld_upper, LmPublished* pub, unsigned long long seq,
                                                              LmDecideArgs da) {
   __shared__ double red[32];
-  const int np = a.dims.np, nL = a.dims.nL;
-  double v = 0.0;
-  for (int i = blockIdx.x * blockDim.x + threadIdx.x; i < np + nL; i += gridDim.x * blockDim.x) {
-    if (!a.active[i]) continue;
-    double x;
-    if (i < np) {
-      x = fabs(a.ne.gc[i]);
-      if (i == a.dims.idx_ld && !fix_ld) {
-        const double ld = *st.ld;
-        x = fabs(ld - fmin(fmax(ld - a.ne.gc[i], ld_lower), ld_upper));
-      }
-    } else {
-      x = fabs(a.ne.gl[i - np]);
-    }
-    v = fmax(v, x);
-  }
-  v = warp_max_d(v);
-  if ((threadIdx.x & 31) == 0) red[threadIdx.x >> 5] = v;
-  __syncthreads();
-  if (threadIdx.x < 32) {
-    v = warp_max_d(red[threadIdx.x]);
-    if (threadIdx.x == 0) {
-      bool last = true;
-      if (gridDim.x > 1) {
-        atomicMax(reinterpret_cast<unsigned long long*>(&a.scal->gmax), static_cast<unsigned long long>(__double_as_longlong(v)));
-        __threadfence();
-        last = atomicAdd(&a.scal->pad[0], 1) == int(gridDim.x) - 1;
-        if (last) a.scal->pad[0] = 0;
-      } else {
-        a.scal->gmax = fmax(a.scal->gmax, v);
-      }
-      if (last && pub) {
-        static_assert(sizeof(LmScalars) == 88, "scalar block is copied as five 16-byte words + one 8-byte word");
-        __threadfence();
-        const uint4* src = reinterpret_cast<const uint4*>(a.scal);
-        uint4 w[5];
-#pragma unroll
-        for (int k = 0; k < 5; ++k) w[k] = __ldcg(src + k);
-        const uint2 w5 = __ldcg(reinterpret_cast<const uint2*>(src + 5));
-        uint4* dst = reinterpret_cast<uint4*>(&pub->s);
-#pragma unroll
-        for (int k = 0; k < 5; ++k) dst[k] = w[k];
-        *reinterpret_cast<uint2*>(dst + 5) = w5;
-        if (da.dec) {
-          LmScalars sc;
-          uint4* loc = reinterpret_cast<uint4*>(&sc);
-#pragma unroll
-          for (int k = 0; k < 5; ++k) loc[k] = w[k];
-          *reinterpret_cast<uint2*>(loc + 5) = w5;
-          LmDecision d;
-          d.model_cost_change = __dsub_rn(-sc.gd, __dmul_rn(0.5, sc.dHd));
-          d.valid = (!sc.chol_fail && isfinite(d.model_cost_change) && d.model_cost_change > 0.0) ? 1 : 0;
-          d.rho = __ddiv_rn(__dsub_rn(da.x_cost, sc.cost_eval), d.model_cost_change);
-          d.accept = (d.valid && d.rho > da.min_relative_decrease) ? 1 : 0;
-          const double t = __dsub_rn(__dmul_rn(2.0, d.rho), 1.0);
-          const double t3 = __dmul_rn(__dmul_rn(t, t), t);
-          d.radius_next = fmin(da.max_radius, __ddiv_rn(da.radius, fmax(1.0 / 3.0, __dsub_rn(1.0, t3))));
-          const double step_norm = sqrt(sc.step_norm2), x_norm = sqrt(sc.x_norm2);
-          const bool stop = step_norm <= __dmul_rn(da.parameter_tolerance, __dadd_rn(x_norm, da.parameter_tolerance)) ||
-                            fabs(__dsub_rn(da.x_cost, sc.cost_eval)) <= __dmul_rn(da.function_tolerance, da.x_cost) ||
-                            fmax(sc.gmax, v) <= da.gradient_tolerance || d.radius_next < da.min_radius;
-          d.go = (d.accept && !stop) ? 1 : 0;
-          d.pad = 0;
-          *da.dec = d;
-          pub->dec = d;
-        }
-        __threadfence_system();
-        *reinterpret_cast<volatile unsigned long long*>(&pub->seq) = seq;
-      }
-    }
-  }
+  gradient_norm_block(a, st, fix_ld, ld_lower, ld_upper, pub, seq, da, blockIdx.x, gridDim.x, red);
 }
 int launch_gradient_norm(const LinearLaunch& a, const StatePtrs& st, int fix_ld, double ld_lower, double ld_upper,
                          cudaStream_t s, bool reset, LmPublished* pub, unsigned long long seq, const LmDecideArgs* decide) {
diff --git a/ctrl-vio_b200/csrc/kernels_residual.cu b/ctrl-vio_b200/csrc/kernels_residual.cu
--- a/ctrl-vio_b200/csrc/kernels_residual.cu
+++ b/ctrl-vio_b200/csrc/kernels_residual.cu
@@ -1,6 +1,9 @@
+#include <algorithm>
 #include <cstdio>
+#include <cstring>
 
 #include "kernels.h"
+#include "step_publish.cuh"
 
 namespace ctvio {
 
@@ -89,13 +92,15 @@
 
 #ifdef CTVIO_CHOL_TIMING
 __device__ long long g_vis_clk[8];
-#define VCLK(i) do { if (blockIdx.x == 0 && threadIdx.x == 0) g_vis_clk[(i)] = clock64(); } while (0)
+#define VCLK(i) do { if (bid == 0 && threadIdx.x == 0) g_vis_clk[(i)] = clock64(); } while (0)
 extern "C" int ctvio_debug_vis_clk(long long* out) {
   return cudaMemcpyFromSymbol(out, g_vis_clk, sizeof(g_vis_clk)) == cudaSuccess ? 0 : -1;
 }
 #else
 #define VCLK(i)
 #endif
+
+extern __shared__ __align__(128) unsigned char dyn_smem[];
 
 size_t visual_smem_bytes() {
   return size_t(kVisObsPerRound) * kObsStride * sizeof(double) + size_t(36) * 64 * sizeof(double);
@@ -167,15 +172,14 @@
 }
 
 template <bool FULL>
-__global__ void __launch_bounds__(kVisThreads, 1) visual_kernel(const __grid_constant__ VisArgs a) {
-  extern __shared__ __align__(128) unsigned char dyn_smem[];
+__device__ __forceinline__ void visual_role(const VisArgs& a, int bid) {
   double* Jt = reinterpret_cast<double*>(dyn_smem);
   double* accs = Jt + size_t(kVisObsPerRound) * kObsStride;
   __shared__ VisStatic sm;
 
   const int tid = threadIdx.x;
   const int lane = tid & 31, warp = tid >> 5;
-  const VisualItem item = a.items[blockIdx.x];
+  const VisualItem item = a.items[bid];
   const int nK = a.dims.nK;
   VCLK(0);
 
@@ -351,7 +355,7 @@
       __syncthreads();
       VCLK(3);
       if (a.det_ticket) {
-        det_ticket_wait(a.det_ticket, blockIdx.x * 1024 + base / kVisObsPerRound);
+        det_ticket_wait(a.det_ticket, bid * 1024 + base / kVisObsPerRound);
         if (active && valid) {
           const int oi = item.start + base + ol;
           const int l = a.obs.meta[oi].z;
@@ -378,7 +382,7 @@
           __threadfence();
           __syncthreads();
         }
-        det_ticket_done(a.det_ticket, blockIdx.x * 1024 + base / kVisObsPerRound);
+        det_ticket_done(a.det_ticket, bid * 1024 + base / kVisObsPerRound);
       }
       syrk_round(Jt, accs, nround, tid);
       VCLK(4);
@@ -386,7 +390,7 @@
   }
 
   const int n_rounds = (item.count + kVisObsPerRound - 1) / kVisObsPerRound;
-  det_ticket_wait(a.det_ticket, blockIdx.x * 1024 + (FULL ? n_rounds : 0));
+  det_ticket_wait(a.det_ticket, bid * 1024 + (FULL ? n_rounds : 0));
   cost_local = warp_sum(cost_local);
   if (lane == 0) sm.cost_part[warp] = cost_local;
   __syncthreads();
@@ -436,9 +440,14 @@
   if (a.det_ticket) {
     __threadfence();
     __syncthreads();
-    if (tid == 0) asm volatile("st.release.gpu.global.s32 [%0], %1;" ::"l"(a.det_ticket), "r"((int(blockIdx.x) + 1) * 1024) : "memory");
+    if (tid == 0) asm volatile("st.release.gpu.global.s32 [%0], %1;" ::"l"(a.det_ticket), "r"((bid + 1) * 1024) : "memory");
   }
   VCLK(5);
+}
+
+template <bool FULL>
+__global__ void __launch_bounds__(kVisThreads, 1) visual_kernel(const __grid_constant__ VisArgs a) {
+  visual_role<FULL>(a, blockIdx.x);
 }
 
 int launch_visual(const VisualLaunch& l, bool full, cudaStream_t s) {
@@ -468,24 +477,25 @@
   int* det_ticket;
 };
 
-constexpr int kImuThreads = 64;
+constexpr int kImuThreads = 4 * kImuMaxPerItem;
 constexpr int kImuCols = 32;
 constexpr int kImuRowStride = 34;
 __constant__ uint8_t c_imu_tile_i[10] = {0, 0, 0, 0, 1, 1, 1, 2, 2, 3};
 __constant__ uint8_t c_imu_tile_j[10] = {0, 1, 2, 3, 1, 2, 3, 2, 3, 3};
 
 template <bool FULL>
-__global__ void __launch_bounds__(kImuThreads) imu_kernel(const __grid_constant__ ImuArgs a) {
-  extern __shared__ __align__(16) unsigned char dyn_smem[];
+__device__ __forceinline__ void imu_role(const ImuArgs& a, int bid) {
+  const int nthr = blockDim.x;
   double* Js = reinterpret_cast<double*>(dyn_smem);
   double* accs = Js + kImuMaxPerItem * 6 * kImuRowStride;
   const int tid = threadIdx.x;
-  const ImuItem item = a.items[blockIdx.x];
+  const ImuItem item = a.items[bid];
   double cost = 0.0;
   if (FULL)
-    for (int i = tid; i < 10 * 64; i += kImuThreads) accs[i] = 0.0;
-  if (tid < item.count) {
-    const int n = item.start + tid;
+    for (int i = tid; i < 10 * 64; i += nthr) accs[i] = 0.0;
+  const int smp = tid >> 2, kb = tid & 3;
+  if (smp < item.count && (FULL || kb == 0)) {
+    const int n = item.start + smp;
     const longlong2 tn = a.obs.t_node[n];
     const double2 g0 = a.obs.ga[3 * n], g1 = a.obs.ga[3 * n + 1], g2 = a.obs.ga[3 * n + 2];
     const double gyro[3] = {g0.x, g0.y, g1.x}, accel[3] = {g1.y, g2.x, g2.y};
@@ -496,31 +506,38 @@
     int32_t s;
     double u;
     const bool ok = spline_index(a.sp, tn.x, s, u) && s == item.s;
-    double* J = Js + size_t(tid) * 6 * kImuRowStride;
+    double* J = Js + size_t(smp) * 6 * kImuRowStride;
     if (!ok) {
-      atomicOr(&a.scal->error_flags, 1);
+      if (kb == 0) atomicOr(&a.scal->error_flags, 1);
       if (FULL)
-        for (int e = 0; e < 6 * kImuRowStride; ++e) J[e] = 0.0;
+        for (int e = kb; e < 6 * kImuRowStride; e += 4) J[e] = 0.0;
     } else {
-      ImuEvalOut o;
-      eval_imu<FULL, kPStride>(a.sp, a.rig, a.st.q, a.st.p, a.st.tab, s, u, gyro, accel, bias, o);
-      cost = o.cost;
+      ImuShared sh;
+      imu_shared_stage<kPStride>(a.sp, a.rig, a.st.q, a.st.p, a.st.tab, s, u, gyro, accel, bias, sh);
+      if (kb == 0) cost = sh.cost;
       if (FULL) {
-        const int gb0 = a.dims.idx_bias0 + 6 * node;
+        double jr[18], jp[18];
+        imu_knot_block<kPStride>(a.rig, a.st.tab, s, sh, kb, jr, jp);
+        const int gd = 6 * (s + kb);
 #pragma unroll
         for (int r = 0; r < 6; ++r) {
-          double* Jr = J + r * kImuRowStride;
-#pragma unroll
-          for (int k = 0; k < 4; ++k)
-#pragma unroll
-            for (int c = 0; c < 3; ++c) {
-              Jr[k * 6 + c] = a.cmask[6 * (s + k) + c] ? 0.0 : o.Jrot[k][3 * r + c];
-              Jr[k * 6 + 3 + c] = a.cmask[6 * (s + k) + 3 + c] ? 0.0 : o.Jpos[k][3 * r + c];
-            }
-#pragma unroll
-          for (int c = 0; c < 6; ++c) Jr[24 + c] = (c == r && !a.cmask[gb0 + c]) ? a.rig.imu_info[r] : 0.0;
-          Jr[30] = o.r[r];
-          Jr[31] = 0.0;
+          double* Jr = J + r * kImuRowStride + kb * 6;
+#pragma unroll
+          for (int c = 0; c < 3; ++c) {
+            Jr[c] = a.cmask[gd + c] ? 0.0 : jr[3 * r + c];
+            Jr[3 + c] = a.cmask[gd + 3 + c] ? 0.0 : jp[3 * r + c];
+          }
+        }
+        if (kb == 0) {
+          const int gb0 = a.dims.idx_bias0 + 6 * node;
+#pragma unroll
+          for (int r = 0; r < 6; ++r) {
+            double* Jr = J + r * kImuRowStride;
+#pragma unroll
+            for (int c = 0; c < 6; ++c) Jr[24 + c] = (c == r && !a.cmask[gb0 + c]) ? a.rig.imu_info[r] : 0.0;
+            Jr[30] = sh.r[r];
+            Jr[31] = 0.0;
+          }
         }
       }
     }
@@ -558,8 +575,8 @@
       __syncthreads();
     }
     const int np = a.dims.np;
-    det_ticket_wait(a.det_ticket, blockIdx.x);
-    for (int idx = tid; idx < 10 * 64; idx += kImuThreads) {
+    det_ticket_wait(a.det_ticket, bid);
+    for (int idx = tid; idx < 10 * 64; idx += nthr) {
       const double val = accs[idx];
       if (val == 0.0) continue;
       const int tile2 = idx >> 6, e = idx & 63;
@@ -574,16 +591,30 @@
       atomicAdd(a.ne.A + size_t(ga) * np + gb, val);
     }
   }
-  if (!FULL) det_ticket_wait(a.det_ticket, blockIdx.x);
+  if (!FULL) det_ticket_wait(a.det_ticket, bid);
+  __shared__ double cost_part[kVisThreads / 32];
   cost = warp_sum(cost);
-  if (tid == 0 && cost != 0.0) atomicAdd(a.ne.cost, cost);
-  det_ticket_done(a.det_ticket, blockIdx.x);
-}
+  if ((tid & 31) == 0) cost_part[tid >> 5] = cost;
+  __syncthreads();
+  if (tid == 0) {
+    double c = 0.0;
+    for (int w = 0; w < nthr / 32; ++w) c += cost_part[w];
+    if (c != 0.0) atomicAdd(a.ne.cost, c);
+  }
+  det_ticket_done(a.det_ticket, bid);
+}
+
+template <bool FULL>
+__global__ void __launch_bounds__(kImuThreads) imu_kernel(const __grid_constant__ ImuArgs a) {
+  imu_role<FULL>(a, blockIdx.x);
+}
+
+size_t imu_smem_bytes() { return (size_t(kImuMaxPerItem) * 6 * kImuRowStride + 10 * 64) * sizeof(double); }
 
 int launch_imu(const ImuLaunch& l, bool full, cudaStream_t s) {
   if (l.n_items <= 0) return 0;
   ImuArgs a{l.obs, l.items, l.st, l.ne, l.dims, l.sp, l.rig, l.cmask, l.scal, l.det_ticket};
-  const size_t smem = (size_t(kImuMaxPerItem) * 6 * kImuRowStride + 10 * 64) * sizeof(double);
+  const size_t smem = imu_smem_bytes();
   static PerDeviceOnce once;
   if (once.first()) cudaFuncSetAttribute(imu_kernel<true>, cudaFuncAttributeMaxDynamicSharedMemorySize, int(smem));
   if (full) imu_kernel<true><<<l.n_items, kImuThreads, smem, s>>>(a);
@@ -615,7 +646,7 @@
 }
 
 template <bool FULL>
-__global__ void __launch_bounds__(256) small_factors_kernel(const __grid_constant__ SmallArgs a) {
+__device__ __forceinline__ void small_role(const SmallArgs& a) {
   __shared__ double red[8];
   const int tid = threadIdx.x;
   double cost = 0.0;
@@ -689,8 +720,12 @@
   }
 }
 
-__global__ void prior_add_jtj_kernel(PriorPtrs pr, double* A, int np) {
-  const int idx = blockIdx.x * blockDim.x + threadIdx.x;
+template <bool FULL>
+__global__ void __launch_bounds__(256) small_factors_kernel(const __grid_constant__ SmallArgs a) {
+  small_role<FULL>(a);
+}
+
+__device__ __forceinline__ void prior_add_jtj_entry(const PriorPtrs& pr, double* A, int np, int idx) {
   const int n = pr.n;
   if (idx >= n * n) return;
   const int i = idx / n, j = idx % n;
@@ -700,6 +735,9 @@
   const double v = pr.JtJ[idx];
   if (v == 0.0) return;
   atomicAdd(A + size_t(min(gi, gj)) * np + max(gi, gj), v);
+}
+__global__ void prior_add_jtj_kernel(PriorPtrs pr, double* A, int np) {
+  prior_add_jtj_entry(pr, A, np, blockIdx.x * blockDim.x + threadIdx.x);
 }
 
 int launch_small_factors(const SmallFactorsLaunch& l, bool full, cudaStream_t s) {
@@ -714,6 +752,83 @@
     ++launches;
   }
   return launches;
+}
+
+
+struct EvalArgs {
+  VisArgs vis;
+  ImuArgs imu;
+  SmallArgs small;
+  int n_imu, n_small, n_prior, n_vis;
+  int has_tail;
+  EvalTail tail;
+};
+
+template <bool FULL>
+__global__ void __launch_bounds__(kVisThreads, 1) evaluation_kernel(const __grid_constant__ EvalArgs a) {
+  __shared__ double red[32];
+  __shared__ int last;
+  int b = blockIdx.x;
+  if (b < a.n_imu) {
+    imu_role<FULL>(a.imu, b);
+  } else if ((b -= a.n_imu) < a.n_small) {
+    small_role<FULL>(a.small);
+  } else if ((b -= a.n_small) < a.n_prior) {
+    const int n2 = a.small.prior.n * a.small.prior.n;
+    for (int idx = b * kVisThreads + threadIdx.x; idx < n2; idx += a.n_prior * kVisThreads)
+      prior_add_jtj_entry(a.small.prior, a.small.ne.A, a.small.dims.np, idx);
+  } else if ((b -= a.n_prior) < a.n_vis) {
+    visual_role<FULL>(a.vis, b);
+  }
+  if (!a.has_tail) return;
+  LmScalars* scal = a.tail.lin.scal;
+  __threadfence();
+  __syncthreads();
+  if (threadIdx.x == 0) {
+    last = atomicAdd(&scal->pad[1], 1) == int(gridDim.x) - 1;
+    if (last) scal->pad[1] = 0;
+  }
+  __syncthreads();
+  if (!last) return;
+  __threadfence();
+  gradient_norm_block(a.tail.lin, a.tail.st, a.tail.fix_ld, a.tail.ld_lower, a.tail.ld_upper, a.tail.pub, a.tail.seq,
+                      a.tail.da, 0, 1, red);
+}
+
+int launch_evaluation(const VisualLaunch& v, const ImuLaunch* imu, const SmallFactorsLaunch* small, bool full,
+                      const EvalTail* tail, cudaStream_t s) {
+  EvalArgs a;
+  std::memset(&a, 0, sizeof(a));
+  a.vis = VisArgs{v.obs, v.items, v.st, v.ne, v.lm, v.dims, v.sp, v.rig, v.cauchy, v.cmask, v.scal, v.use_tma ? 1 : 0, nullptr};
+  a.n_vis = std::max(v.n_items, 0);
+  size_t smem = 0;
+  if (full && a.n_vis > 0) smem = visual_smem_bytes();
+  if (imu && imu->n_items > 0) {
+    const ImuLaunch& l = *imu;
+    a.imu = ImuArgs{l.obs, l.items, l.st, l.ne, l.dims, l.sp, l.rig, l.cmask, l.scal, nullptr};
+    a.n_imu = l.n_items;
+    if (full) smem = std::max(smem, imu_smem_bytes());
+  }
+  if (small && (small->bf.n > 0 || small->prior.n > 0)) {
+    const SmallFactorsLaunch& l = *small;
+    a.small = SmallArgs{l.bf, l.prior, l.st, l.ne, l.dims, l.cmask, l.scal, 0};
+    a.n_small = 1;
+    if (full && l.prior.n > 0)
+      a.n_prior = std::min(kEvalPriorCtas, (l.prior.n * l.prior.n + kVisThreads - 1) / kVisThreads);
+  }
+  if (tail) {
+    a.has_tail = 1;
+    a.tail = *tail;
+  }
+  const int grid = a.n_imu + a.n_small + a.n_prior + a.n_vis;
+  if (grid == 0 && !tail) return 0;
+  static PerDeviceOnce once;
+  if (once.first())
+    cudaFuncSetAttribute(evaluation_kernel<true>, cudaFuncAttributeMaxDynamicSharedMemorySize,
+                         int(std::max(visual_smem_bytes(), imu_smem_bytes())));
+  if (full) evaluation_kernel<true><<<std::max(grid, 1), kVisThreads, smem, s>>>(a);
+  else evaluation_kernel<false><<<std::max(grid, 1), kVisThreads, 0, s>>>(a);
+  return 1;
 }
 
 
diff --git a/ctrl-vio_b200/csrc/spline_eval.cuh b/ctrl-vio_b200/csrc/spline_eval.cuh
--- a/ctrl-vio_b200/csrc/spline_eval.cuh
+++ b/ctrl-vio_b200/csrc/spline_eval.cuh
@@ -461,4 +461,112 @@
       }
 }
 
-}
+struct ImuShared {
+  double lam[4], dl[4], ca[4];
+  Q4 E[3];
+  V3 phi[3], d[3], om[4];
+  Q4 Rinv_q;
+  V3 ag;
+  double r[6];
+  double cost;
+};
+
+template <int PS>
+CTVIO_HD void imu_shared_stage(const SplineParams& sp, const RigParams& rig, const double* q, const double* p,
+                               const KnotPair* tab, int32_t s, double u, const double gyro[3], const double accel[3],
+                               const double bias[6], ImuShared& o) {
+  cum_coeffs(u, o.lam);
+  cum_dcoeffs(u, sp.inv_dt, o.dl);
+  plain_coeffs<2>(u, sp.inv_dt, o.ca);
+  V3 acc = o.ca[0] * load_p<PS>(p, s);
+#pragma unroll
+  for (int k = 1; k < 4; ++k) acc = acc + o.ca[k] * load_p<PS>(p, s + k);
+#pragma unroll
+  for (int j = 0; j < 3; ++j) {
+    const KnotPair& kp = tab[s + j];
+    o.d[j] = V3{kp.d[0], kp.d[1], kp.d[2]};
+    o.phi[j] = o.lam[j + 1] * o.d[j];
+    const double th = fabs(o.lam[j + 1]) * kp.theta;
+    o.E[j] = so3_exp_theta(neg(o.phi[j]), th * th, th);
+  }
+  const Q4 B321 = so3_mul(so3_mul(o.E[2], o.E[1]), o.E[0]);
+  o.om[0] = V3{0, 0, 0};
+#pragma unroll
+  for (int i = 0; i < 3; ++i) o.om[i + 1] = so3_rotate(o.E[i], o.om[i]) + o.dl[i + 1] * o.d[i];
+  o.Rinv_q = so3_mul(B321, q_conj(load_q(q, s)));
+  o.ag = acc + rig.gravity;
+  const V3 a_body = so3_rotate(o.Rinv_q, o.ag);
+  const V3 g = o.om[3];
+  o.r[0] = rig.imu_info[0] * (g.x - (gyro[0] - bias[0]));
+  o.r[1] = rig.imu_info[1] * (g.y - (gyro[1] - bias[1]));
+  o.r[2] = rig.imu_info[2] * (g.z - (gyro[2] - bias[2]));
+  o.r[3] = rig.imu_info[3] * (a_body.x - (accel[0] - bias[3]));
+  o.r[4] = rig.imu_info[4] * (a_body.y - (accel[1] - bias[4]));
+  o.r[5] = rig.imu_info[5] * (a_body.z - (accel[2] - bias[5]));
+  double cs = 0;
+#pragma unroll
+  for (int k = 0; k < 6; ++k) cs += o.r[k] * o.r[k];
+  o.cost = 0.5 * cs;
+}
+
+CTVIO_HD M3 imu_post(const ImuShared& o, int i) {
+  if (i == 3) return m3_identity();
+  Q4 b = o.E[2];
+  if (i <= 1) b = so3_mul(b, o.E[1]);
+  if (i == 0) b = so3_mul(b, o.E[0]);
+  return so3_matrix(b);
+}
+
+template <int PS>
+CTVIO_HD void imu_knot_block(const RigParams& rig, const KnotPair* tab, int32_t s, const ImuShared& o, int k,
+                             double Jrot[18], double Jpos[18]) {
+  const M3 Rinv = so3_matrix(o.Rinv_q);
+  const M3 lR = m3_mul(m3_mul_hat(Rinv, o.ag), m3_transpose(Rinv));
+  M3 Jw, Ja;
+#pragma unroll
+  for (int e = 0; e < 9; ++e) Jw.m[e] = Ja.m[e] = 0.0;
+  if (k == 0) {
+    const M3 t = m3_mul(lR, imu_post(o, 0));
+#pragma unroll
+    for (int e = 0; e < 9; ++e) Ja.m[e] += t.m[e];
+  }
+#pragma unroll
+  for (int h = 0; h < 2; ++h) {
+    const int i = k - 1 + h;
+    if (i < 0 || i > 2) continue;
+    const M3 Pi = imu_post(o, i);
+    M3 JI, dw;
+#pragma unroll
+    for (int e = 0; e < 9; ++e) JI.m[e] = tab[s + i].jrinv[e];
+    const M3 JrN = right_jacobian_from_half(neg(o.phi[i]), o.E[i]);
+    if (i == 0) {
+      dw = m3_scale(o.dl[1], imu_post(o, 1));
+    } else {
+      const M3 t = m3_mul(m3_mul_hat(Pi, o.om[i]), JrN);
+      const M3 Pn = imu_post(o, i + 1);
+#pragma unroll
+      for (int e = 0; e < 9; ++e) dw.m[e] = o.lam[i + 1] * t.m[e] + o.dl[i + 1] * Pn.m[e];
+    }
+    const M3 da = m3_scale(o.lam[i + 1], m3_mul(m3_mul(lR, Pi), JrN));
+    if (h == 0) {
+      const M3 bw = m3_mul(dw, JI), ba = m3_mul(da, JI);
+#pragma unroll
+      for (int e = 0; e < 9; ++e) { Jw.m[e] += bw.m[e]; Ja.m[e] += ba.m[e]; }
+    } else {
+      const M3 aw = m3_mul_bt(dw, JI), aa = m3_mul_bt(da, JI);
+#pragma unroll
+      for (int e = 0; e < 9; ++e) { Jw.m[e] -= aw.m[e]; Ja.m[e] -= aa.m[e]; }
+    }
+  }
+#pragma unroll
+  for (int r = 0; r < 3; ++r)
+#pragma unroll
+    for (int c = 0; c < 3; ++c) {
+      Jrot[3 * r + c] = rig.imu_info[r] * Jw.m[3 * r + c];
+      Jrot[9 + 3 * r + c] = rig.imu_info[3 + r] * Ja.m[3 * r + c];
+      Jpos[3 * r + c] = 0.0;
+      Jpos[9 + 3 * r + c] = rig.imu_info[3 + r] * (o.ca[k] * Rinv.m[3 * r + c]);
+    }
+}
+
+}
diff --git a/ctrl-vio_b200/csrc/step_publish.cuh b/ctrl-vio_b200/csrc/step_publish.cuh
--- /dev/null
+++ b/ctrl-vio_b200/csrc/step_publish.cuh
@@ -0,0 +1,89 @@
+#pragma once
+#include "kernels.h"
+
+namespace ctvio {
+
+__device__ __forceinline__ double step_warp_max(double v) {
+#pragma unroll
+  for (int o = 16; o > 0; o >>= 1) v = fmax(v, __shfl_xor_sync(0xffffffffu, v, o));
+  return v;
+}
+
+__device__ __forceinline__ void gradient_norm_block(const LinearLaunch& a, const StatePtrs& st, int fix_ld,
+                                                    double ld_lower, double ld_upper, LmPublished* pub,
+                                                    unsigned long long seq, const LmDecideArgs& da, int block,
+                                                    int nblocks, double* red) {
+  const int np = a.dims.np, nL = a.dims.nL;
+  double v = 0.0;
+  for (int i = block * blockDim.x + threadIdx.x; i < np + nL; i += nblocks * blockDim.x) {
+    if (!a.active[i]) continue;
+    double x;
+    if (i < np) {
+      x = fabs(__ldcg(a.ne.gc + i));
+      if (i == a.dims.idx_ld && !fix_ld) {
+        const double ld = *st.ld;
+        x = fabs(ld - fmin(fmax(ld - __ldcg(a.ne.gc + i), ld_lower), ld_upper));
+      }
+    } else {
+      x = fabs(__ldcg(a.ne.gl + (i - np)));
+    }
+    v = fmax(v, x);
+  }
+  v = step_warp_max(v);
+  if ((threadIdx.x & 31) == 0) red[threadIdx.x >> 5] = v;
+  __syncthreads();
+  if (threadIdx.x < 32) {
+    v = step_warp_max(threadIdx.x < (blockDim.x >> 5) ? red[threadIdx.x] : 0.0);
+    if (threadIdx.x == 0) {
+      bool last = true;
+      if (nblocks > 1) {
+        atomicMax(reinterpret_cast<unsigned long long*>(&a.scal->gmax), static_cast<unsigned long long>(__double_as_longlong(v)));
+        __threadfence();
+        last = atomicAdd(&a.scal->pad[0], 1) == nblocks - 1;
+        if (last) a.scal->pad[0] = 0;
+      } else {
+        a.scal->gmax = fmax(__ldcg(&a.scal->gmax), v);
+      }
+      if (last && pub) {
+        static_assert(sizeof(LmScalars) == 88, "scalar block is copied as five 16-byte words + one 8-byte word");
+        __threadfence();
+        const uint4* src = reinterpret_cast<const uint4*>(a.scal);
+        uint4 w[5];
+#pragma unroll
+        for (int k = 0; k < 5; ++k) w[k] = __ldcg(src + k);
+        const uint2 w5 = __ldcg(reinterpret_cast<const uint2*>(src + 5));
+        uint4* dst = reinterpret_cast<uint4*>(&pub->s);
+#pragma unroll
+        for (int k = 0; k < 5; ++k) dst[k] = w[k];
+        *reinterpret_cast<uint2*>(dst + 5) = w5;
+        if (da.dec) {
+          LmScalars sc;
+          uint4* loc = reinterpret_cast<uint4*>(&sc);
+#pragma unroll
+          for (int k = 0; k < 5; ++k) loc[k] = w[k];
+          *reinterpret_cast<uint2*>(loc + 5) = w5;
+          LmDecision d;
+          d.model_cost_change = __dsub_rn(-sc.gd, __dmul_rn(0.5, sc.dHd));
+          d.valid = (!sc.chol_fail && isfinite(d.model_cost_change) && d.model_cost_change > 0.0) ? 1 : 0;
+          d.rho = __ddiv_rn(__dsub_rn(da.x_cost, sc.cost_eval), d.model_cost_change);
+          d.accept = (d.valid && d.rho > da.min_relative_decrease) ? 1 : 0;
+          const double t = __dsub_rn(__dmul_rn(2.0, d.rho), 1.0);
+          const double t3 = __dmul_rn(__dmul_rn(t, t), t);
+          d.radius_next = fmin(da.max_radius, __ddiv_rn(da.radius, fmax(1.0 / 3.0, __dsub_rn(1.0, t3))));
+          const double step_norm = sqrt(sc.step_norm2), x_norm = sqrt(sc.x_norm2);
+          const bool stop = step_norm <= __dmul_rn(da.parameter_tolerance, __dadd_rn(x_norm, da.parameter_tolerance)) ||
+                            fabs(__dsub_rn(da.x_cost, sc.cost_eval)) <= __dmul_rn(da.function_tolerance, da.x_cost) ||
+                            fmax(sc.gmax, v) <= da.gradient_tolerance || d.radius_next < da.min_radius;
+          d.go = (d.accept && !stop) ? 1 : 0;
+          d.pad = 0;
+          *da.dec = d;
+          pub->dec = d;
+        }
+        __threadfence_system();
+        *reinterpret_cast<volatile unsigned long long*>(&pub->seq) = seq;
+      }
+    }
+  }
+}
+
+}
```

After: 34.20 million (median of 6 runs). +8.7%, better.
